# goldenBill/Byzantine_AirComp

Hardware: AMD Instinct MI355X
Metric: GM aggregations/sec at K=1000,d=11M; % HBM roofline; 1/2/4/8 GPUs (higher is better)
Workload: dtype f32; 1 GPU; c3: gm2 K=1000 x d=11000000 fp32, B=200 Byzantine, tol 1e-5, maxiter 1000; K=1000, d=11000000, d_local=11000000, byzantine=200, iters=5, algo=stream, gram_guard=none, layout=panels, parallelism=none, passes_per_aggregation=6, input=row-major fill, packed to panels once (untimed)

## Files before the change

byzantine_aircomp_amd/_lib.py:

```python
from __future__ import annotations

import ctypes as C
import os
import threading

HERE = os.path.dirname(os.path.abspath(__file__))
LIB_PATH = os.environ.get("GMAGG_LIB") or os.path.join(HERE, "libgmagg.so")
ABI_VERSION = 5

GM_MODE_IDEAL, GM_MODE_AIRCOMP = 0, 1
GM_NOISE_PHILOX, GM_NOISE_HOST = 0, 1
GM_ALGO_AUTO, GM_ALGO_STREAM, GM_ALGO_TWOPASS, GM_ALGO_GRAM, GM_ALGO_RESIDENT = 0, 1, 2, 3, 4
GM_ALGO_GRAM_F32 = 5
GM_LAYOUT_ROWS, GM_LAYOUT_PANELS = 0, 1
GM_GUARD_NONE, GM_GUARD_ACCEPTED, GM_GUARD_REJECTED, GM_GUARD_ACCEPTED_FLOOR = 0, 1, 2, 3
GM_EXCHANGE_NONE, GM_EXCHANGE_AGENT, GM_EXCHANGE_XCD_LOCAL, GM_EXCHANGE_XCD_HIER = 0, 1, 2, 3
GM_EXCHANGE_XCD_SPLIT = 4
GM_CLIP_STATIC, GM_CLIP_ARC = 0, 1

NOISE_CB = C.CFUNCTYPE(C.c_int, C.c_void_p, C.c_int64, C.POINTER(C.c_float),
                       C.POINTER(C.c_float), C.POINTER(C.c_float))
ALLREDUCE_CB = C.CFUNCTYPE(C.c_int, C.c_void_p, C.c_void_p, C.c_int64, C.c_void_p)


class GmOpts(C.Structure):
    _fields_ = [
        ("maxiter", C.c_int64),
        ("tol", C.c_double),
        ("eps", C.c_double),
        ("mode", C.c_int32),
        ("has_noise", C.c_int32),
        ("noise_var", C.c_double),
        ("P_max", C.c_double),
        ("seed", C.c_uint64),
        ("noise_source", C.c_int32),
        ("algo", C.c_int32),
        ("noise_cb", NOISE_CB),
        ("noise_user", C.c_void_p),
        ("check_every", C.c_int32),
        ("layout", C.c_int32),
        ("pre_oma", C.c_int32),
        ("pre_oma_var", C.c_double),
        ("pre_oma_seed", C.c_uint64),
    ]


class GmResult(C.Structure):
    _fields_ = [
        ("iters", C.c_int64),
        ("last_movement", C.c_double),
        ("converged", C.c_int32),
        ("algo_used", C.c_int32),
        ("guard", C.c_int32),
        ("gram_kind", C.c_int32),
        ("exchange", C.c_int32),
    ]


class GmCclipOpts(C.Structure):
    _fields_ = [
        ("tau", C.c_double),
        ("maxiter", C.c_int64),
        ("tol", C.c_double),
        ("layout", C.c_int32),
        ("check_every", C.c_int32),
    ]


class GmCclipResult(C.Structure):
    _fields_ = [
        ("iters", C.c_int64),
        ("last_movement", C.c_double),
        ("converged", C.c_int32),
        ("clipped", C.c_int32),
    ]


_P = C.c_void_p
_I64 = C.c_int64
SIGNATURES = [
    ("gm_ctx_create", C.c_int, [C.c_int, C.POINTER(_P)]),
    ("gm_ctx_destroy", C.c_int, [_P]),
    ("gm_ctx_set_shard", C.c_int, [_P, _I64, _I64]),
    ("gm_ctx_set_allreduce", C.c_int, [_P, ALLREDUCE_CB, _P]),
    ("gm_rccl_get_unique_id", C.c_int, [_P]),
    ("gm_ctx_init_rccl", C.c_int, [_P, _P, C.c_int, C.c_int]),
    ("gm_weiszfeld_f32", C.c_int, [_P, _P, _I64, _I64, _I64, _P, _P, C.POINTER(GmOpts),
                                   C.POINTER(GmResult), _P]),
    ("gm_panel_width", _I64, [_I64]),
    ("gm_weiszfeld_bf16", C.c_int, [_P, _P, _I64, _I64, _I64, _P, _P, C.POINTER(GmOpts),
                                    C.POINTER(GmResult), _P]),
    ("gm_panel_width_bf16", _I64, [_I64]),
    ("gm_cclip_f32", C.c_int, [_P, _P, _I64, _I64, _I64, _P, _P, C.POINTER(GmCclipOpts),
                               C.POINTER(GmCclipResult), _P]),
    ("gm_cclip_bf16", C.c_int, [_P, _P, _I64, _I64, _I64, _P, _P, C.POINTER(GmCclipOpts),
                                C.POINTER(GmCclipResult), _P]),
    ("gm_weiszfeld_batched_f32", C.c_int, [_P, _P, _I64, _I64, _I64, _I64, _I64, _P, _I64, _P,
                                           _I64, C.POINTER(GmOpts), C.POINTER(GmResult), _P]),
    ("gm_mean_f32", C.c_int, [_P, _P, _I64, _I64, _I64, _P, _P]),
    ("gm_median_f32", C.c_int, [_P, _P, _I64, _I64, _I64, _P, _P]),
    ("gm_trimmed_mean_f32", C.c_int, [_P, _P, _I64, _I64, _I64, _I64, _P, _P]),
    ("gm_krum_f32", C.c_int, [_P, _P, _I64, _I64, _I64, _I64, _P, C.POINTER(_I64), _P]),
    ("gm_mean_panels_f32", C.c_int, [_P, _P, _I64, _I64, _I64, _P, _P]),
    ("gm_median_panels_f32", C.c_int, [_P, _P, _I64, _I64, _I64, _P, _P]),
    ("gm_trimmed_mean_panels_f32", C.c_int, [_P, _P, _I64, _I64, _I64, _I64, _P, _P]),
    ("gm_krum_panels_f32", C.c_int, [_P, _P, _I64, _I64, _I64, _I64, _P, C.POINTER(_I64), _P]),
    ("gm_krum_last_info", C.c_int, [_P, C.POINTER(_I64)]),
    ("gm_meamed_f32", C.c_int, [_P, _P, _I64, _I64, _I64, C.c_int32, _P, _I64, _I64, _P, _P]),
    ("gm_multi_krum_f32", C.c_int, [_P, _P, _I64, _I64, _I64, C.c_int32, _I64, _I64, _P, _P, _P]),
    ("gm_bulyan_f32", C.c_int, [_P, _P, _I64, _I64, _I64, C.c_int32, _I64, _P, _P, _P]),
    ("gm_nnm_f32", C.c_int, [_P, _P, _I64, _I64, _I64, C.c_int32, _I64, _P, _I64, C.c_int32, _P,
                             _P]),
    ("gm_dnc_f32", C.c_int, [_P, _P, _I64, _I64, _I64, C.c_int32, _P, _I64, _I64, _I64, _I64,
                             C.c_double, _P, _P, C.POINTER(C.c_int32), C.POINTER(_I64),
                             C.POINTER(C.c_int32), C.POINTER(C.c_int32), _P]),
    ("gm_fltrust_f32", C.c_int, [_P, _P, _I64, _I64, _I64, C.c_int32, _P, _I64, _P, _P, _P, _P]),
    ("gm_fltrust_bf16", C.c_int, [_P, _P, _I64, _I64, _I64, C.c_int32, _P, _I64, _P, _P, _P, _P]),
    ("gm_clip_rows_f32", C.c_int, [_P, _P, _I64, _I64, _I64, C.c_int32, _P, C.c_int32, _I64,
                                   C.c_double, _P, _I64, C.c_int32, _P, _P]),
    ("gm_clip_rows_bf16", C.c_int, [_P, _P, _I64, _I64, _I64, C.c_int32, _P, C.c_int32, _I64,
                                    C.c_double, _P, _I64, C.c_int32, _P, _P]),
    ("gm_oma_philox_f32", C.c_int, [_P, _P, _I64, _I64, _I64, C.c_double, C.c_uint64, _P]),
    ("gm_honest_variance_f32", C.c_int, [_P, _P, _I64, _I64, _I64, _P, _P]),
    ("gm_honest_variance_panels_f32", C.c_int, [_P, _P, _I64, _I64, _I64, _I64, _P, _P]),
    ("gm_oma_philox_batched_f32", C.c_int,
     [_P, _P, _I64, _I64, _I64, _I64, _I64, C.c_double, C.c_uint64, _P]),
    ("gm_oma_philox_panels_f32", C.c_int, [_P, _P, _I64, _I64, _I64, C.c_double, C.c_uint64,
                                            _P]),
    ("gm_oma_philox_batched_panels_f32", C.c_int,
     [_P, _P, _I64, _I64, _I64, _I64, _I64, C.c_double, C.c_uint64, _P]),
    ("gm_rows_to_panels_f32", C.c_int, [_P, _P, _I64, _I64, _I64, _P, _I64, _I64, _P]),
    ("gm_rows_to_panels_bf16_from_f32", C.c_int, [_P, _P, _I64, _I64, _I64, _P, _I64, _I64, _P]),
    ("gm_rows_to_panels_bf16", C.c_int, [_P, _P, _I64, _I64, _I64, _P, _I64, _I64, _P]),
    ("gm_bucket_means_f32", C.c_int, [_P, _P, _I64, _I64, _I64, C.c_int32, _P, _I64, _P, _I64,
                                      C.c_int32, _P]),
    ("gm_bucket_means_bf16", C.c_int, [_P, _P, _I64, _I64, _I64, C.c_int32, _P, _I64, _P, _I64,
                                       C.c_int32, _P]),
    ("gm_attack_affine_f32", C.c_int, [_P, _P, _I64, _I64, _I64, C.c_int32, _I64, C.c_double,
                                       C.c_double, _P]),
    ("gm_attack_affine_bf16", C.c_int, [_P, _P, _I64, _I64, _I64, C.c_int32, _I64, C.c_double,
                                        C.c_double, _P]),
    ("gm_attack_minmax_f32", C.c_int, [_P, _P, _I64, _I64, _I64, C.c_int32, _I64, C.c_int32,
                                       C.c_int32, C.POINTER(C.c_double), _P]),
    ("gm_oma_apply_f32", C.c_int, [_P, _P, _I64, _I64, _I64, _P, _P, _P, _P, _P]),
    ("gm_client_chain_f32", C.c_int, [_P, _P, _I64, _P, _I64, _I64, _P, _I64, _I64, _I64,
                                      C.c_int32, C.c_float, C.c_float, _P, _P, _P, _I64,
                                      C.c_int32, _P]),
    ("gm_fill_clients_f32", C.c_int, [_P, _P, _I64, _I64, _I64, _I64, C.c_float, C.c_float,
                                      C.c_float, C.c_float, C.c_uint64, _P]),
    ("gm_fill_normal_f32", C.c_int, [_P, _P, _I64, C.c_float, C.c_float, C.c_uint64, _P]),
    ("gm_ctx_pass_timing", C.c_int, [_P, C.c_int, C.POINTER(C.c_double), C.POINTER(_I64)]),
    ("gm_last_error", C.c_char_p, []),
    ("gm_abi_version", C.c_int, []),
]

_lib = None
_lock = threading.Lock()


class GmError(RuntimeError):
    """A libgmagg call returned a negative status."""


def load():
    global _lib
    with _lock:
        if _lib is not None:
            return _lib
        if not os.path.exists(LIB_PATH):
            raise ImportError(
                f"libgmagg.so not found at {LIB_PATH}: build it with `make` (or "
                "__graft_entry__.build()); there is no non-HIP fallback")
        lib = C.CDLL(LIB_PATH)
        for name, res, args in SIGNATURES:
            fn = getattr(lib, name)
            fn.restype, fn.argtypes = res, args
        if lib.gm_abi_version() != ABI_VERSION:
            raise ImportError(f"libgmagg ABI {lib.gm_abi_version()} != {ABI_VERSION}")
        _lib = lib
        return lib


def check(rc: int, what: str = ""):
    if rc != 0:
        msg = (_lib.gm_last_error() or b"").decode(errors="replace") if _lib else ""
        raise GmError(f"{what} failed ({rc}): {msg}")
    return rc
```

byzantine_aircomp_amd/aggregators.py:

```python
from __future__ import annotations

import atexit
import ctypes as C
import math
import operator
import os
from dataclasses import dataclass

import torch

from . import _lib
from .panels import ClientPanels

__all__ = ["gm2", "gm", "cclip", "OMA", "mean", "median", "trimmed_mean", "Krum", "GMResult",
           "last_result", "Context", "context", "honest_variance", "bucketing", "bucketed",
           "multi_krum", "bulyan", "meamed", "nnm", "mixed", "dnc", "fltrust", "clip", "arc",
           "clipped"]


@dataclass
class GMResult:
    iters: int
    last_movement: float
    converged: bool
    algo: str
    guard: str = "none"
    gram_kind: str = ""
    exchange: str = "none"


last_result: GMResult | None = None
_ALGOS = {"auto": _lib.GM_ALGO_AUTO, "stream": _lib.GM_ALGO_STREAM,
          "twopass": _lib.GM_ALGO_TWOPASS, "gram": _lib.GM_ALGO_GRAM,
          "resident": _lib.GM_ALGO_RESIDENT, "gram_f32": _lib.GM_ALGO_GRAM_F32}
_ALGO_NAMES = {v: k for k, v in _ALGOS.items()}
_GUARD_NAMES = {_lib.GM_GUARD_NONE: "none", _lib.GM_GUARD_ACCEPTED: "accepted",
                _lib.GM_GUARD_REJECTED: "rejected", _lib.GM_GUARD_ACCEPTED_FLOOR: "accepted_floor"}


def _result(res) -> "GMResult":
    return GMResult(res.iters, res.last_movement, bool(res.converged),
                    _ALGO_NAMES.get(res.algo_used, "?"), _GUARD_NAMES.get(res.guard, "?"),
                    {1: "f16_split", 2: "bf16_split", 3: "f32"}.get(res.gram_kind, ""),
                    {1: "agent", 2: "xcd_local", 3: "xcd_hier",
                     4: "xcd_split"}.get(res.exchange, "none"))


class Context:

    def __init__(self, device: int):
        self.lib = _lib.load()
        self.device = device
        h = C.c_void_p()
        _lib.check(self.lib.gm_ctx_create(device, C.byref(h)), "gm_ctx_create")
        self.handle = h
        self._keep = []

    def set_shard(self, d_total: int, d_offset: int):
        _lib.check(self.lib.gm_ctx_set_shard(self.handle, d_total, d_offset), "gm_ctx_set_shard")

    def set_allreduce(self, fn):
        def tramp(user, buf, count, stream):
            try:
                fn(buf, count, stream)
                return 0
            except Exception:
                return 1
        cb = _lib.ALLREDUCE_CB(tramp)
        self._keep.append(cb)
        _lib.check(self.lib.gm_ctx_set_allreduce(self.handle, cb, None), "gm_ctx_set_allreduce")

    def init_rccl(self, unique_id: bytes, nranks: int, rank: int):
        buf = C.create_string_buffer(bytes(unique_id), 128)
        _lib.check(self.lib.gm_ctx_init_rccl(self.handle, buf, nranks, rank), "gm_ctx_init_rccl")

    def pass_timing(self, enable: bool):
        ms, n = C.c_double(), C.c_int64()
        _lib.check(self.lib.gm_ctx_pass_timing(self.handle, int(enable), C.byref(ms),
                                               C.byref(n)), "gm_ctx_pass_timing")
        return ms.value, n.value

    def call(self, fn: str, *args):
        with torch.cuda.device(self.device):
            return _lib.check(getattr(self.lib, fn)(self.handle, *args), fn)

    def close(self):
        h, self.handle = getattr(self, "handle", None), None
        if h:
            self.lib.gm_ctx_destroy(h)
        for k, v in list(_contexts.items()):
            if v is self:
                del _contexts[k]

    def __del__(self):
        try:
            if getattr(self, "handle", None):
                self.lib.gm_ctx_destroy(self.handle)
        except Exception:
            pass


_contexts: dict[int, Context] = {}


def close_all():
    for ctx in list(_contexts.values()):
        ctx.close()


if os.environ.get("GMAGG_ATEXIT_CLOSE", "1") != "0":
    atexit.register(close_all)


def context(device: torch.device | int | None = None) -> Context:
    if not torch.cuda.is_available():
        raise RuntimeError("byzantine_aircomp_amd needs a ROCm GPU (torch.cuda.is_available() "
                           "is False); there is no CPU fallback")
    if device is None:
        idx = torch.cuda.current_device()
    elif isinstance(device, int):
        idx = device
    else:
        idx = device.index if device.index is not None else torch.cuda.current_device()
    ctx = _contexts.get(idx)
    if ctx is None:
        ctx = _contexts[idx] = Context(idx)
    return ctx


def _stream_ptr(dev: torch.device) -> int:
    return torch.cuda.current_stream(dev).cuda_stream


def _stage(t: torch.Tensor, bf16_ok: bool = False) -> torch.Tensor:
    if t.dtype != torch.float32 and not (bf16_ok and t.dtype == torch.bfloat16):
        raise TypeError(f"aggregation kernels are fp32 (got {t.dtype})")
    if t.device.type == "cuda":
        return t
    return t.to(torch.device("cuda", torch.cuda.current_device()))


def _unit_rows(X: torch.Tensor):
    if X.stride(-1) != 1 or X.stride(-2) < X.shape[-1] or X.shape[-2] == 0:
        X = X.contiguous()
    return X, max(X.stride(-2), X.shape[-1])


def _rows(X: torch.Tensor):
    if X.dim() != 2:
        raise ValueError(f"wList must be [K, d] (got {tuple(X.shape)})")
    return _unit_rows(X)


def _fp32_panels(p: ClientPanels, who: str) -> ClientPanels:
    if p.dtype != torch.float32:
        raise TypeError(f"{who} is fp32 only (got {p.dtype} ClientPanels); gm2 / gm read bf16")
    return p


def _bf16_operand(X: torch.Tensor):
    if X.dim() != 2:
        raise ValueError(f"wList must be [K, d] (got {tuple(X.shape)})")
    K, d = X.shape
    if (K > 0 and X.stride(1) == 1 and X.stride(0) >= d and X.stride(0) % 8 == 0 and d % 8 == 0
            and X.data_ptr() % 16 == 0):
        return X, X.stride(0), _lib.GM_LAYOUT_ROWS
    P = ClientPanels.from_rows(X)
    return P.data, P.panel_stride, _lib.GM_LAYOUT_PANELS


def _client_operand(wList):
    if isinstance(wList, ClientPanels):
        K, d = wList.shape
        return wList.data, wList.panel_stride, _lib.GM_LAYOUT_PANELS, K, d
    if wList.dtype == torch.bfloat16:
        K, d = wList.shape
        X, ldx, layout = _bf16_operand(_stage(wList, bf16_ok=True))
        return X, ldx, layout, K, d
    X, ldx = _rows(_stage(wList))
    K, d = X.shape
    return X, ldx, _lib.GM_LAYOUT_ROWS, K, d


def _noise_source(options) -> int:
    src = options.get("noise_source", os.environ.get("BYZ_AIRCOMP_NOISE", "device"))
    if src == "device":
        return _lib.GM_NOISE_PHILOX
    if src == "host":
        return _lib.GM_NOISE_HOST
    raise ValueError(f"noise_source must be 'device' or 'host' (got {src!r})")


def _seed(options) -> int:
    if options.get("seed") is not None:
        return int(options["seed"]) & (2 ** 64 - 1)
    return int(torch.randint(0, 2 ** 62, (1,)).item())


def _host_draws(K: int, d: int, noise_var):
    def cb(user, it, hr, hi, n):
        try:
            a = torch.normal(torch.zeros(K), 1 / math.sqrt(2))
            b = torch.normal(torch.zeros(K), 1 / math.sqrt(2))
            C.memmove(hr, a.data_ptr(), 4 * K)
            C.memmove(hi, b.data_ptr(), 4 * K)
            if noise_var is not None:
                z = torch.normal(torch.zeros(d + 1), math.sqrt(noise_var / 2))
                C.memmove(n, z.data_ptr(), 4 * (d + 1))
            return 0
        except Exception:
            return 1
    return _lib.NOISE_CB(cb)


def _gm_opts(opts: dict, aircomp: bool, layout: int, pre_var=None, pre_seed=None, shape=None):
    o = _lib.GmOpts()
    o.maxiter = int(opts["maxiter"])
    o.tol = float(opts["tol"])
    o.eps = 1e-4
    o.mode = _lib.GM_MODE_AIRCOMP if aircomp else _lib.GM_MODE_IDEAL
    o.algo = _ALGOS[opts.get("algo", "auto")]
    o.check_every = int(opts.get("check_every", 0))
    o.layout = layout
    if pre_var is not None:
        o.pre_oma = 1
        o.pre_oma_var = float(pre_var)
        o.pre_oma_seed = _seed({"seed": pre_seed})
    if aircomp:
        var = opts["noise_var"]
        o.has_noise = int(var is not None)
        o.noise_var = float(var) if var is not None else 0.0
        o.P_max = float(opts["P_max"])
        o.noise_source = _noise_source(opts)
        if o.noise_source == _lib.GM_NOISE_HOST:
            o.noise_cb = o.keep_cb = _host_draws(*shape, var)
        else:
            o.seed = _seed(opts)
    return o


def _weiszfeld(wList: torch.Tensor, options: dict, aircomp: bool):
    global last_result
    opts = {"maxiter": 200, "tol": 1e-5}
    if aircomp:
        opts.update({"noise_var": None, "P_max": 1})
    opts.update(options or {})
    pre_var = None if aircomp else opts.get("pre_oma_var")
    pre_seed = opts.get("pre_oma_seed")
    if pre_var is not None and (opts.get("guess") is None or wList.device.type != "cuda"
                                or _noise_source(opts) == _lib.GM_NOISE_HOST):
        OMA(wList, float(pre_var), noise_source=opts.get("noise_source"), seed=pre_seed)
        pre_var = None
    guess = opts.get("guess")
    bf16 = wList.dtype == torch.bfloat16
    if guess is None:
        guess = wList.mean(dim=0, dtype=torch.float32) if bf16 and not isinstance(
            wList, ClientPanels) else wList.mean(dim=0)
    maxiter = int(opts["maxiter"])
    if maxiter <= 0:
        if pre_var is not None:
            OMA(wList, float(pre_var), seed=pre_seed)
        last_result = GMResult(0, float("nan"), False, "none")
        return guess
    X, ldx, layout, K, d = _client_operand(wList)
    g0 = guess.detach().to(device=X.device, dtype=torch.float32).contiguous()
    if g0.numel() != d:
        raise ValueError(f"guess has {g0.numel()} elements, wList rows have {d}")
    out = torch.empty(d, dtype=torch.float32, device=X.device)
    if d == 0:
        last_result = GMResult(1, 0.0, True, "none")
        return out.to(wList.device)

    o = _gm_opts(opts, aircomp, layout, pre_var, pre_seed, (K, d))
    res = _lib.GmResult()
    context(X.device).call("gm_weiszfeld_bf16" if bf16 else "gm_weiszfeld_f32", X.data_ptr(), K, d,
                           ldx, g0.data_ptr(), out.data_ptr(), C.byref(o), C.byref(res),
                           _stream_ptr(X.device))
    last_result = _result(res)
    if pre_var is not None and not isinstance(wList, ClientPanels) and X is not wList:
        wList.copy_(X)
    return out if wList.device == out.device else out.to(wList.device)


def gm2(wList, options={}):
    return _weiszfeld(wList, options, aircomp=False)


def gm(wList, options={}):
    return _weiszfeld(wList, options, aircomp=True)


_CCLIP_KEYS = ("tau", "clip_iters", "clip_tol")


def _cclip_params(options):
    if options.get("tau") is None:
        raise ValueError("cclip needs options['tau'] (the clipping radius; there is no default)")
    tau = float(options["tau"])
    if not tau > 0:
        raise ValueError(f"cclip: tau must be > 0 (got {options['tau']!r})")
    iters = int(options.get("clip_iters", 1))
    if iters < 0:
        raise ValueError(f"cclip: clip_iters must be >= 0 (got {iters})")
    ctol = options.get("clip_tol")
    if ctol is not None and not float(ctol) >= 0:
        raise ValueError(f"cclip: clip_tol must be None or >= 0 (got {ctol!r})")
    return tau, iters, -1.0 if ctol is None else float(ctol)


def _run_cclip(ctx, ptr: int, bf16: bool, K: int, d: int, ldx: int, layout: int, g0, params,
               check_every: int = 0):
    tau, iters, tol = params
    out = torch.empty(d, dtype=torch.float32, device=g0.device)
    o = _lib.GmCclipOpts()
    o.tau, o.maxiter, o.tol, o.layout, o.check_every = tau, iters, tol, layout, check_every
    res = _lib.GmCclipResult()
    ctx.call("gm_cclip_bf16" if bf16 else "gm_cclip_f32", ptr, K, d, ldx, g0.data_ptr(),
             out.data_ptr(), C.byref(o), C.byref(res), _stream_ptr(g0.device))
    return out, GMResult(res.iters, res.last_movement, bool(res.converged),
                         "stream" if iters else "none"), int(res.clipped)


def cclip(wList, options={}):
    global last_result
    options = options or {}
    params = _cclip_params(options)
    if not isinstance(wList, ClientPanels) and wList.dtype not in (torch.float32, torch.bfloat16):
        raise TypeError(f"cclip reads fp32 or bf16 client updates (got {wList.dtype})")
    guess = options.get("guess")
    if guess is None:
        guess = torch.zeros(wList.shape[1], dtype=torch.float32, device=wList.device)
    if params[1] == 0:
        last_result = GMResult(0, float("nan"), False, "none")
        cclip.last_info = {"clipped": 0}
        return guess
    X, ldx, layout, K, d = _client_operand(wList)
    g0 = guess.detach().to(device=X.device, dtype=torch.float32).contiguous()
    if g0.numel() != d:
        raise ValueError(f"guess has {g0.numel()} elements, wList rows have {d}")
    if d == 0:
        last_result = GMResult(1, 0.0, True, "none")
        cclip.last_info = {"clipped": 0}
        return torch.empty(d, dtype=torch.float32, device=wList.device)
    out, last_result, clipped = _run_cclip(
        context(X.device), X.data_ptr(), X.dtype == torch.bfloat16, K, d, ldx, layout, g0, params,
        int(options.get("check_every", 0)))
    cclip.last_info = {"clipped": clipped}
    return out if wList.device == out.device else out.to(wList.device)


def _cclip_with_options(**fixed):
    unknown = sorted(set(fixed) - set(_CCLIP_KEYS))
    if unknown:
        raise TypeError(f"cclip.with_options takes {', '.join(_CCLIP_KEYS)} (got {unknown})")
    _cclip_params(fixed if "tau" in fixed else dict(fixed, tau=1.0))

    def aggregate(wList, options={}):
        return cclip(wList, {**(options or {}), **fixed})
    aggregate.__name__ = aggregate.__qualname__ = "cclip"
    aggregate.__doc__ = f"cclip with {fixed}"
    return aggregate


cclip.with_options = _cclip_with_options
cclip.last_info = {"clipped": 0}


def _fp32_operand(wList, who: str, fn: str):
    if isinstance(wList, ClientPanels):
        _fp32_panels(wList, who)
        return (wList.data, wList.panel_stride, *wList.shape, fn.replace("_f32", "_panels_f32"))
    X, ldx = _rows(_stage(wList))
    return (X, ldx, *X.shape, fn)


def _coordinate(wList, fn_name, *extra):
    X, ldx, K, d, fn_name = _fp32_operand(wList, fn_name[3:-4], fn_name)
    out = torch.empty(d, dtype=torch.float32, device=X.device)
    context(X.device).call(fn_name, X.data_ptr(), K, d, ldx, *extra, out.data_ptr(),
                           _stream_ptr(X.device))
    return out if wList.device == out.device else out.to(wList.device)


def mean(wList, options={}):
    return _coordinate(wList, "gm_mean_f32")


def median(wList, options={}):
    return _coordinate(wList, "gm_median_f32")


def trimmed_mean(wList, options={}):
    return _coordinate(wList, "gm_trimmed_mean_f32", int(wList.shape[0] * 0.1))


def Krum(wList, options):
    X, ldx, K, d, fn = _fp32_operand(wList, "Krum", "gm_krum_f32")
    out = torch.empty(d, dtype=torch.float32, device=X.device)
    idx = C.c_int64()
    ctx = context(X.device)
    ctx.call(fn, X.data_ptr(), K, d, ldx, int(options["honestSize"]), out.data_ptr(),
             C.byref(idx), _stream_ptr(X.device))
    info = (C.c_int64 * 3)()
    _lib.check(ctx.lib.gm_krum_last_info(ctx.handle, info), "gm_krum_last_info")
    Krum.last_index = idx.value
    Krum.last_info = {"algo": ("exact", "gram")[info[0]], "candidates": info[1],
                      "reason": ("ok", "not_chosen", "not_eligible", "gram_nonfinite",
                                 "candidates")[info[2]]}
    return out if wList.device == out.device else out.to(wList.device)


def _robust_operand(wList, who: str):
    if isinstance(wList, ClientPanels):
        _fp32_panels(wList, who)
        return (wList.data, wList.panel_stride, _lib.GM_LAYOUT_PANELS, *wList.shape)
    X, ldx = _rows(_stage(wList))
    return (X, ldx, _lib.GM_LAYOUT_ROWS, *X.shape)


def _robust_shape(wList, who: str):
    if isinstance(wList, ClientPanels):
        _fp32_panels(wList, who)
    elif not isinstance(wList, torch.Tensor) or wList.dtype != torch.float32:
        raise TypeError(f"{who} is fp32 only (got {getattr(wList, 'dtype', type(wList))})")
    elif wList.dim() != 2:
        raise ValueError(f"wList must be [K, d] (got {tuple(wList.shape)})")
    K, d = (int(n) for n in wList.shape)
    if K < 1:
        raise ValueError(f"{who}: wList has no rows")
    return K, d


def _honest_size(options, who: str) -> int:
    if not options or options.get("honestSize") is None:
        raise ValueError(f"{who} needs options['honestSize']")
    return int(options["honestSize"])


def meamed(wList, options):
    K, d = _robust_shape(wList, "meamed")
    keep = _honest_size(options, "meamed")
    if not 1 <= keep <= K:
        raise ValueError(f"meamed: honestSize {keep} not in [1, {K}]")
    if K > 1024:
        raise ValueError(f"meamed: K <= 1024 (got {K})")
    X, ldx, layout, K, d = _robust_operand(wList, "meamed")
    out = torch.empty(d, dtype=torch.float32, device=X.device)
    context(X.device).call("gm_meamed_f32", X.data_ptr(), K, d, ldx, layout, None, K, keep,
                           out.data_ptr(), _stream_ptr(X.device))
    return out if wList.device == out.device else out.to(wList.device)


def multi_krum(wList, options):
    K, d = _robust_shape(wList, "multi_krum")
    honest = _honest_size(options, "multi_krum")
    if not 2 <= honest <= K + 1:
        raise ValueError(f"multi_krum: honestSize {honest} not in [2, {K + 1}]")
    m = options.get("m")
    m = honest if m is None else int(m)
    if not 1 <= m <= K:
        raise ValueError(f"multi_krum: m = {m} not in [1, {K}]")
    if K > 4096:
        raise ValueError(f"multi_krum: K <= 4096 (got {K})")
    X, ldx, layout, K, d = _robust_operand(wList, "multi_krum")
    out = torch.empty(d, dtype=torch.float32, device=X.device)
    sel = (C.c_int32 * m)()
    if d > 0:
        context(X.device).call("gm_multi_krum_f32", X.data_ptr(), K, d, ldx, layout, honest, m,
                               out.data_ptr(), sel, _stream_ptr(X.device))
    multi_krum.last_selected = list(sel) if d > 0 else []
    return out if wList.device == out.device else out.to(wList.device)


multi_krum.last_selected = None


def bulyan(wList, options):
    K, d = _robust_shape(wList, "bulyan")
    honest = _honest_size(options, "bulyan")
    f = K - honest
    if honest < 1 or f < 0:
        raise ValueError(f"bulyan: honestSize {honest} not in [1, {K}]")
    if K < 4 * f + 3:
        raise ValueError(f"bulyan: K = {K} < 4f + 3 = {4 * f + 3} with f = K - honestSize = {f}")
    if K > 1024:
        raise ValueError(f"bulyan: K <= 1024 (got {K})")
    X, ldx, layout, K, d = _robust_operand(wList, "bulyan")
    out = torch.empty(d, dtype=torch.float32, device=X.device)
    theta = K - 2 * f
    sel = (C.c_int32 * theta)()
    if d > 0:
        context(X.device).call("gm_bulyan_f32", X.data_ptr(), K, d, ldx, layout, honest,
                               out.data_ptr(), sel, _stream_ptr(X.device))
    bulyan.last_selected = list(sel) if d > 0 else []
    return out if wList.device == out.device else out.to(wList.device)


bulyan.last_selected = None


def _bucket_size(s) -> int:
    try:
        if isinstance(s, bool):
            raise TypeError
        n = operator.index(s)
    except TypeError:
        raise ValueError(f"bucketing: s must be an integer >= 1 (got {s!r})") from None
    if n < 1:
        raise ValueError(f"bucketing: s must be >= 1 (got {s!r})")
    return n


def _assignment(K: int, s: int, generator=None) -> torch.Tensor:
    _bucket_size(s)
    return torch.randperm(int(K), generator=generator)


def _bucket_perm(perm, K: int) -> torch.Tensor:
    p = torch.as_tensor(perm).detach().cpu()
    if p.dim() != 1 or p.numel() != K or p.dtype.is_floating_point or p.dtype == torch.bool:
        raise ValueError(f"bucketing: perm must be {K} integers (got {tuple(p.shape)} {p.dtype})")
    p = p.to(torch.int64)
    if not torch.equal(torch.sort(p).values, torch.arange(K)):
        raise ValueError(f"bucketing: perm is not a permutation of 0..{K - 1}")
    return p


def bucketing(wList, s, perm=None, generator=None, layout=None):
    s = _bucket_size(s)
    if layout not in (None, "rows", "panels"):
        raise ValueError(f"bucketing: layout must be None, 'rows' or 'panels' (got {layout!r})")
    panels_in = isinstance(wList, ClientPanels)
    if not panels_in and (not isinstance(wList, torch.Tensor) or wList.dim() != 2):
        raise ValueError("bucketing: wList must be a [K, d] tensor or ClientPanels")
    if wList.dtype not in (torch.float32, torch.bfloat16):
        raise TypeError(f"bucketing reads fp32 or bf16 client updates (got {wList.dtype})")
    if s == 1:
        return wList
    K, d = (int(n) for n in wList.shape)
    if K < 1:
        raise ValueError("bucketing: wList has no rows")
    p = _bucket_perm(perm, K) if perm is not None else _assignment(K, s, generator)
    bucketing.last_perm = p
    if panels_in:
        X, ldx, lin = wList.data, wList.panel_stride, _lib.GM_LAYOUT_PANELS
    else:
        X, ldx = _unit_rows(_stage(wList, bf16_ok=True))
        lin = _lib.GM_LAYOUT_ROWS
    Kb = -(-K // s)
    if layout == "panels" or (layout is None and panels_in):
        out = ClientPanels(Kb, d, device=X.device, zero=False)
        Y, ldy, lout = out.data, out.panel_stride, _lib.GM_LAYOUT_PANELS
    else:
        out = Y = torch.empty(Kb, d, dtype=torch.float32, device=X.device)
        ldy, lout = max(d, 1), _lib.GM_LAYOUT_ROWS
    if d > 0:
        pdev = p.to(device=X.device, dtype=torch.int32)
        context(X.device).call(
            "gm_bucket_means_bf16" if X.dtype == torch.bfloat16 else "gm_bucket_means_f32",
            X.data_ptr(), K, d, ldx, lin, pdev.data_ptr(), s, Y.data_ptr(), ldy, lout,
            _stream_ptr(X.device))
    if out is Y and wList.device != Y.device:
        return Y.to(wList.device)
    return out


bucketing.assignment = _assignment
bucketing.last_perm = None


def bucketed(aggregate, s, generator=None, layout="panels"):
    s = _bucket_size(s)
    if layout not in (None, "rows", "panels"):
        raise ValueError(f"bucketed: layout must be None, 'rows' or 'panels' (got {layout!r})")

    def agg(wList, options={}):
        if s == 1:
            return aggregate(wList, options)
        K = int(wList.shape[0])
        Kb = -(-K // s)
        opts = options
# ... 484 lines not shown
```

byzantine_aircomp_amd/csrc/api.hip:

```cpp
#include <cstring>

#include "host_ctx.h"

using namespace gmh;

extern "C" {

const char* gm_last_error(void) { return g_err.c_str(); }
int gm_abi_version(void) { return GMAGG_ABI_VERSION; }

int64_t gm_panel_width(int64_t K) {
  PassCfg cfg{};
  return K >= 1 && pick_cfg(K, 4, 1, &cfg, true) ? (int64_t)cfg.LPR * cfg.V : 0;
}

int64_t gm_panel_width_bf16(int64_t K) {
  PassCfg cfg{};
  return K >= 1 && pick_cfg(K, 8, 1, &cfg, true, true) ? (int64_t)cfg.LPR * cfg.V : 0;
}

int gm_ctx_create(int device, gm_ctx** out) {
  if (!out) return fail(GM_ERR_INVALID, "gm_ctx_create: out is NULL");
  *out = nullptr;
  int n = 0;
  HIPCHK(hipGetDeviceCount(&n));
  if (device < 0 || device >= n)
    return fail(GM_ERR_INVALID, "gm_ctx_create: device %d of %d", device, n);
  gm_ctx* c = new gm_ctx();
  c->device = device;
  hipDeviceProp_t prop;
  if (hipGetDeviceProperties(&prop, device) == hipSuccess && prop.multiProcessorCount > 0)
    c->num_cu = prop.multiProcessorCount;
  *out = c;
  return GM_OK;
}

int gm_ctx_destroy(gm_ctx* c) {
  if (!c) return GM_OK;
  (void)hipSetDevice(c->device);
  if (c->comm) ncclCommDestroy(c->comm);
  if (c->ws) (void)hipFree(c->ws);
  if (c->stage) (void)hipFree(c->stage);
  if (c->host) (void)hipHostFree(c->host);
  for (auto e : c->poll_ev)
    if (e) (void)hipEventDestroy(e);
  for (auto e : c->ev_free) (void)hipEventDestroy(e);
  for (auto& p : c->ev_used) {
    (void)hipEventDestroy(p.first);
    (void)hipEventDestroy(p.second);
  }
  delete c;
  return GM_OK;
}

int gm_ctx_set_shard(gm_ctx* c, int64_t d_total, int64_t d_offset) {
  if (!c || d_total < -1 || d_offset < 0) return fail(GM_ERR_INVALID, "gm_ctx_set_shard: bad args");
  c->d_total = d_total;
  c->d_offset = d_offset;
  return GM_OK;
}

int gm_ctx_set_allreduce(gm_ctx* c, gm_allreduce_cb fn, void* user) {
  if (!c) return fail(GM_ERR_INVALID, "gm_ctx_set_allreduce: ctx is NULL");
  c->ar_fn = fn;
  c->ar_user = user;
  return GM_OK;
}

int gm_rccl_get_unique_id(void* uid) {
  if (!uid) return fail(GM_ERR_INVALID, "gm_rccl_get_unique_id: NULL");
  static_assert(sizeof(ncclUniqueId) == 128, "ncclUniqueId size");
  ncclUniqueId id;
  ncclResult_t r = ncclGetUniqueId(&id);
  if (r != ncclSuccess) return fail(GM_ERR_COMM, "ncclGetUniqueId: %s", ncclGetErrorString(r));
  memcpy(uid, &id, sizeof id);
  return GM_OK;
}

int gm_ctx_init_rccl(gm_ctx* c, const void* uid, int nranks, int rank) {
  if (!c || !uid || nranks < 1 || rank < 0 || rank >= nranks)
    return fail(GM_ERR_INVALID, "gm_ctx_init_rccl: bad args");
  HIPCHK(hipSetDevice(c->device));
  ncclUniqueId id;
  memcpy(&id, uid, sizeof id);
  ncclResult_t r = ncclCommInitRank(&c->comm, nranks, id, rank);
  if (r != ncclSuccess) {
    c->comm = nullptr;
    return fail(GM_ERR_COMM, "ncclCommInitRank: %s", ncclGetErrorString(r));
  }
  return GM_OK;
}

int gm_ctx_pass_timing(gm_ctx* c, int enable, double* total_ms, int64_t* launches) {
  if (!c) return fail(GM_ERR_INVALID, "gm_ctx_pass_timing: ctx is NULL");
  double tot = 0.0;
  int64_t n = 0;
  for (auto& p : c->ev_used) {
    HIPCHK(hipEventSynchronize(p.second));
    float ms = 0.f;
    HIPCHK(hipEventElapsedTime(&ms, p.first, p.second));
    tot += ms;
    ++n;
    c->ev_free.push_back(p.first);
    c->ev_free.push_back(p.second);
  }
  c->ev_used.clear();
  if (total_ms) *total_ms = tot;
  if (launches) *launches = n;
  c->timing = enable != 0;
  return GM_OK;
}

int gm_mean_f32(gm_ctx* c, const float* X, int64_t K, int64_t d, int64_t ldx, float* out,
                void* stream) {
  if (!c || !X || !out || K < 1 || d < 0 || ldx < d) return fail(GM_ERR_INVALID, "gm_mean_f32: bad args");
  if (d == 0) return GM_OK;
  HIPCHK(hipSetDevice(c->device));
  HIPCHK(launch_col_mean(X, K, d, ldx, out, reinterpret_cast<hipStream_t>(stream)));
  return GM_OK;
}

static int panel_shift(int64_t K, int64_t panel_stride, int* ws) {
  const int64_t W = gm_panel_width(K);
  if (W == 0 || panel_stride < K * W) return GM_ERR_INVALID;
  *ws = wshift_of(W);
  return GM_OK;
}

static int col_select(const char* fn, gm_ctx* c, const float* X, int64_t K, int64_t d, int64_t ldx,
                      int ws, int mode, int64_t trim, float* out, void* stream) {
  if (K > 2048) return fail(GM_ERR_UNSUPPORTED, "%s: K <= 2048", fn);
  if (d == 0) return GM_OK;
  HIPCHK(hipSetDevice(c->device));
  HIPCHK(launch_col_select(X, K, d, ldx, mode, trim, out, reinterpret_cast<hipStream_t>(stream),
                           ws));
  return GM_OK;
}

int gm_mean_panels_f32(gm_ctx* c, const float* X, int64_t K, int64_t d, int64_t panel_stride,
                       float* out, void* stream) {
  int ws = 0;
  if (!c || !X || !out || K < 1 || d < 0 || panel_shift(K, panel_stride, &ws))
    return fail(GM_ERR_INVALID, "gm_mean_panels_f32: bad args");
  if (d == 0) return GM_OK;
  HIPCHK(hipSetDevice(c->device));
  HIPCHK(launch_col_mean(X, K, d, panel_stride, out, reinterpret_cast<hipStream_t>(stream), ws));
  return GM_OK;
}

int gm_median_panels_f32(gm_ctx* c, const float* X, int64_t K, int64_t d, int64_t panel_stride,
                         float* out, void* stream) {
  int ws = 0;
  if (!c || !X || !out || K < 1 || d < 0 || panel_shift(K, panel_stride, &ws))
    return fail(GM_ERR_INVALID, "gm_median_panels_f32: bad args");
  return col_select("gm_median_panels_f32", c, X, K, d, panel_stride, ws, 0, 0, out, stream);
}

int gm_trimmed_mean_panels_f32(gm_ctx* c, const float* X, int64_t K, int64_t d,
                               int64_t panel_stride, int64_t trim, float* out, void* stream) {
  int ws = 0;
  if (!c || !X || !out || K < 1 || d < 0 || trim < 0 || 2 * trim >= K ||
      panel_shift(K, panel_stride, &ws))
    return fail(GM_ERR_INVALID, "gm_trimmed_mean_panels_f32: bad args");
  return col_select("gm_trimmed_mean_panels_f32", c, X, K, d, panel_stride, ws, 1, trim, out,
                    stream);
}

static int honest_variance(gm_ctx* c, const float* X, int64_t honest, int64_t d, int64_t ldx,
                           int wshift, float* out, void* stream) {
  hipStream_t s = reinterpret_cast<hipStream_t>(stream);
  WsOrder order(c, s);
  HIPCHK(order.err);
  const int nb = honest_var_blocks(d, c->num_cu);
  Workspace w;
  const int rc = ensure_ws(c, 1, 1, nb, &w);
  if (rc) return rc;
  HIPCHK(launch_honest_var(X, honest, d, ldx, wshift, nb, w.slab, out, s));
  return GM_OK;
}

int gm_honest_variance_f32(gm_ctx* c, const float* X, int64_t honest, int64_t d, int64_t ldx,
                           float* out, void* stream) {
  if (!c || !X || !out || honest < 1 || d < 1 || ldx < d)
    return fail(GM_ERR_INVALID, "gm_honest_variance_f32: bad args");
  return honest_variance(c, X, honest, d, ldx, 0, out, stream);
}

int gm_honest_variance_panels_f32(gm_ctx* c, const float* X, int64_t K, int64_t honest, int64_t d,
                                  int64_t panel_stride, float* out, void* stream) {
  const int64_t W = gm_panel_width(K);
  if (!c || !X || !out || honest < 1 || honest > K || d < 1 || W == 0 || panel_stride < K * W)
    return fail(GM_ERR_INVALID, "gm_honest_variance_panels_f32: bad args");
  return honest_variance(c, X, honest, d, panel_stride, wshift_of(W), out, stream);
}

int gm_median_f32(gm_ctx* c, const float* X, int64_t K, int64_t d, int64_t ldx, float* out,
                  void* stream) {
  if (!c || !X || !out || K < 1 || d < 0 || ldx < d) return fail(GM_ERR_INVALID, "gm_median_f32: bad args");
  return col_select("gm_median_f32", c, X, K, d, ldx, 0, 0, 0, out, stream);
}

int gm_trimmed_mean_f32(gm_ctx* c, const float* X, int64_t K, int64_t d, int64_t ldx,
                        int64_t trim, float* out, void* stream) {
  if (!c || !X || !out || K < 1 || d < 0 || ldx < d || trim < 0 || 2 * trim >= K)
    return fail(GM_ERR_INVALID, "gm_trimmed_mean_f32: bad args");
  return col_select("gm_trimmed_mean_f32", c, X, K, d, ldx, 0, 1, trim, out, stream);
}

static int krum_impl(gm_ctx* c, const float* X, int64_t K, int64_t d, int64_t ldx, int ws,
                     int64_t honest, float* out, int64_t* index, void* stream);

int gm_krum_f32(gm_ctx* c, const float* X, int64_t K, int64_t d, int64_t ldx, int64_t honest,
                float* out, int64_t* index, void* stream) {
  if (!c || !X || !out || K < 1 || d < 0 || ldx < d || honest < 2 || honest - 1 > K)
    return fail(GM_ERR_INVALID, "gm_krum_f32: bad args (needs 2 <= honestSize <= K+1)");
  if (K > 4096) return fail(GM_ERR_UNSUPPORTED, "gm_krum_f32: K <= 4096");
  return krum_impl(c, X, K, d, ldx, 0, honest, out, index, stream);
}

int gm_krum_panels_f32(gm_ctx* c, const float* X, int64_t K, int64_t d, int64_t panel_stride,
                       int64_t honest, float* out, int64_t* index, void* stream) {
  int ws = 0;
  if (!c || !X || !out || K < 1 || d < 0 || honest < 2 || honest - 1 > K ||
      panel_shift(K, panel_stride, &ws))
    return fail(GM_ERR_INVALID, "gm_krum_panels_f32: bad args (needs 2 <= honestSize <= K+1)");
  if (K > 4096) return fail(GM_ERR_UNSUPPORTED, "gm_krum_panels_f32: K <= 4096");
  return krum_impl(c, X, K, d, panel_stride, ws, honest, out, index, stream);
}

static double krum_gram_eps() { return 6e-5; }

static int krum_mode() {
  const char* e = getenv("GMAGG_KRUM");
  return e ? atoi(e) : 2;
}

static int krum_gram(gm_ctx* c, const float* X, int64_t K, int64_t d, int64_t ldx, int ws,
                     int64_t honest, float* out, int64_t* index, hipStream_t s, bool* done) {
  *done = false;
  const int KT = gram_kt(K), KP = 32 * KT;
  const int64_t kk = honest - 1;
  const GramGrid gg = gram_grid(d, GramKind::H16, c->num_cu);
  const int64_t S = krum_slices(K, d);
  const int64_t RC = krum_refine_max();
  const int64_t maxc = 4 * RC;
  size_t body = std::max(gram_slab_floats(KT, gg), (size_t)2 * (size_t)(S * RC * K + RC * K));
  body = (body + 1) / 2 * 2;
  Workspace w;
  int rc = ensure_ws(c, K, d, 1, &w, body + 2 * (size_t)(maxc + 2), KP);
  if (rc) return rc;
  rc = ensure_host(c, sizeof(KState) + 2 * sizeof(int64_t));
  if (rc) return rc;
  double* part = reinterpret_cast<double*>(w.gslab);
  double* Dc = part + (size_t)S * RC * K;
  int64_t* cand = reinterpret_cast<int64_t*>(w.gslab + body);
  int64_t* didx = reinterpret_cast<int64_t*>(w.r);
  KState* hst = host_state(c);
  int64_t* hcand = host_after_states<int64_t>(c);
  const int64_t W = ws ? (int64_t)1 << ws : 0;
  int64_t n = 0, centre = 0;
  for (int attempt = 0; attempt < 2; ++attempt) {
    float* p = w.g[1];
    HIPCHK(launch_copy_row_k(X, d, ldx, ws, centre, p, s));
    HIPCHK(hipMemsetAsync(w.st, 0, sizeof(KState), s));
    HIPCHK(launch_gram(X, K, d, ws ? W : ldx, p, GramKind::H16, gg, w.gslab, w.G, w.st, s,
                       ws ? ldx : 0, ws));
    HIPCHK(launch_gram_check(w.G, KP, w.st, s));
    HIPCHK(launch_krum_gram_select(w.G, KP, K, kk, krum_gram_eps(),
                                   gram_block_exp(w.gslab, KT, gg), gg.nb, d, w.alpha, w.u, maxc,
                                   cand, s));
    HIPCHK(hipMemcpyAsync(hst, w.st, sizeof(KState), hipMemcpyDeviceToHost, s));
    HIPCHK(hipMemcpyAsync(hcand, cand, sizeof(int64_t), hipMemcpyDeviceToHost, s));
    HIPCHK(hipMemcpyAsync(hcand + 1, cand + maxc + 1, sizeof(int64_t), hipMemcpyDeviceToHost, s));
    HIPCHK(hipStreamSynchronize(s));
    if (hst->gram_bad) {
      c->krum_info[2] = GM_KRUM_REASON_GRAM_NONFINITE;
      return GM_OK;
    }
    n = hcand[0];
    if (n != -2 || hcand[1] == centre) break;
    centre = hcand[1];
  }
  if (n < 1) {
    c->krum_info[2] = GM_KRUM_REASON_CANDIDATES;
    return GM_OK;
  }
  for (int64_t q = 0; q < n; q += RC) {
    const int m = (int)std::min<int64_t>(RC, n - q);
    HIPCHK(launch_krum_refine(X, K, d, ldx, ws, cand + 1 + q, m, kk, part, Dc, w.sums + q, s));
  }
  HIPCHK(launch_krum_pick(w.sums, cand + 1, n, X, d, ldx, ws, didx, out, s));
  if (index) {
    HIPCHK(hipMemcpyAsync(index, didx, sizeof(int64_t), hipMemcpyDeviceToHost, s));
    HIPCHK(hipStreamSynchronize(s));
  }
  c->krum_info[0] = GM_KRUM_GRAM;
  c->krum_info[1] = n;
  c->krum_info[2] = GM_KRUM_REASON_OK;
  *done = true;
  return GM_OK;
}

int gm_krum_last_info(gm_ctx* c, int64_t* info) {
  if (!c || !info) return fail(GM_ERR_INVALID, "gm_krum_last_info: bad args");
  for (int i = 0; i < 3; ++i) info[i] = c->krum_info[i];
  return GM_OK;
}

static int krum_impl(gm_ctx* c, const float* X, int64_t K, int64_t d, int64_t ldx, int ws,
                     int64_t honest, float* out, int64_t* index, void* stream) {
  const hipStream_t s = reinterpret_cast<hipStream_t>(stream);
  WsOrder order(c, s);
  HIPCHK(order.err);
  c->krum_info[0] = GM_KRUM_EXACT;
  c->krum_info[1] = 0;
  c->krum_info[2] = GM_KRUM_REASON_NOT_CHOSEN;
  const bool eligible =
      gram_kt(K) > 0 && d > 0 && honest - 1 <= K &&
      (ws ? (ws >= 6 && ws <= 8 && K * ((int64_t)1 << ws) * 4 <= 0x7fffffff)
          : (d % 4 == 0 && ldx % 4 == 0 && (reinterpret_cast<uintptr_t>(X) & 15) == 0 &&
             ldx < ((int64_t)1 << 26)));
  const int mode = krum_mode();
  const bool want = mode == 1 || (mode == 2 && K >= 64 && (double)K * K * d >= 536870912.0);
  if (want && !eligible) c->krum_info[2] = GM_KRUM_REASON_NOT_ELIGIBLE;
  if (want && eligible) {
    bool done = false;
    const int rc = krum_gram(c, X, K, d, ldx, ws, honest, out, index, s, &done);
    if (rc || done) return rc;
  }
  Workspace w;
  const size_t part_doubles = (size_t)krum_slices(K, d) * (size_t)(K * K);
  int rc = ensure_ws(c, K, 1, 1, &w, 2 * part_doubles, (int)K);
  if (rc) return rc;
  int64_t* didx = reinterpret_cast<int64_t*>(w.u);
  HIPCHK(launch_krum(X, K, d, ldx, honest - 1, w.G, reinterpret_cast<double*>(w.gslab), w.alpha,
                     out, didx, s, ws));
  if (index) {
    HIPCHK(hipMemcpyAsync(index, didx, sizeof(int64_t), hipMemcpyDeviceToHost, s));
    HIPCHK(hipStreamSynchronize(s));
  }
  return GM_OK;
}


static int robust_shift(const char* fn, int64_t K, int64_t d, int64_t ldx, int32_t layout,
                        int* ws) {
  *ws = 0;
  if (layout == GM_LAYOUT_ROWS) {
    if (ldx < d) return fail(GM_ERR_INVALID, "%s: ldx = %lld < d", fn, (long long)ldx);
    return GM_OK;
  }
  const int64_t W = gm_panel_width(K);
  if (W == 0)
    return fail(GM_ERR_UNSUPPORTED, "%s: no panel layout for K = %lld rows (pass them row-major)",
                fn, (long long)K);
  if (ldx < K * W)
    return fail(GM_ERR_INVALID, "%s: panel stride %lld < K * W = %lld", fn, (long long)ldx,
                (long long)(K * W));
  *ws = wshift_of(W);
  return GM_OK;
}

static bool known_layout(int32_t l) { return l == GM_LAYOUT_ROWS || l == GM_LAYOUT_PANELS; }

int gm_meamed_f32(gm_ctx* c, const float* X, int64_t K, int64_t d, int64_t ldx, int32_t layout,
                  const int32_t* rows, int64_t n_rows, int64_t keep, float* out, void* stream) {
  if (!c || !X || !out || K < 1 || d < 0 || !known_layout(layout) || n_rows < 1 || n_rows > K ||
      (!rows && n_rows != K) || keep < 1 || keep > n_rows)
    return fail(GM_ERR_INVALID, "gm_meamed_f32: bad args (a NULL ctx, X or out, K < 1, d < 0, an "
                "unknown layout, n_rows outside [1, K] or != K without rows, keep outside "
                "[1, n_rows])");
  if (K > 1024) return fail(GM_ERR_UNSUPPORTED, "gm_meamed_f32: K <= 1024 (got %lld)", (long long)K);
  int ws = 0;
  const int rc = robust_shift("gm_meamed_f32", K, d, ldx, layout, &ws);
  if (rc) return rc;
  if (d == 0) return GM_OK;
  HIPCHK(hipSetDevice(c->device));
  HIPCHK(launch_meamed(X, d, ldx, ws, rows, n_rows, keep, out,
                       reinterpret_cast<hipStream_t>(stream)));
  return GM_OK;
}

static int krum_distances(gm_ctx* c, const float* X, int64_t K, int64_t d, int64_t ldx, int ws,
                          Workspace* w, hipStream_t s) {
  const size_t part_doubles = (size_t)krum_slices(K, d) * (size_t)(K * K);
  const int rc = ensure_ws(c, K, 1, 1, w, 2 * part_doubles, (int)K);
  if (rc) return rc;
  HIPCHK(launch_krum_dist(X, K, d, ldx, ws, w->G, reinterpret_cast<double*>(w->gslab), s));
  return GM_OK;
}

static int copy_selected(int32_t* selected, const int32_t* dev, int64_t n, hipStream_t s) {
  if (!selected) return GM_OK;
  HIPCHK(hipMemcpyAsync(selected, dev, sizeof(int32_t) * (size_t)n, hipMemcpyDeviceToHost, s));
  HIPCHK(hipStreamSynchronize(s));
  return GM_OK;
}

int gm_multi_krum_f32(gm_ctx* c, const float* X, int64_t K, int64_t d, int64_t ldx, int32_t layout,
                      int64_t honest, int64_t m, float* out, int32_t* selected, void* stream) {
  if (!c || !X || !out || K < 1 || d < 0 || !known_layout(layout) || honest < 2 ||
      honest - 1 > K || m < 1 || m > K)
    return fail(GM_ERR_INVALID, "gm_multi_krum_f32: bad args (a NULL ctx, X or out, K < 1, d < 0, "
                "an unknown layout; needs 2 <= honestSize <= K+1 and 1 <= m <= K)");
  if (K > 4096)
    return fail(GM_ERR_UNSUPPORTED, "gm_multi_krum_f32: K <= 4096 (got %lld)", (long long)K);
  int ws = 0;
  int rc = robust_shift("gm_multi_krum_f32", K, d, ldx, layout, &ws);
  if (rc) return rc;
  if (d == 0) return GM_OK;
  const hipStream_t s = reinterpret_cast<hipStream_t>(stream);
  WsOrder order(c, s);
  HIPCHK(order.err);
  Workspace w;
  rc = krum_distances(c, X, K, d, ldx, ws, &w, s);
  if (rc) return rc;
  HIPCHK(launch_krum_scores(w.G, K, honest - 1, w.alpha, s));
  int32_t* flag = reinterpret_cast<int32_t*>(w.u);
  int32_t* list = flag + K;
  HIPCHK(launch_multi_krum_pick(w.alpha, K, m, X, d, ldx, ws, flag, list, out, s));
  return copy_selected(selected, list, m, s);
}

int gm_bulyan_f32(gm_ctx* c, const float* X, int64_t K, int64_t d, int64_t ldx, int32_t layout,
                  int64_t honest, float* out, int32_t* selected, void* stream) {
  const int64_t f = K - honest;
  if (!c || !X || !out || K < 1 || d < 0 || !known_layout(layout) || honest < 1 || f < 0 ||
      K < 4 * f + 3)
    return fail(GM_ERR_INVALID, "gm_bulyan_f32: bad args (a NULL ctx, X or out, K < 1, d < 0, an "
                "unknown layout; needs f = K - honestSize >= 0 and K >= 4f + 3)");
  if (K > 1024) return fail(GM_ERR_UNSUPPORTED, "gm_bulyan_f32: K <= 1024 (got %lld)", (long long)K);
  int ws = 0;
  int rc = robust_shift("gm_bulyan_f32", K, d, ldx, layout, &ws);
  if (rc) return rc;
  if (d == 0) return GM_OK;
  const int64_t theta = K - 2 * f, beta = theta - 2 * f;
  const hipStream_t s = reinterpret_cast<hipStream_t>(stream);
  WsOrder order(c, s);
  HIPCHK(order.err);
  Workspace w;
  rc = krum_distances(c, X, K, d, ldx, ws, &w, s);
  if (rc) return rc;
  int32_t* alive = reinterpret_cast<int32_t*>(w.u);
  int32_t* list = alive + K;
  int32_t* picked = reinterpret_cast<int32_t*>(w.r);
  int32_t* ord = reinterpret_cast<int32_t*>(w.gslab);
  HIPCHK(launch_bulyan_select(w.G, K, f, theta, w.alpha, ord, alive, picked, list, s));
  HIPCHK(launch_meamed(X, d, ldx, ws, list, theta, beta, out, s));
  return copy_selected(selected, picked, theta, s);
}

static int nnm_stop() { return env_int("GMAGG_NNM_STOP", 0); }

int gm_nnm_f32(gm_ctx* c, const float* X, int64_t K, int64_t d, int64_t ldx, int32_t layout_in,
               int64_t f, float* Y, int64_t ldy, int32_t layout_out, int32_t* neighbors,
               void* stream) {
  if (!c || !X || !Y || K < 1 || d < 0 || f < 0 || f > K - 1 || !known_layout(layout_in) ||
      !known_layout(layout_out))
    return fail(GM_ERR_INVALID, "gm_nnm_f32: bad args (a NULL ctx, X or Y, K < 1, d < 0, f outside "
                "[0, K - 1] or an unknown layout)");
  if (K > 4096) return fail(GM_ERR_UNSUPPORTED, "gm_nnm_f32: K <= 4096 (got %lld)", (long long)K);
  int ws = 0, wsy = 0;
  int rc = robust_shift("gm_nnm_f32", K, d, ldx, layout_in, &ws);
  if (rc) return rc;
  rc = robust_shift("gm_nnm_f32", K, d, ldy, layout_out, &wsy);
  if (rc) return rc;
  if (d == 0) return GM_OK;
  if (c->d_total > 0 || c->comm || c->ar_fn)
    return fail(GM_ERR_UNSUPPORTED, "gm_nnm_f32: a d-sharded or collective context (the distances would need a "
                "K x K all-reduce)");
  const int64_t m = K - f;
  const hipStream_t s = reinterpret_cast<hipStream_t>(stream);
  WsOrder order(c, s);
  HIPCHK(order.err);
  const size_t part_doubles = (size_t)krum_slices(K, d) * (size_t)(K * K);
  Workspace w;
  rc = ensure_ws(c, K, 1, 1, &w, std::max(2 * part_doubles, (size_t)nnm_mask_words(K)), (int)K);
  if (rc) return rc;
  HIPCHK(launch_krum_dist(X, K, d, ldx, ws, w.G, reinterpret_cast<double*>(w.gslab), s));
  const int stop = nnm_stop();
  if (stop == 1) return GM_OK;
  uint32_t* mask = reinterpret_cast<uint32_t*>(w.gslab);
  HIPCHK(launch_nnm_neighbors(w.G, K, m, mask, neighbors, s));
  if (stop == 2) return GM_OK;
  HIPCHK(launch_nnm_mix(X, K, d, ldx, ws, mask, m, Y, ldy, wsy, s));
  return GM_OK;
}

static int dnc_stop() { return env_int("GMAGG_DNC_STOP", 0); }

constexpr int64_t kDncMaxElems = (int64_t)1 << 27;

int gm_dnc_f32(gm_ctx* c, const float* X, int64_t K, int64_t d, int64_t ldx, int32_t layout,
               const int64_t* columns, int64_t n, int64_t iters, int64_t remove,
               int64_t power_iters, double power_tol, float* out, double* scores, int32_t* good,
               int64_t* n_good, int32_t* niter, int32_t* converged, void* stream) {
  if (!c || !X || !out || !scores || !good || !n_good || !niter || !converged ||
      (remove > 0 && !columns))
    return fail(GM_ERR_INVALID, "gm_dnc_f32: a NULL ctx, X, out, scores, good, n_good, niter or "
                "converged, or NULL columns with remove > 0");
  if (K < 2 || d < 0 || !known_layout(layout) || iters < 1 || remove < 0 || remove >= K ||
      (remove > 0 && iters > (K - 1) / remove) || power_iters < 1 || !(power_tol >= 0) ||
      (remove > 0 && (n < 1 || n > d)))
    return fail(GM_ERR_INVALID, "gm_dnc_f32: bad args (K < 2, d < 0, an unknown layout, iters < 1, "
                "remove < 0, remove * iters >= K, power_iters < 1, power_tol not >= 0, n outside "
                "[1, d])");
  if (K > 4096) return fail(GM_ERR_UNSUPPORTED, "gm_dnc_f32: K <= 4096 (got %lld)", (long long)K);
  if (remove > 0 && n > kDncMaxElems / K)
    return fail(GM_ERR_UNSUPPORTED, "gm_dnc_f32: K * n = %lld x %lld sampled elements exceed %lld",
                (long long)K, (long long)n, (long long)kDncMaxElems);
  int ws = 0;
  int rc = robust_shift("gm_dnc_f32", K, d, ldx, layout, &ws);
  if (rc) return rc;
  if (c->d_total > 0 || c->comm || c->ar_fn)
    return fail(GM_ERR_UNSUPPORTED, "gm_dnc_f32: a d-sharded or collective context (the sampled "
                "columns and the final mean would span the shards)");
  const hipStream_t s = reinterpret_cast<hipStream_t>(stream);
  if (remove == 0) {
    HIPCHK(hipSetDevice(c->device));
    if (d > 0) HIPCHK(launch_col_mean(X, K, d, ldx, out, s, ws));
    HIPCHK(hipMemsetAsync(scores, 0, sizeof(double) * (size_t)(iters * K), s));
    for (int64_t t = 0; t < iters; ++t) { niter[t] = 0; converged[t] = 1; }
    for (int64_t k = 0; k < K; ++k) good[k] = (int32_t)k;
    *n_good = K;
    return GM_OK;
  }
  WsOrder order(c, s);
  HIPCHK(order.err);
  DncWork w{};
  dnc_slices(K, n, &w.slices, &w.slice_rows);
  int32_t *flag = nullptr, *goodf = nullptr, *list = nullptr;
  auto lay = [&](char* base) {
    Carve cv{base};
    w.st = cv.take<DncState>(1);
    w.G = cv.take<float>((size_t)(K * n));
    w.mu = cv.take<double>(n);
    w.v = cv.take<double>(n);
    w.w = cv.take<double>(n);
    w.part = cv.take<double>((size_t)(w.slices * n));
    w.p = cv.take<double>(K);
    w.bn = cv.take<double>(kDncBlocks);
    w.bm = cv.take<double>(kDncBlocks);
    flag = cv.take<int32_t>(K);
    goodf = cv.take<int32_t>(K);
    list = cv.take<int32_t>(K);
    return cv.off;
  };
  rc = grow_ws(c, lay(nullptr));
  if (rc) return rc;
  lay(c->ws);
  rc = ensure_host(c, 256 + sizeof(int32_t) * (size_t)K);
  if (rc) return rc;
  DncState* hst = reinterpret_cast<DncState*>(c->host);
  int32_t* hflag = reinterpret_cast<int32_t*>(c->host + 256);
  const int stop = dnc_stop();
  for (int64_t t = 0; t < iters; ++t) {
    HIPCHK(launch_dnc_gather(X, K, ldx, ws, columns + t * n, n, w.G, s));
    if (stop == 1) return GM_OK;
    HIPCHK(launch_dnc_center(w, K, n, s));
    HIPCHK(launch_dnc_start(w, K, n, s));
    for (int64_t it = 0; it < power_iters;) {
      const int64_t chunk = std::min<int64_t>(it == 0 ? 8 : 16, power_iters - it);
      HIPCHK(launch_dnc_iterate(w, K, n, power_tol, chunk, s));
      it += chunk;
      HIPCHK(hipMemcpyAsync(hst, w.st, sizeof(DncState), hipMemcpyDeviceToHost, s));
      HIPCHK(hipStreamSynchronize(s));
      if (hst->done) break;
    }
    niter[t] = hst->iters;
    converged[t] = hst->converged;
    double* sc = scores + t * K;
    HIPCHK(launch_dnc_scores(w, K, n, sc, s));
    HIPCHK(launch_score_top_m(sc, K, K - remove, flag, s));
    HIPCHK(launch_dnc_and_flags(goodf, flag, K, t == 0, s));
  }
  HIPCHK(launch_flags_to_list(goodf, K, 1, list, s));
  HIPCHK(hipMemcpyAsync(hflag, goodf, sizeof(int32_t) * (size_t)K, hipMemcpyDeviceToHost, s));
  HIPCHK(hipStreamSynchronize(s));
  int64_t m = 0;
  for (int64_t k = 0; k < K; ++k)
    if (hflag[k]) good[m++] = (int32_t)k;
  *n_good = m;
  if (stop == 2) return GM_OK;
  HIPCHK(launch_gather_mean(X, d, ldx, ws, list, m, out, s));
  return GM_OK;
}

int gm_oma_philox_f32(gm_ctx* c, float* X, int64_t K, int64_t d, int64_t ldx, double noise_var,
                      uint64_t seed, void* stream) {
  if (!c || !X || K < 0 || d < 0 || ldx < d || noise_var < 0)
    return fail(GM_ERR_INVALID, "gm_oma_philox_f32: bad args");
  if (K == 0 || d == 0) return GM_OK;
  HIPCHK(hipSetDevice(c->device));
  const int64_t d_total = c->d_total > 0 ? c->d_total : d;
  const int64_t col_off = c->d_total > 0 ? c->d_offset : 0;
  HIPCHK(launch_oma_philox(X, K, d, ldx, d_total, col_off, (float)std::sqrt(noise_var), seed,
                           reinterpret_cast<hipStream_t>(stream)));
  return GM_OK;
}

int gm_oma_philox_batched_f32(gm_ctx* c, float* X, int64_t P, int64_t K, int64_t d, int64_t ldx,
                              int64_t pstride, double noise_var, uint64_t seed, void* stream) {
  if (!c || !X || P < 0 || K < 0 || d < 0 || ldx < d || noise_var < 0 ||
      (P > 1 && pstride < K * ldx))
    return fail(GM_ERR_INVALID, "gm_oma_philox_batched_f32: bad args");
// ... 262 lines not shown
```

byzantine_aircomp_amd/csrc/gmagg_internal.h:

```cpp
#pragma once
#include <hip/hip_runtime.h>
#include <stdint.h>

namespace gmk {

constexpr int kTPB = 1024;
constexpr int kWaves = kTPB / 64;

struct alignas(64) KState {
  int32_t done;
  int32_t converged;
  int64_t iters;
  double last_movement;
  float a_noise;
  float s;
  double guard_q;
  double guard_r;
  int32_t gram_bad;
  int32_t clipped;
  double pad1;
};

struct PassCfg {
  int V, NW, LPR, R;
  int OCC = 1;
  bool B16 = false;
};

struct PassArgs {
  const float* X;
  int64_t K, d, ldx;
  const float* g_old;
  float* g_new;
  const float* coef;
  const KState* st;
  double* slab;
  int64_t slab_stride;
  int noise;
  const float* hnoise;
  uint64_t seed;
  int64_t iter;
  int64_t col_off;
  int64_t x_ps, gold_ps, gnew_ps;
  int64_t panel_stride;
  float oma_sd;
  uint64_t oma_seed;
  int chunk_pair;
};

__host__ __device__ inline int64_t first_chunk(int P, int64_t b, int64_t grid) {
  if (P <= 0 || grid % (2 * P) != 0) return b;
  return 2 * ((b / (2 * P)) * P + b % P) + (b / P) % 2;
}

constexpr uint64_t kSeedStride = 0x9E3779B97F4A7C15ull;
constexpr double kFloorUlps = 2.0;

constexpr int kModeCclip = 2;

struct KspaceArgs {
  int64_t K, d_total, t;
  int mode;
  int has_noise, noise_src;
  float tol, eps;
  double P_max, noise_sd;
  uint64_t seed;
  int do_check, do_coef;
  const double* sums;
  double* r;
  const float* h_re;
  const float* h_im;
  const float* n_last;
  float* coef;
  KState* st;
  int64_t sums_ps;
  int* n_done;
  KState* mirror;
  double tau;
};

constexpr int kPassStepSelf = 5;
hipError_t launch_pass(const PassCfg& cfg, int mode, int grid, const PassArgs& a, hipStream_t s,
                       int problems = 1);
int pass_blocks_per_cu(const PassCfg& cfg, int mode);
bool rows_pass_eligible(const PassArgs& a, int mode);
hipError_t launch_rows_pass(int mode, int grid, const PassArgs& a, hipStream_t s);
bool pass_cfg_supported(const PassCfg& cfg);
int pass_variant();
const void* pass_kernel_bf16(const PassCfg& cfg, int mode, bool panel);
const void* pass_kernel_self(const PassCfg& cfg, bool panel);

hipError_t launch_slab_reduce(const double* slab, int nb, int64_t S, double* sums,
                              const KState* st, hipStream_t s, int problems = 1,
                              int64_t sums_ps = 0);
hipError_t launch_kspace(const KspaceArgs& a, hipStream_t s, int problems = 1);
hipError_t launch_twopass(bool init, const float* X, int64_t K, int64_t d, int64_t ldx,
                          const float* g_old, float* g_new, const float* coef, const KState* st,
                          int noise, const float* hnoise, uint64_t seed, int64_t iter,
                          int64_t col_off, double* slab, int nb, double* sums, hipStream_t s);
int twopass_blocks(int64_t K, int64_t d, int num_cu);
hipError_t launch_batched_finalize(const float* g0, const float* g1, int64_t d, int problems,
                                   const KState* st, float* out, int64_t ldo, hipStream_t s);

struct ResArgs {
  const float* X;
  int64_t K, d, ldx;
  int64_t pstride;
  int wshift;
  const float* guess0;
  float* out;
  int64_t maxiter;
  float tol, eps;
  int mode, has_noise;
  double P_max, noise_sd;
  uint64_t seed;
  unsigned long long* gran;
  unsigned* bar;
  unsigned long long* checkin;
  unsigned need;
  unsigned stride;
  int local;
  int hier;
  unsigned long long* lvl2;
  int split;
  unsigned long long* granL;
  KState* st;
};
bool resident_plan(const PassCfg& cfg, int64_t nch, int num_cu, int* cpb, int* nb);
size_t resident_gran_words(int64_t K, const PassCfg& cfg, int nb);
bool resident_has_exchange(const PassCfg& cfg, int cpb, int xg);
hipError_t launch_resident(const PassCfg& cfg, int cpb, int grid, const ResArgs& a, hipStream_t s);
bool res_coop_launch();

struct ResBArgs {
  const float* X;
  int64_t P, K, d, ldx, x_ps, pstride;
  int wshift;
  int prob_bytes;
  int nb;
  const float* guess0;
  int64_t ldg;
  float* out;
  int64_t ldo;
  int64_t maxiter;
  float tol, eps;
  int mode, has_noise;
  double P_max, noise_sd;
  uint64_t seed;
  int pre_oma;
  float oma_sd;
  uint64_t oma_seed;
  unsigned long long* gran;
  unsigned* flag;
  unsigned long long* checkin;
  unsigned need;
  int xcd_major;
  int local;
  int hier;
  unsigned long long* lvl2;
  KState* st;
};
struct RbPlan {
  int kr;
  int nb;
  int ng;
  int mode;
};
bool rb_plan(int64_t K, int64_t d, int64_t P, int mode, int num_cu, RbPlan* plan,
             bool xcd_whole = false);
size_t rb_gran_words(int64_t K, const RbPlan& plan);
hipError_t launch_resident_batched(const RbPlan& plan, const ResBArgs& a, bool coop, hipStream_t s);

enum class GramKind { F32, BF16, H16 };
struct GramGrid {
  int nb;
  int64_t cpb;
  int nseg;
};
int gram_kt(int64_t K);
GramGrid gram_grid(int64_t d, GramKind kind, int num_cu);
size_t gram_slab_floats(int KT, const GramGrid& g);
int* gram_block_exp(float* slab, int KT, const GramGrid& g);
hipError_t launch_gram(const float* X, int64_t K, int64_t d, int64_t ldx, const float* p,
                       GramKind kind, const GramGrid& g, float* slab, double* G, KState* st,
                       hipStream_t s, int64_t pstride = 0, int wshift = 0);
hipError_t launch_gram_check(const double* G, int KP, KState* st, hipStream_t s);
hipError_t launch_gram_verify(const double* G, int KP, int64_t K, float eps, const double* u,
                              const double* alpha, const double* Dx, double* bvec, KState* st,
                              hipStream_t s);
hipError_t launch_gram_solve(const double* G, int KP, int64_t K, int64_t maxiter, float tol,
                             float eps, double* alpha, double* u, float* coef, KState* st,
                             hipStream_t s);

hipError_t launch_col_mean(const float* X, int64_t K, int64_t d, int64_t ldx, float* out,
                           hipStream_t s, int ws = 0);
hipError_t launch_col_select(const float* X, int64_t K, int64_t d, int64_t ldx, int mode,
                             int64_t b, float* out, hipStream_t s, int ws = 0);
int honest_var_blocks(int64_t d, int num_cu);
hipError_t launch_honest_var(const float* X, int64_t H, int64_t d, int64_t ldx, int wshift,
                             int nb, double* part, float* out, hipStream_t s);
int64_t krum_slices(int64_t K, int64_t d);
hipError_t launch_krum(const float* X, int64_t K, int64_t d, int64_t ldx, int64_t kk, double* D,
                       double* part, double* score, float* out, int64_t* index, hipStream_t s,
                       int ws = 0);
hipError_t launch_krum_dist(const float* X, int64_t K, int64_t d, int64_t ldx, int ws, double* D,
                            double* part, hipStream_t s);
hipError_t launch_krum_scores(const double* D, int64_t K, int64_t kk, double* score,
                              hipStream_t s);
hipError_t launch_meamed(const float* X, int64_t d, int64_t ldx, int ws, const int32_t* rows,
                         int64_t n, int64_t keep, float* out, hipStream_t s);
hipError_t launch_multi_krum_pick(const double* score, int64_t K, int64_t m, const float* X,
                                  int64_t d, int64_t ldx, int ws, int32_t* flag, int32_t* list,
                                  float* out, hipStream_t s);
hipError_t launch_score_top_m(const double* score, int64_t K, int64_t m, int32_t* flag,
                              hipStream_t s);
hipError_t launch_flags_to_list(const int32_t* flag, int64_t K, int32_t want, int32_t* list,
                                hipStream_t s);
hipError_t launch_gather_mean(const float* X, int64_t d, int64_t ldx, int ws, const int32_t* list,
                              int64_t m, float* out, hipStream_t s);
hipError_t launch_bulyan_select(const double* D, int64_t K, int64_t f, int64_t theta,
                                double* score, int32_t* ord, int32_t* alive, int32_t* order,
                                int32_t* list, hipStream_t s);
hipError_t launch_copy_row_k(const float* X, int64_t d, int64_t ldx, int ws, int64_t k, float* out,
                             hipStream_t s);
hipError_t launch_krum_gram_select(const double* G, int KP, int64_t K, int64_t kk, double epsg,
                                   const int* bexp, int nb, int64_t d, double* lb, double* ub,
                                   int64_t maxc, int64_t* cand, hipStream_t s);
int krum_refine_max();
hipError_t launch_krum_refine(const float* X, int64_t K, int64_t d, int64_t ldx, int ws,
                              const int64_t* cidx, int m, int64_t kk, double* part, double* Dc,
                              double* score, hipStream_t s);
hipError_t launch_krum_pick(const double* score, const int64_t* cidx, int64_t m, const float* X,
                            int64_t d, int64_t ldx, int ws, int64_t* index, float* out,
                            hipStream_t s);

struct ClientChainArgs {
  const float* data;
  int64_t ldd;
  const int64_t* labels;
  int64_t F, C;
  const int* idx;
  int64_t K, B, honest;
  int attack;
  float gamma, wd;
  float* W;
  float* b;
  float* X;
  int64_t ldx;
  int64_t pstride;
  int wshift;
  int stage;
};
bool client_chain_supported(int64_t F, int64_t C, int64_t B);
hipError_t launch_client_chain(const ClientChainArgs& a, hipStream_t s);

hipError_t launch_oma_apply(float* X, int64_t K, int64_t d, int64_t ldx, const float* hr,
                            const float* hi, const float* nr, const float* ni, hipStream_t s);
hipError_t launch_rows_to_panels(const float* X, int64_t K, int64_t d, int64_t ldx, float* P,
                                 int64_t W, int64_t pstride, hipStream_t s);
hipError_t launch_rows_to_panels_bf16(const void* X, bool src_f32, int64_t K, int64_t d,
                                      int64_t ldx, uint16_t* P, int64_t W, int64_t pstride,
                                      hipStream_t s);
hipError_t launch_bucket_means(const void* X, bool bf16, int64_t K, int64_t d, int64_t ldx,
                               int64_t Wi, const int32_t* perm, int64_t s, float* Y, int64_t ldy,
                               int64_t Wo, hipStream_t stream);
int64_t nnm_mask_words(int64_t K);
hipError_t launch_nnm_neighbors(const double* D, int64_t K, int64_t m, uint32_t* mask,
                                int32_t* list, hipStream_t s);
hipError_t launch_nnm_mix(const float* X, int64_t K, int64_t d, int64_t ldx, int ws,
                          const uint32_t* mask, int64_t m, float* Y, int64_t ldy, int wsy,
                          hipStream_t s);
struct DncState {
  int32_t done;
  int32_t converged;
  int32_t iters;
  int32_t degenerate;
  int64_t kstar;
  double val;
  double movement;
};
constexpr int kDncBlocks = 1024;
struct DncWork {
  float* G;
  double* mu;
  double* v;
  double* w;
  double* part;
  double* p;
  double* bn;
  double* bm;
  DncState* st;
  int64_t slices, slice_rows;
};
void dnc_slices(int64_t K, int64_t n, int64_t* slices, int64_t* slice_rows);
hipError_t launch_dnc_gather(const float* X, int64_t K, int64_t ldx, int ws, const int64_t* cols,
                             int64_t n, float* G, hipStream_t s);
hipError_t launch_dnc_center(const DncWork& w, int64_t K, int64_t n, hipStream_t s);
hipError_t launch_dnc_start(const DncWork& w, int64_t K, int64_t n, hipStream_t s);
hipError_t launch_dnc_iterate(const DncWork& w, int64_t K, int64_t n, double tol, int64_t count,
                              hipStream_t s);
hipError_t launch_dnc_scores(const DncWork& w, int64_t K, int64_t n, double* score, hipStream_t s);
hipError_t launch_dnc_and_flags(int32_t* good, const int32_t* flag, int64_t K, bool first,
                                hipStream_t s);
hipError_t launch_attack_affine(void* X, bool bf16, int64_t K, int64_t H, int64_t d, int64_t ldx,
                                int ws, double a, double b, hipStream_t stream);
int attack_term_blocks(int64_t d);
hipError_t launch_attack_minmax(float* X, int64_t K, int64_t H, int64_t d, int64_t ldx, int ws,
                                int rule, int dev, const double* D, double* mu, double* p,
                                double* slab, int nb, double* sums, double* rb, double* gam,
                                hipStream_t stream);
hipError_t launch_oma_philox(float* X, int64_t K, int64_t d, int64_t ldx, int64_t d_total,
                             int64_t col_off, float sd, uint64_t seed, hipStream_t s,
                             int wshift = 0, int64_t problems = 1, int64_t pstride = 0);
hipError_t launch_fill_clients(float* X, int64_t K, int64_t d, int64_t ldx, int64_t B,
                               float mu_h, float sd_h, float mu_b, float sd_b, int64_t d_total,
                               int64_t col_off, uint64_t seed, hipStream_t s);
hipError_t launch_fill_normal(float* v, int64_t n, float mu, float sd, int64_t off,
                              uint64_t seed, hipStream_t s);

}
```

byzantine_aircomp_amd/csrc/host_ctx.h:

```cpp
#pragma once
#include <rccl/rccl.h>

#include <algorithm>
#include <cmath>
#include <cstdarg>
#include <cstdio>
#include <cstdlib>
#include <string>
#include <utility>
#include <vector>

#include "../../include/gmagg.h"
#include "gmagg_internal.h"

struct gm_ctx {
  int device = 0;
  int num_cu = 256;
  int64_t d_total = -1;
  int64_t d_offset = 0;
  gm_allreduce_cb ar_fn = nullptr;
  void* ar_user = nullptr;
  ncclComm_t comm = nullptr;
  char* ws = nullptr;
  size_t ws_bytes = 0;
  char* host = nullptr;
  size_t host_bytes = 0;
  bool timing = false;
  hipEvent_t poll_ev[2] = {nullptr, nullptr};
  std::vector<hipEvent_t> ev_free;
  std::vector<std::pair<hipEvent_t, hipEvent_t>> ev_used;
  hipEvent_t ws_ev = nullptr;
  hipStream_t ws_stream = nullptr;
  bool ws_pending = false;
  float* stage = nullptr;
  size_t stage_bytes = 0;
  int res_skip = 0;
  int64_t krum_info[3] = {GM_KRUM_EXACT, 0, GM_KRUM_REASON_NOT_CHOSEN};
};

namespace gmh {

using namespace gmk;

inline thread_local std::string g_err;

inline int fail(int code, const char* fmt, ...) __attribute__((format(printf, 2, 3)));
inline int fail(int code, const char* fmt, ...) {
  char buf[512];
  va_list ap;
  va_start(ap, fmt);
  vsnprintf(buf, sizeof buf, fmt, ap);
  va_end(ap);
  g_err = buf;
  return code;
}

#define HIPCHK(expr)                                                                    \
  do {                                                                                  \
    hipError_t e_ = (expr);                                                             \
    if (e_ != hipSuccess)                                                               \
      return fail(GM_ERR_HIP, "%s failed: %s (%s:%d)", #expr, hipGetErrorString(e_),    \
                  __FILE__, __LINE__);                                                  \
  } while (0)

constexpr size_t align_up(size_t v, size_t a) { return (v + a - 1) / a * a; }

inline int wshift_of(int64_t W) {
  int ws = 0;
  while (((int64_t)1 << ws) < W) ++ws;
  return ws;
}

constexpr int kDeclined = 1;

inline int env_int(const char* name, int dflt) {
  const char* e = getenv(name);
  return e ? atoi(e) : dflt;
}
inline int env_pos(const char* name, int dflt) {
  const int v = env_int(name, 0);
  return v > 0 ? v : dflt;
}


constexpr int kResSkipAfterCheckinFail = 64;

inline bool resident_allowed(gm_ctx* c) {
  if (c->res_skip <= 0) return true;
  --c->res_skip;
  return false;
}

inline unsigned checkin_need(unsigned blocks) {
  return blocks + (env_int("GMAGG_RES_CHECKIN_FAIL", 0) != 0 ? 1u : 0u);
}

inline int res_xcd_mode() { return env_int("GMAGG_RES_XCD", 2); }
inline int rb_hier_mode() { return env_int("GMAGG_RB_HIER", 0); }
inline int res_split_mode() { return env_int("GMAGG_RES_SPLIT", 1); }
inline int res_hier_mode() { return env_int("GMAGG_RES_HIER", 1); }
inline unsigned res_xcd_stride(int nb, int num_cu) {
  static const int bpc = std::max(1, env_int("GMAGG_RES_XCD_BPC", 1));
  return (res_xcd_mode() != 0 && nb <= num_cu / 8 * bpc) ? 8u : 1u;
}
inline void resident_tile(PassCfg* cfg, int64_t K) {
  if (cfg->LPR != 64) return;
  int nw = 0, r = 0;
  if (const char* e = getenv("GMAGG_RES_CFG")) {
    if (sscanf(e, "%d,%d", &nw, &r) != 2 || (int64_t)nw * r < K) nw = 0;
  } else if (K > 32 && K <= 64 && cfg->NW == 16 && cfg->R == 4) {
    nw = 8;
    r = 8;
  }
  if (nw > 0) {
    cfg->NW = nw;
    cfg->R = r;
  }
}
inline int rb_xcd_major() {
  return env_int("GMAGG_RB_XCD", 1);
}


inline double noise_sd(const gm_opts* o) { return std::sqrt(std::max(0.0, o->noise_var) / 2.0); }
inline int aircomp_noise(const gm_opts* o) { return o->mode == GM_MODE_AIRCOMP && o->has_noise; }
inline float pre_oma_sd(const gm_opts* o) {
  return (float)std::sqrt(std::max(0.0, o->pre_oma_var));
}
struct AirNoise {
  int has_noise;
  double noise_sd, P_max;
  uint64_t seed;
};
inline AirNoise air_noise(const gm_opts* o) {
  return {aircomp_noise(o), noise_sd(o), o->P_max, o->seed};
}
inline KspaceArgs kspace_args(int64_t K, int64_t d_total, int mode, double tol, double eps,
                              const AirNoise& n) {
  KspaceArgs ka{};
  ka.K = K;
  ka.d_total = d_total;
  ka.mode = mode;
  ka.has_noise = n.has_noise;
  ka.tol = (float)tol;
  ka.eps = (float)eps;
  ka.P_max = n.P_max;
  ka.noise_sd = n.noise_sd;
  ka.seed = n.seed;
  return ka;
}

inline gm_result result_from(const KState& st, int algo) {
  gm_result r{};
  r.iters = st.iters;
  r.last_movement = st.last_movement;
  r.converged = st.converged;
  r.algo_used = algo;
  return r;
}


struct WsOrder {
  gm_ctx* c;
  hipStream_t s;
  hipError_t err;
  WsOrder(gm_ctx* c_, hipStream_t s_) : c(c_), s(s_), err(hipSetDevice(c_->device)) {
    if (err == hipSuccess && !c->ws_ev) err = hipEventCreateWithFlags(&c->ws_ev, hipEventDisableTiming);
    if (err == hipSuccess && c->ws_pending && c->ws_stream != s)
      err = hipStreamWaitEvent(s, c->ws_ev, 0);
  }
  ~WsOrder() {
    if (c->ws_ev && hipEventRecord(c->ws_ev, s) == hipSuccess) {
      c->ws_stream = s;
      c->ws_pending = true;
    }
  }
};

inline int grow_ws(gm_ctx* c, size_t bytes) {
  if (bytes <= c->ws_bytes) return GM_OK;
  if (c->ws) HIPCHK(hipFree(c->ws));
  c->ws = nullptr;
  c->ws_bytes = 0;
  HIPCHK(hipMalloc(&c->ws, bytes));
  c->ws_bytes = bytes;
  return GM_OK;
}

struct Carve {
  char* base;
  size_t off = 0;
  template <class T>
  T* take(size_t count) {
    const size_t o = off;
    off = align_up(off + sizeof(T) * count, 256);
    return base ? reinterpret_cast<T*>(base + o) : nullptr;
  }
};

struct Workspace {
  KState* st;
  double* sums;
  double* r;
  float* coef;
  double* slab;
  float* g[2];
  float* h_re;
  float* h_im;
  float* hnoise;
  float* gslab;
  double* G;
  double* alpha;
  double* u;
};

inline int ensure_ws(gm_ctx* c, int64_t K, int64_t d, int nb, Workspace* w,
                     size_t gram_slab_n = 0, int KP = 0) {
  const size_t S = 2 * K + 2;
  auto lay = [&](char* base) {
    Carve cv{base};
    w->st = cv.take<KState>(1);
    w->sums = cv.take<double>(S);
    w->r = cv.take<double>(K);
    w->coef = cv.take<float>(K);
    w->slab = cv.take<double>(S * (size_t)nb);
    w->g[0] = cv.take<float>(d);
    w->g[1] = cv.take<float>(d);
    w->h_re = cv.take<float>(K);
    w->h_im = cv.take<float>(K);
    w->hnoise = cv.take<float>(d + 1);
    w->gslab = cv.take<float>(gram_slab_n);
    w->G = cv.take<double>((size_t)KP * KP);
    w->alpha = cv.take<double>(K);
    w->u = cv.take<double>(K);
    return cv.off;
  };
  const int rc = grow_ws(c, lay(nullptr));
  if (rc) return rc;
  lay(c->ws);
  return GM_OK;
}

inline KState* host_state(gm_ctx* c) { return reinterpret_cast<KState*>(c->host); }
inline KState* host_lagged(gm_ctx* c) { return host_state(c) + 1; }
constexpr size_t kHostNoiseOff = align_up(3 * sizeof(KState), 256);
inline float* host_noise_stage(gm_ctx* c) { return reinterpret_cast<float*>(c->host + kHostNoiseOff); }
template <class T>
inline T* host_after_states(gm_ctx* c, int64_t P = 1) {
  return reinterpret_cast<T*>(c->host + sizeof(KState) * P);
}

inline int ensure_host(gm_ctx* c, size_t bytes) {
  if (bytes <= c->host_bytes) return GM_OK;
  if (c->host) HIPCHK(hipHostFree(c->host));
  c->host = nullptr;
  c->host_bytes = 0;
  HIPCHK(hipHostMalloc(&c->host, bytes, hipHostMallocDefault));
  c->host_bytes = bytes;
  return GM_OK;
}


inline int allreduce(gm_ctx* c, double* buf, int64_t n, hipStream_t s) {
  if (c->comm) {
    ncclResult_t r = ncclAllReduce(buf, buf, (size_t)n, ncclDouble, ncclSum, c->comm, s);
    if (r != ncclSuccess) return fail(GM_ERR_COMM, "ncclAllReduce: %s", ncclGetErrorString(r));
    return GM_OK;
  }
  if (c->ar_fn) {
    if (c->ar_fn(c->ar_user, buf, n, (void*)s) != 0)
      return fail(GM_ERR_CALLBACK, "all-reduce callback failed");
  }
  return GM_OK;
}

inline int record_pass_begin(gm_ctx* c, hipStream_t s, hipEvent_t* e0, hipEvent_t* e1) {
  *e0 = *e1 = nullptr;
  if (!c->timing) return GM_OK;
  for (int i = 0; i < 2; ++i) {
    hipEvent_t e;
    if (!c->ev_free.empty()) {
      e = c->ev_free.back();
      c->ev_free.pop_back();
    } else {
      HIPCHK(hipEventCreate(&e));
    }
    (i == 0 ? *e0 : *e1) = e;
  }
  HIPCHK(hipEventRecord(*e0, s));
  return GM_OK;
}

inline int record_pass_end(gm_ctx* c, hipStream_t s, hipEvent_t e0, hipEvent_t e1) {
  if (!c->timing) return GM_OK;
  HIPCHK(hipEventRecord(e1, s));
  c->ev_used.emplace_back(e0, e1);
  return GM_OK;
}

inline void drop_last_timing(gm_ctx* c) {
  if (!c->timing || c->ev_used.empty()) return;
  c->ev_free.push_back(c->ev_used.back().first);
  c->ev_free.push_back(c->ev_used.back().second);
  c->ev_used.pop_back();
}


inline bool pick_cfg(int64_t K, int V, int64_t ldx, PassCfg* cfg, bool panel = false,
                     bool b16 = false) {
  int nw = 16, lpr, r, occ = 1;
  if (K <= 16) { lpr = 64; r = 1; }
  else if (K <= 32) { lpr = 64; r = 2; }
  else if (K <= 64) { if (panel) { nw = 8; lpr = 32; r = 4; } else { lpr = 64; r = 4; } }
  else if (K <= 128) { lpr = 64; r = 8; }
  else if (K <= 256) { if (panel) { lpr = 16; r = 4; } else { lpr = 32; r = 8; } }
  else if (K <= 512) { lpr = 16; r = 8; }
  else if (K <= 1024) { nw = 8; lpr = 8; r = 16; occ = 2; }
  else if (K <= 2048) { lpr = 4; r = 8; }
  else return false;
  if (const char* e = getenv("GMAGG_PASS_CFG")) {
    int a = 0, b = 0, c2 = 0, o = 1;
    const int n = sscanf(e, "%d,%d,%d,%d", &a, &b, &c2, &o);
    if (n >= 3 && b > 0 && (int64_t)a * (64 / b) * c2 >= K) {
      nw = a; lpr = b; r = c2; occ = n == 4 ? o : 1;
    }
  }
  if ((uint64_t)(64 / lpr) * (uint64_t)ldx * 4u >= (1ull << 31)) return false;
  *cfg = PassCfg{V, nw, lpr, r, occ, b16};
  return pass_cfg_supported(*cfg);
}

inline PassCfg light_cfg(int64_t K, const PassCfg& step) {
  if (getenv("GMAGG_PASS_CFG") || step.V != 4 || K <= 128 || K > 256) return step;
  const PassCfg c{4, 16, 64, 16, 1};
  return pass_cfg_supported(c) ? c : step;
}

inline int pick_vec(const float* X, int64_t d, int64_t ldx) {
  const uintptr_t p = reinterpret_cast<uintptr_t>(X);
  if (d % 4 == 0 && ldx % 4 == 0 && p % 16 == 0) return 4;
  if (d % 2 == 0 && ldx % 2 == 0 && p % 8 == 0) return 2;
  return 1;
}

inline int chunk_pair(const gm_ctx* c, const PassCfg& cfg, int64_t grid) {
  static const bool off = env_int("GMAGG_CHUNK_PAIR", 1) == 0;
  return !off && cfg.OCC == 2 && grid == 2 * (int64_t)c->num_cu ? c->num_cu : 0;
}


inline bool stage_enabled() {
  static const bool on = env_int("GMAGG_STAGE_PANELS", 1) != 0;
  return on;
}

inline bool ensure_stage(gm_ctx* c, size_t bytes) {
  if (bytes <= c->stage_bytes) return true;
  if (c->stage) (void)hipFree(c->stage);
  c->stage = nullptr;
  c->stage_bytes = 0;
  if (hipMalloc(&c->stage, bytes) != hipSuccess) {
    (void)hipGetLastError();
    c->stage = nullptr;
    return false;
  }
  c->stage_bytes = bytes;
  return true;
}


struct PreOma {
  bool pending;
  float* X;
  int64_t K, d, ldx, d_total, col_off;
  bool panels;
  float sd;
  uint64_t seed;
  hipStream_t s;
  int64_t P = 1, ldp = 0;
  int apply() {
    if (!pending) return GM_OK;
    pending = false;
    const int wshift = panels ? wshift_of(gm_panel_width(K)) : 0;
    HIPCHK(launch_oma_philox(X, K, d, ldx, d_total, col_off, sd, seed, s, wshift, P,
                             P > 1 ? ldp : 0));
    return GM_OK;
  }
};

struct StreamPasses {
  gm_ctx* c;
  hipStream_t s;
  PassArgs a;
  bool twopass;
  PassCfg cfg[2];
  int mode[2], nb[2];
  int problems;
  double* sums;
  int64_t sums_ps;
  bool pair;
  PreOma* oma;
};

inline int stream_pass(const StreamPasses& p, int64_t t, const float* g_old, int64_t gold_ps,
                       float* g_new) {
  const bool init = t < 0;
  const PassCfg& cfg = p.cfg[init];
  const int nb = p.nb[init];
  int mode = p.mode[init];
  PassArgs a = p.a;
  a.g_old = g_old; a.gold_ps = gold_ps; a.g_new = g_new;
  a.slab_stride = init ? 2 * a.K + 2 : a.K + 2;
  a.iter = t;
  a.chunk_pair = p.pair ? chunk_pair(p.c, cfg, nb) : 0;
  if (init && p.oma->pending) {
    if (!p.twopass && cfg.V == 4 && mode == 1 && a.col_off % 4 == 0) {
      mode = 4;
      a.oma_sd = p.oma->sd;
      a.oma_seed = p.oma->seed;
      p.oma->pending = false;
    } else {
      const int rco = p.oma->apply();
      if (rco) return rco;
    }
  }
  hipEvent_t e0, e1;
  int rc = init ? GM_OK : record_pass_begin(p.c, p.s, &e0, &e1);
  if (rc) return rc;
  if (p.twopass)
    HIPCHK(launch_twopass(init, a.X, a.K, a.d, a.ldx, g_old, g_new, a.coef, a.st, a.noise,
                          a.hnoise, a.seed, t, a.col_off, a.slab, nb, p.sums, p.s));
  else
    HIPCHK(launch_pass(cfg, mode, nb, a, p.s, p.problems));
  if (!init) { rc = record_pass_end(p.c, p.s, e0, e1); if (rc) return rc; }
  if (!p.twopass)
    HIPCHK(launch_slab_reduce(a.slab, nb, a.slab_stride, p.sums, a.st, p.s, p.problems,
                              p.sums_ps));
  return GM_OK;
}

int run_resident_batched(gm_ctx* c, const float* X, int64_t P, int64_t K, int64_t d,
                         int64_t ldx, int64_t ldp, bool panels, int64_t Wp, const float* guess0,
                         int64_t ldg, float* out, int64_t ldo, const gm_opts* o,
                         gm_result* results, hipStream_t s, bool res_ok);

}
```

byzantine_aircomp_amd/csrc/host_weiszfeld.hip:

```cpp
#include <cstring>

#include "host_ctx.h"

using namespace gmh;

namespace {

struct CallTraits {
  bool sharded;
  int64_t d_total, col_off;
  bool host_noise;
  bool collective;
};

CallTraits traits_of(const gm_ctx* c, int64_t d) {
  CallTraits tr{};
  tr.sharded = c->d_total > 0;
  tr.d_total = tr.sharded ? c->d_total : d;
  tr.col_off = tr.sharded ? c->d_offset : 0;
  tr.collective = tr.sharded || c->comm || c->ar_fn;
  return tr;
}

enum class Rule { Gm2, Gm, Cclip };

struct StreamJob {
  const void* X;
  int64_t K, d, ldx;
  bool panels;
  PassCfg cfg;
  int algo;
  const float* guess0;
  float* out;
  Rule rule;
  double tau;
  int64_t maxiter;
  double tol, eps;
  int check_every;
  AirNoise air;
  gm_noise_cb noise_cb;
  void* noise_user;
  CallTraits tr;
  PreOma oma;
  hipStream_t s;
  bool guard_rejected;
};

int upload_draws(gm_ctx* c, const StreamJob& j, const Workspace& w, int64_t it) {
  const int64_t K = j.K, d = j.d;
  hipStream_t s = j.s;
  float* h_hr = host_noise_stage(c);
  float* h_hi = h_hr + K;
  float* h_n = h_hi + K;
  if (j.noise_cb(j.noise_user, it, h_hr, h_hi, j.air.has_noise ? h_n : nullptr) != 0)
    return fail(GM_ERR_CALLBACK, "noise callback failed at iteration %lld", (long long)it);
  HIPCHK(hipMemcpyAsync(w.h_re, h_hr, sizeof(float) * K, hipMemcpyHostToDevice, s));
  HIPCHK(hipMemcpyAsync(w.h_im, h_hi, sizeof(float) * K, hipMemcpyHostToDevice, s));
  if (j.air.has_noise) {
    const float* n_cols = h_n + j.tr.col_off;
    HIPCHK(hipMemcpyAsync(w.hnoise, n_cols, sizeof(float) * d, hipMemcpyHostToDevice, s));
    HIPCHK(hipMemcpyAsync(w.hnoise + d, h_n + j.tr.d_total, sizeof(float), hipMemcpyHostToDevice,
                          s));
  }
  return GM_OK;
}

int run_resident(gm_ctx* c, const float* X, int64_t K, int64_t d, int64_t ldx,
                 const float* guess0, float* out, const gm_opts* o, gm_result* res,
                 const PassCfg& cfg, int cpb, int nb, hipStream_t s, bool* timed_out,
                 int64_t pstride = 0, int wshift = 0) {
  *timed_out = false;
  const size_t words = resident_gran_words(K, cfg, nb);
  const int64_t S = 2 * K + 2;
  Workspace w;
  int rc = ensure_ws(c, K, d, (int)((words + S - 1) / S), &w);
  if (rc) return rc;
  rc = ensure_host(c, sizeof(KState));
  if (rc) return rc;
  unsigned* bar = reinterpret_cast<unsigned*>(w.sums);
  HIPCHK(hipMemsetAsync(w.st, 0, sizeof(KState), s));
  HIPCHK(hipMemsetAsync(bar, 0, 16, s));
  HIPCHK(hipMemsetAsync(w.slab, 0, align_up(words * 8, 16), s));
  ResArgs a{};
  a.X = X; a.K = K; a.d = d; a.ldx = ldx; a.guess0 = guess0; a.out = out;
  a.pstride = pstride; a.wshift = wshift;
  a.maxiter = o->maxiter; a.tol = (float)o->tol; a.eps = (float)o->eps;
  a.mode = o->mode; a.has_noise = aircomp_noise(o);
  a.P_max = o->P_max; a.noise_sd = noise_sd(o);
  a.seed = o->seed;
  a.gran = reinterpret_cast<unsigned long long*>(w.slab);
  a.checkin = a.gran + (size_t)2 * nb * S;
  a.need = checkin_need((unsigned)nb);
  a.stride = res_xcd_stride(nb, c->num_cu);
  const int hm = res_hier_mode();
  a.hier = a.stride == 1 && nb > 8 && 2 * K + 2 <= cfg.NW * 64 &&
           (hm == 2 || (hm == 1 && nb >= 90 && K > 32)) && resident_has_exchange(cfg, cpb, 1);
  a.local = (a.stride == 8 || a.hier) && res_xcd_mode() == 2;
  a.lvl2 = a.checkin + nb + 1;
  a.split = a.stride == 1 && !a.hier && nb > 8 && res_xcd_mode() == 2 && res_split_mode() != 0 &&
            resident_has_exchange(cfg, cpb, 2);
  a.granL = a.lvl2 + (size_t)32 * (2 * K + 2);
  a.bar = bar; a.st = w.st;
  hipEvent_t e0, e1;
  rc = record_pass_begin(c, s, &e0, &e1);
  if (rc) return rc;
  HIPCHK(launch_resident(cfg, cpb, nb * (int)a.stride, a, s));
  rc = record_pass_end(c, s, e0, e1);
  if (rc) return rc;
  KState* hst = host_state(c);
  HIPCHK(hipMemcpyAsync(hst, w.st, sizeof(KState), hipMemcpyDeviceToHost, s));
  unsigned hbar[4] = {0, 0, 0, 0};
  HIPCHK(hipMemcpyAsync(hbar, bar, 16, hipMemcpyDeviceToHost, s));
  HIPCHK(hipStreamSynchronize(s));
  static const bool verbose = getenv("GMAGG_RES_VERBOSE") != nullptr;
  if (verbose)
    fprintf(stderr, "gmagg resident: nb=%d stride=%u local=%d (requested %d) timed_out=%u\n", nb,
            a.stride, hbar[0] ? (int)hbar[0] - 1 : -1, a.local, hbar[2]);
  if (hbar[2]) {
    *timed_out = true;
    if (!hbar[3]) c->res_skip = kResSkipAfterCheckinFail;
    drop_last_timing(c);
    return GM_OK;
  }
  gm_result r = result_from(*hst, GM_ALGO_RESIDENT);
  r.exchange = a.hier ? GM_EXCHANGE_XCD_HIER
               : hbar[0] != 2 ? GM_EXCHANGE_AGENT
               : a.split ? GM_EXCHANGE_XCD_SPLIT : GM_EXCHANGE_XCD_LOCAL;
  if (res) *res = r;
  return GM_OK;
}

int run_gram(gm_ctx* c, const float* X, int64_t K, int64_t d, int64_t ldx, const float* guess0,
             float* out, const gm_opts* o, gm_result* res, const PassCfg& cfg, hipStream_t s,
             bool split, bool guarded, bool* rejected, int64_t pstride = 0) {
  *rejected = false;
  int wshift = 0;
  if (pstride) {
    const int W = cfg.LPR * cfg.V;
    wshift = wshift_of(W);
    if ((1 << wshift) != W || W % 64 || !split) return fail(GM_ERR_UNSUPPORTED, "Gram on panels: W=%d", W);
  }
  const int KT = gram_kt(K), KP = 32 * KT;
  const char* kind_env = getenv("GMAGG_GRAM_KIND");
  const bool force_bf16 = kind_env && strcmp(kind_env, "bf16") == 0;
  GramKind kind = !split ? GramKind::F32 : (force_bf16 && !pstride) ? GramKind::BF16 : GramKind::H16;
  GramGrid gg = gram_grid(d, kind, c->num_cu);
  const GramGrid gb = gram_grid(d, GramKind::BF16, c->num_cu);
  const size_t slab_n = std::max(gram_slab_floats(KT, gg),
                                 kind == GramKind::H16 ? gram_slab_floats(KT, gb) : 0);
  const PassCfg ccfg = (guarded || pstride) ? cfg : light_cfg(K, cfg);
  const int J = ccfg.LPR * ccfg.V;
  const int nb_p = (int)std::max<int64_t>(
      1, std::min<int64_t>((d + J - 1) / J,
                           (int64_t)c->num_cu * pass_blocks_per_cu(ccfg, guarded ? 0 : 3)));
  Workspace w;
  int rc = ensure_ws(c, K, d, nb_p, &w, slab_n, KP);
  if (rc) return rc;
  rc = ensure_host(c, sizeof(KState) + 4 * sizeof(double));
  if (rc) return rc;
  KState* hst = host_state(c);
  double* hsums = host_after_states<double>(c);
  float* p = w.g[1];
  HIPCHK(hipMemcpyAsync(p, guess0, sizeof(float) * d, hipMemcpyDeviceToDevice, s));
again:
  HIPCHK(hipMemsetAsync(w.st, 0, sizeof(KState), s));
  hipEvent_t e0, e1;
  rc = record_pass_begin(c, s, &e0, &e1);
  if (rc) return rc;
  HIPCHK(launch_gram(X, K, d, ldx, p, kind, gg, w.gslab, w.G, w.st, s, pstride, wshift));
  rc = record_pass_end(c, s, e0, e1);
  if (rc) return rc;
  rc = allreduce(c, w.G, (int64_t)KP * KP, s);
  if (rc) return rc;
  HIPCHK(launch_gram_check(w.G, KP, w.st, s));
  HIPCHK(launch_gram_solve(w.G, KP, K, o->maxiter, (float)o->tol, (float)o->eps, w.alpha, w.u,
                           w.coef, w.st, s));
  const int64_t S = guarded ? K + 2 : 2;
  PassArgs a{};
  a.X = X; a.K = K; a.d = d; a.ldx = pstride ? pstride : ldx;
  a.g_old = p; a.g_new = out; a.coef = w.coef; a.st = w.st;
  a.slab = w.slab; a.slab_stride = S;
  a.panel_stride = pstride;
  HIPCHK(launch_pass(ccfg, guarded ? 0 : 3, nb_p, a, s));
  HIPCHK(launch_slab_reduce(w.slab, nb_p, S, w.sums, w.st, s));
  rc = allreduce(c, w.sums, S, s);
  if (rc) return rc;
  if (guarded)
    HIPCHK(launch_gram_verify(w.G, KP, K, (float)o->eps, w.u, w.alpha, w.sums, w.r, w.st, s));
  HIPCHK(hipMemcpyAsync(hst, w.st, sizeof(KState), hipMemcpyDeviceToHost, s));
  HIPCHK(hipMemcpyAsync(hsums, w.sums + (S - 2), 2 * sizeof(double), hipMemcpyDeviceToHost, s));
  HIPCHK(hipStreamSynchronize(s));
  if (hst->gram_bad && kind == GramKind::H16) {
    if (pstride) {
      *rejected = true;
      return GM_OK;
    }
    kind = GramKind::BF16;
    gg = gb;
    goto again;
  }
  bool floor_band = false;
  if (guarded) {
    const double u = std::ldexp(1.0, -24);
    const double gn = std::sqrt(std::max(0.0, hsums[1]));
    double rho = hst->guard_r;
    rho = rho != rho ? 0.5 : std::min(0.95, std::max(0.5, rho));
    const double pred = hst->guard_q / (1.0 - rho) / gn;
    const bool accurate = pred <= 1e-6;
    const double floor = kFloorUlps * u * gn;
    const bool floor_ok = !hst->converged || floor <= o->tol;
    floor_band = hst->converged && floor > o->tol / 3.0;
    static const bool dbg = getenv("GMAGG_GUARD_DEBUG") != nullptr;
    if (dbg)
      fprintf(stderr, "[gram guard] K=%lld d=%lld q=%.3e rho=%.3f |g|=%.4e pred=%.3e converged=%d "
              "iters=%d floor_ok=%d band=%d accurate=%d\n", (long long)K, (long long)d, hst->guard_q,
              rho, gn, pred, (int)hst->converged, (int)hst->iters, (int)floor_ok, (int)floor_band,
              (int)accurate);
    if (!accurate || !floor_ok) {
      *rejected = true;
      return GM_OK;
    }
  }
  gm_result r = result_from(*hst, split ? GM_ALGO_GRAM : GM_ALGO_GRAM_F32);
  r.gram_kind = kind == GramKind::H16 ? 1 : kind == GramKind::BF16 ? 2 : 3;
  r.guard = !guarded ? GM_GUARD_NONE : floor_band ? GM_GUARD_ACCEPTED_FLOOR : GM_GUARD_ACCEPTED;
  if (res) *res = r;
  return GM_OK;
}

void stream_grids(const gm_ctx* c, int64_t K, int64_t d, int algo, const PassCfg& cfg,
                  const PassCfg& cfg_i, int init_mode, int step_mode, int* nb_step, int* nb_init) {
  if (algo != GM_ALGO_STREAM) {
    *nb_step = *nb_init = twopass_blocks(K, d, c->num_cu);
    return;
  }
  const int J = cfg.LPR * cfg.V, Ji = cfg_i.LPR * cfg_i.V;
  const int64_t nch = (d + J - 1) / J, nchi = (d + Ji - 1) / Ji;
  const int64_t cap_s = (int64_t)c->num_cu * pass_blocks_per_cu(cfg, step_mode);
  const int64_t cap_i = (int64_t)c->num_cu * pass_blocks_per_cu(cfg_i, init_mode);
  *nb_step = (int)std::max<int64_t>(1, std::min(nch, cap_s));
  *nb_init = (int)std::max<int64_t>(1, std::min(nchi, cap_i));
}

int run_stream(gm_ctx* c, StreamJob& j, gm_result* res, KState* final_state = nullptr) {
  const int64_t K = j.K, d = j.d;
  hipStream_t s = j.s;
  const bool host_noise = j.tr.host_noise;
  const int64_t d_total = j.tr.d_total;
  const bool cclip = j.rule == Rule::Cclip, air = j.rule == Rule::Gm;
  const int init_mode = air ? 2 : 1;
  const int step_mode = cclip ? kPassStepSelf : 0;
  const int noise_kind = cclip ? 3 : !j.air.has_noise ? 0 : (host_noise ? 2 : 1);
  const int kmode = cclip ? kModeCclip : air ? GM_MODE_AIRCOMP : GM_MODE_IDEAL;

  StreamPasses sp{c, s};
  sp.twopass = j.algo != GM_ALGO_STREAM;
  sp.cfg[0] = j.cfg;
  sp.cfg[1] = j.panels ? j.cfg : light_cfg(K, j.cfg);
  sp.mode[0] = step_mode;
  sp.mode[1] = init_mode;
  stream_grids(c, K, d, j.algo, sp.cfg[0], sp.cfg[1], init_mode, step_mode, &sp.nb[0], &sp.nb[1]);
  const int nb = std::max(sp.nb[0], sp.nb[1]);
  Workspace w;
  int rc = ensure_ws(c, K, d, nb, &w);
  if (rc) return rc;
  rc = ensure_host(c, kHostNoiseOff + sizeof(float) * (2 * K + d_total + 1) + 256);
  if (rc) return rc;
  KState* hst = host_state(c);
  KState* hslot = host_lagged(c);
  HIPCHK(hipMemsetAsync(w.st, 0, sizeof(KState), s));

  sp.a.X = static_cast<const float*>(j.X);
  sp.a.K = K; sp.a.d = d; sp.a.ldx = j.ldx;
  sp.a.coef = w.coef; sp.a.st = w.st; sp.a.slab = w.slab;
  sp.a.noise = noise_kind; sp.a.hnoise = w.hnoise; sp.a.seed = j.air.seed;
  sp.a.col_off = j.tr.col_off;
  sp.a.panel_stride = j.panels ? j.ldx : 0;
  sp.problems = 1;
  sp.sums = w.sums;
  sp.pair = !j.panels;
  sp.oma = &j.oma;

  KspaceArgs ka = kspace_args(K, d_total, kmode, j.tol, j.eps, j.air);
  ka.tau = j.tau;
  ka.noise_src = host_noise ? 1 : 0;
  ka.sums = w.sums;
  ka.r = w.r;
  ka.h_re = w.h_re;
  ka.h_im = w.h_im;
  ka.n_last = w.hnoise + d;
  ka.coef = w.coef;
  ka.st = w.st;

  auto poll = [&](KState* dst) -> int {
    HIPCHK(hipMemcpyAsync(dst, w.st, sizeof(KState), hipMemcpyDeviceToHost, s));
    HIPCHK(hipStreamSynchronize(s));
    return GM_OK;
  };

  auto do_pass = [&](int64_t t) -> int {
    const int rc2 = t <= 0 ? stream_pass(sp, t, j.guess0, 0, t < 0 ? nullptr : w.g[0])
                           : stream_pass(sp, t, w.g[(t - 1) & 1], 0, w.g[t & 1]);
    return rc2 ? rc2 : allreduce(c, w.sums, t < 0 ? 2 * K + 2 : K + 2, s);
  };

  rc = do_pass(-1);
  if (rc) return rc;
  ka.t = -1;
  ka.do_check = 0;
  if (host_noise) { rc = upload_draws(c, j, w, 0); if (rc) return rc; }
  ka.do_coef = 1;
  HIPCHK(launch_kspace(ka, s));

  int check_every = j.check_every;
  if (check_every <= 0) check_every = (K * d_total >= (int64_t)1 << 24) ? 1 : 16;
  if (host_noise) check_every = 1;
  static const bool no_lag = getenv("GMAGG_NO_LAG") != nullptr;
  const bool lagged = check_every == 1 && !host_noise && !no_lag;
  if (lagged)
    for (auto& e : c->poll_ev)
      if (!e) HIPCHK(hipEventCreateWithFlags(&e, hipEventDisableTiming));
  int64_t pending = -1;

  int64_t t = 0, enqueued = 0;
  const KState* final_st = nullptr;
  for (; t < j.maxiter; ++t) {
    rc = do_pass(t);
    if (rc) return rc;
    enqueued = t + 1;
    const bool last = t + 1 == j.maxiter;
    ka.t = t;
    if (host_noise) {
      ka.do_check = 1;
      ka.do_coef = 0;
      HIPCHK(launch_kspace(ka, s));
      rc = poll(hst);
      if (rc) return rc;
      if (hst->done || last) break;
      rc = upload_draws(c, j, w, t + 1);
      if (rc) return rc;
      ka.do_check = 0;
      ka.do_coef = 1;
      HIPCHK(launch_kspace(ka, s));
      continue;
    }
    ka.do_check = 1;
    ka.do_coef = last ? 0 : 1;
    ka.mirror = lagged && !last ? &hslot[t & 1] : nullptr;
    HIPCHK(launch_kspace(ka, s));
    ka.mirror = nullptr;
    if (lagged && !last) {
      HIPCHK(hipEventRecord(c->poll_ev[t & 1], s));
      if (pending >= 0) {
        HIPCHK(hipEventSynchronize(c->poll_ev[pending & 1]));
        if (hslot[pending & 1].done) {
          final_st = &hslot[pending & 1];
          break;
        }
      }
      pending = t;
      continue;
    }
    if (last || (t + 1) % check_every == 0) {
      rc = poll(hst);
      if (rc) return rc;
      if (hst->done) break;
    }
  }
  if (!final_st) {
    rc = poll(hst);
    if (rc) return rc;
    final_st = hst;
  }
  gm_result r = result_from(*final_st, j.algo);
  r.guard = j.guard_rejected ? GM_GUARD_REJECTED : GM_GUARD_NONE;
  if (r.iters < 1) return fail(GM_ERR_HIP, "Weiszfeld loop recorded no iteration");
  for (int64_t k = r.iters; k < enqueued; ++k) drop_last_timing(c);
  HIPCHK(hipMemcpyAsync(j.out, w.g[(r.iters - 1) & 1], sizeof(float) * d, hipMemcpyDeviceToDevice,
                        s));
  if (res) *res = r;
  if (final_state) *final_state = *final_st;
  return GM_OK;
}

struct Call {
  gm_ctx* c;
  const float* X;
  StreamJob j;
  const gm_opts* o;
  gm_result* res;
  bool res_ok;
};

int try_gram(Call& q, int64_t ldx, const PassCfg& cfg, bool split, bool guarded,
             int64_t pstride = 0) {
  bool rejected = false;
  int rc = q.j.oma.apply();
  if (rc) return rc;
  rc = run_gram(q.c, q.X, q.j.K, q.j.d, ldx, q.j.guess0, q.j.out, q.o, q.res, cfg, q.j.s, split,
                guarded, &rejected, pstride);
  if (rc || !rejected) return rc;
  q.j.guard_rejected = true;
  return kDeclined;
}

bool panel_cfg(int64_t K, int64_t W, PassCfg* cfg) {
  return W != 0 && pick_cfg(K, 4, W, cfg, true) && cfg->LPR * cfg->V == W;
}

int check_panels(const char* who, const void* X, int64_t K, int64_t W, int64_t ldx, int elem) {
  if (ldx < K * W || (reinterpret_cast<uintptr_t>(X) & 15) || (elem == 2 && ldx % 8) ||
      K * W * elem > 0x7fffffff)
    return fail(GM_ERR_INVALID, "%s: panel layout: need panel stride >= K*W (%lld)%s, 16-byte "
                "aligned X, K*W*%d < 2^31 (ldx=%lld)", who, (long long)(K * W),
                elem == 2 ? " and a multiple of 8" : "", elem, (long long)ldx);
  return GM_OK;
}

int f32_panel_tile(const char* who, const float* X, int64_t K, int64_t ldx, PassCfg* cfg) {
  const int64_t W = gm_panel_width(K);
  if (!panel_cfg(K, W, cfg))
    return fail(GM_ERR_UNSUPPORTED, "%s: panel layout: no streaming tile of width %lld for "
                "K=%lld", who, (long long)W, (long long)K);
  return check_panels(who, X, K, W, ldx, 4);
}

int select_panels(Call& q, PassCfg* cfg) {
  gm_ctx* c = q.c;
  const gm_opts* o = q.o;
  const int64_t K = q.j.K, d = q.j.d, ldx = q.j.ldx;
  const int64_t W = gm_panel_width(K);
  const int rcp = f32_panel_tile("gm_weiszfeld_f32", q.X, K, ldx, cfg);
  if (rcp) return rcp;
  const bool gram_ok = o->mode == GM_MODE_IDEAL && gram_kt(K) > 0 && W % 64 == 0 &&
                       (W & (W - 1)) == 0;
  if ((q.j.algo == GM_ALGO_AUTO && gram_ok && q.j.tr.d_total >= (int64_t)1 << 18) ||
      (q.j.algo == GM_ALGO_GRAM && gram_ok)) {
    static const bool unguarded = getenv("GMAGG_GRAM_UNGUARDED") != nullptr;
    const int rc0 = try_gram(q, W, *cfg, true, q.j.algo == GM_ALGO_AUTO || !unguarded, ldx);
    if (rc0 != kDeclined) return rc0;
    q.j.algo = GM_ALGO_STREAM;
  }
  auto wants_resident = [&] {
    return (q.j.algo == GM_ALGO_AUTO || q.j.algo == GM_ALGO_RESIDENT) && !q.j.tr.collective;
  };
  if (wants_resident() && !q.j.tr.host_noise && K <= 64 && q.res_ok) {
    PassCfg rcfg{};
    int cpb = 0, nbr = 0;
    if (pick_cfg(K, 2, W, &rcfg) && W % rcfg.V == 0 && (resident_tile(&rcfg, K), true) &&
        resident_plan(rcfg, (d + rcfg.LPR * rcfg.V - 1) / (rcfg.LPR * rcfg.V), c->num_cu, &cpb,
                      &nbr) &&
        res_xcd_stride(nbr, c->num_cu) == 8) {
      bool timed_out = false;
      int rco = q.j.oma.apply();
      if (rco) return rco;
      const int rc0 = run_resident(c, q.X, K, d, K * W, q.j.guess0, q.j.out, o, q.res, rcfg, cpb,
                                   nbr, q.j.s, &timed_out, ldx, wshift_of(W));
      if (rc0 || !timed_out) return rc0;
      q.j.algo = GM_ALGO_STREAM;
    }
  }
  if (wants_resident()) {
    const int rc0 = run_resident_batched(c, q.X, 1, K, d, ldx, (d + W - 1) / W * ldx, true, W,
                                         q.j.guess0, d, q.j.out, d, o, q.res, q.j.s, q.res_ok);
    if (rc0 != kDeclined) return rc0;
  }
  if (q.j.algo == GM_ALGO_AUTO) q.j.algo = GM_ALGO_STREAM;
  if (q.j.algo != GM_ALGO_STREAM)
    return fail(GM_ERR_UNSUPPORTED, "panel layout: streaming, (gm2, K <= 256) Gram or (K <= 52 "
                "gm2 / K <= 50 gm, unsharded) resident only (algo %d)", q.j.algo);
  return kDeclined;
}

int rows_gram_auto(Call& q, int V) {
  const int64_t K = q.j.K, ldx = q.j.ldx, d_total = q.j.tr.d_total;
  PassCfg cfg{};
  const bool local_ok = gram_kt(K) > 0 && V == 4 && ldx < ((int64_t)1 << 26) &&
                        pick_cfg(K, V, ldx, &cfg);
  const bool take = q.j.algo == GM_ALGO_AUTO && q.o->mode == GM_MODE_IDEAL && gram_kt(K) > 0 &&
                    d_total >= (int64_t)1 << 18 && (q.j.tr.sharded ? d_total % 4 == 0 : local_ok);
  if (!take) return kDeclined;
  if (!local_ok)
    return fail(GM_ERR_INVALID, "sharded gm2 (AUTO -> Gram, d_total=%lld): this rank's shard "
                "must be 16-byte aligned with d_local %% 4 == 0 and ldx %% 4 == 0 like every "
                "other rank's (use sharded.shard_range + contiguous shards)",
                (long long)d_total);
  return try_gram(q, ldx, cfg, true, true);
}

int rows_resident(Call& q, int V) {
  gm_ctx* c = q.c;
  PassCfg cfg{};
  if (!((q.j.algo == GM_ALGO_AUTO || q.j.algo == GM_ALGO_RESIDENT) && !q.j.tr.host_noise &&
        !q.j.tr.collective && pick_cfg(q.j.K, V, q.j.ldx, &cfg)))
    return kDeclined;
  resident_tile(&cfg, q.j.K);
  const int J = cfg.LPR * cfg.V;
  const int64_t nch = (q.j.d + J - 1) / J;
  int cpb = 0, nbr = 0;
  if (!(q.res_ok && resident_plan(cfg, nch, c->num_cu, &cpb, &nbr))) return kDeclined;
  bool timed_out = false;
  int rco = q.j.oma.apply();
  if (rco) return rco;
  const int rc0 = run_resident(c, q.X, q.j.K, q.j.d, q.j.ldx, q.j.guess0, q.j.out, q.o, q.res, cfg,
                               cpb, nbr, q.j.s, &timed_out);
  if (rc0 || !timed_out) return rc0;
  if (q.j.algo == GM_ALGO_RESIDENT) q.j.algo = GM_ALGO_AUTO;
  return kDeclined;
}

int rows_staged(Call& q) {
  gm_ctx* c = q.c;
  const gm_opts* o = q.o;
  const int64_t K = q.j.K, d = q.j.d;
  if (!(q.j.algo == GM_ALGO_AUTO && aircomp_noise(o) && !q.j.tr.host_noise &&
        o->maxiter >= 64 && K * d >= ((int64_t)1 << 24)))
    return kDeclined;
  const int64_t W = gm_panel_width(K);
  PassCfg pcfg{};
  if (!stage_enabled() || W <= 0 || K * W * 4 > 0x7fffffff || !panel_cfg(K, W, &pcfg) ||
      !ensure_stage(c, sizeof(float) * (size_t)((d + W - 1) / W) * (size_t)(K * W)))
    return kDeclined;
  HIPCHK(launch_rows_to_panels(q.X, K, d, q.j.ldx, c->stage, W, K * W, q.j.s));
  StreamJob staged = q.j;
  staged.X = c->stage;
  staged.ldx = K * W;
  staged.panels = true;
  staged.cfg = pcfg;
  staged.algo = GM_ALGO_STREAM;
  return run_stream(c, staged, q.res);
}

int rows_gram_explicit(Call& q, int V, PassCfg* cfg) {
  const gm_opts* o = q.o;
  const int64_t K = q.j.K, d = q.j.d, ldx = q.j.ldx;
  if (o->mode != GM_MODE_IDEAL)
    return fail(GM_ERR_UNSUPPORTED, "Gram variant is gm2 only (AirComp noise leaves span(X))");
  if (gram_kt(K) == 0 || V != 4 || !pick_cfg(K, V, ldx, cfg))
    return fail(GM_ERR_UNSUPPORTED, "Gram variant needs K <= 256, d and ldx multiples of 4, "
                "16-byte aligned X (K=%lld d=%lld ldx=%lld)", (long long)K, (long long)d,
                (long long)ldx);
  const bool split = q.j.algo == GM_ALGO_GRAM && ldx < ((int64_t)1 << 26);
  static const bool unguarded = getenv("GMAGG_GRAM_UNGUARDED") != nullptr;
  const int rc0 = try_gram(q, ldx, *cfg, split, !unguarded);
  if (rc0 == kDeclined) q.j.algo = GM_ALGO_STREAM;
  return rc0;
}

int select_rows(Call& q, PassCfg* cfg) {
  const int V = pick_vec(q.X, q.j.d, q.j.ldx);
  int rc = rows_gram_auto(q, V);
  if (rc != kDeclined) return rc;
  rc = rows_resident(q, V);
  if (rc != kDeclined) return rc;
  if (q.j.algo == GM_ALGO_RESIDENT)
    return fail(GM_ERR_UNSUPPORTED, "resident kernel: problem too large, sharded or host noise");
  rc = rows_staged(q);
  if (rc != kDeclined) return rc;
  if (q.j.algo == GM_ALGO_AUTO || q.j.algo == GM_ALGO_STREAM) {
    if (pick_cfg(q.j.K, V, q.j.ldx, cfg)) q.j.algo = GM_ALGO_STREAM;
    else if (q.j.algo == GM_ALGO_STREAM)
      return fail(GM_ERR_UNSUPPORTED, "streaming pass supports K <= 2048 (K=%lld)",
                  (long long)q.j.K);
    else q.j.algo = GM_ALGO_TWOPASS;
  }
  if (q.j.algo == GM_ALGO_GRAM || q.j.algo == GM_ALGO_GRAM_F32) {
    rc = rows_gram_explicit(q, V, cfg);
    if (rc != kDeclined) return rc;
  }
  if (q.j.algo != GM_ALGO_STREAM && q.j.algo != GM_ALGO_TWOPASS)
    return fail(GM_ERR_INVALID, "unknown algo %d", q.o->algo);
  return kDeclined;
}


template <class Opts>
int begin_call(const char* who, gm_ctx* c, const void* X, int64_t K, int64_t d, int64_t ldx,
               const float* guess0, float* out, const Opts* o, void* stream, StreamJob* j) {
  if (!c || !o || !out || !guess0 || !X) return fail(GM_ERR_INVALID, "%s: NULL argument", who);
  if (o->layout != GM_LAYOUT_ROWS && o->layout != GM_LAYOUT_PANELS)
    return fail(GM_ERR_INVALID, "%s: unknown layout %d", who, o->layout);
  if (K < 1 || d < 1 || (ldx < d && o->layout == GM_LAYOUT_ROWS))
    return fail(GM_ERR_INVALID, "%s: bad shape K=%lld d=%lld ldx=%lld", who, (long long)K,
                (long long)d, (long long)ldx);
  if (o->maxiter < 0) return fail(GM_ERR_INVALID, "%s: maxiter < 0", who);
  *j = StreamJob{};
  j->X = X; j->K = K; j->d = d; j->ldx = ldx;
  j->panels = o->layout == GM_LAYOUT_PANELS;
  j->algo = GM_ALGO_STREAM;
  j->guess0 = guess0;
  j->out = out;
  j->maxiter = o->maxiter;
  j->tol = o->tol;
  j->check_every = o->check_every;
  j->tr = traits_of(c, d);
  j->s = reinterpret_cast<hipStream_t>(stream);
  return GM_OK;
}

int gm_rule(const char* who, const gm_opts* o, StreamJob* j) {
  if (o->mode != GM_MODE_IDEAL && o->mode != GM_MODE_AIRCOMP)
    return fail(GM_ERR_INVALID, "%s: unknown mode %d", who, o->mode);
  if (o->mode == GM_MODE_AIRCOMP && o->noise_source == GM_NOISE_HOST && !o->noise_cb)
    return fail(GM_ERR_INVALID, "%s: GM_NOISE_HOST needs noise_cb", who);
  j->rule = o->mode == GM_MODE_AIRCOMP ? Rule::Gm : Rule::Gm2;
  j->eps = o->eps;
  j->air = air_noise(o);
  j->noise_cb = o->noise_cb;
  j->noise_user = o->noise_user;
  j->tr.host_noise = o->mode == GM_MODE_AIRCOMP && o->noise_source == GM_NOISE_HOST;
  return GM_OK;
}

int cclip_rule(const char* who, const gm_cclip_opts* o, StreamJob* j) {
  if (!(o->tau > 0.0))
    return fail(GM_ERR_INVALID, "%s: tau must be > 0 (+inf allowed; got %g)", who, o->tau);
  j->rule = Rule::Cclip;
  j->tau = o->tau;
  return GM_OK;
}

int bf16_refuse_collective(const gm_ctx* c, const char* who) {
  if (c->d_total > 0 || c->comm || c->ar_fn)
    return fail(GM_ERR_UNSUPPORTED, "%s: sharded / collective contexts are not supported", who);
  return GM_OK;
}

int bf16_tile(const char* who, StreamJob* j) {
  const int64_t K = j->K, d = j->d, ldx = j->ldx;
  if (!pick_cfg(K, 8, ldx, &j->cfg, j->panels, true))
    return fail(GM_ERR_UNSUPPORTED, "%s: no streaming tile for K=%lld (K <= 2048) at ldx=%lld",
                who, (long long)K, (long long)ldx);
  if (j->panels) return check_panels(who, j->X, K, (int64_t)j->cfg.LPR * j->cfg.V, ldx, 2);
  if ((reinterpret_cast<uintptr_t>(j->X) & 15) || ldx % 8 || d % 8)
    return fail(GM_ERR_UNSUPPORTED, "%s: row-major bf16 needs 16-byte aligned X with d and ldx "
                "multiples of 8 (d=%lld ldx=%lld); pack panels (gm_rows_to_panels_bf16)", who,
                (long long)d, (long long)ldx);
  return GM_OK;
}

template <class Res>
int no_iteration(StreamJob& j, Res* res) {
  const int rc = j.oma.apply();
  if (rc) return rc;
  HIPCHK(hipMemcpyAsync(j.out, j.guess0, sizeof(float) * j.d, hipMemcpyDeviceToDevice, j.s));
  if (res) {
    *res = Res{};
    res->last_movement = NAN;
  }
  return GM_OK;
}

int run_cclip(gm_ctx* c, StreamJob& j, gm_cclip_result* res) {
  gm_result r{};
  KState fin{};
  const int rc = run_stream(c, j, &r, &fin);
  if (rc || !res) return rc;
  res->iters = r.iters;
  res->last_movement = r.last_movement;
  res->converged = r.converged;
  res->clipped = fin.clipped;
  return GM_OK;
}

}

extern "C" int gm_cclip_f32(gm_ctx* c, const float* X, int64_t K, int64_t d, int64_t ldx,
                            const float* guess0, float* out, const gm_cclip_opts* o,
                            gm_cclip_result* res, void* stream) {
  static const char* const who = "gm_cclip_f32";
  StreamJob j;
  int rc = begin_call(who, c, X, K, d, ldx, guess0, out, o, stream, &j);
  if (!rc) rc = cclip_rule(who, o, &j);
  if (rc) return rc;
  WsOrder order(c, j.s);
  HIPCHK(order.err);
  if (j.maxiter == 0) return no_iteration(j, res);
  if (j.panels) {
    rc = f32_panel_tile(who, X, K, ldx, &j.cfg);
    if (rc) return rc;
// ... 74 lines not shown
```

byzantine_aircomp_amd/csrc/stream_pass.hip:

```cpp
#include "stream_pass_kernel.h"

namespace gmk {


int pass_variant() {
  static const int v = [] {
    const char* e = getenv("GMAGG_PASS_VARIANT");
    return e ? atoi(e) : -1;
  }();
  return v;
}

template <int V, int NW, int LPR, int R, int MODE, int OCC>
static const void* pass_fn(bool panel) {
  constexpr bool kRollDefault = MODE == 0;
  constexpr bool kRollPanel = kRollDefault || MODE == 1 || MODE == 2;
  if constexpr (V == 4) {
    if (panel) {
      const int pv = pass_variant();
      if (pv == 3)
        return reinterpret_cast<const void*>(&weiszfeld_pass<V, NW, LPR, R, MODE, 3, OCC, true>);
      if (pv == 2 || (pv < 0 && kRollPanel))
        return reinterpret_cast<const void*>(&weiszfeld_pass<V, NW, LPR, R, MODE, 2, OCC, true>);
      return reinterpret_cast<const void*>(&weiszfeld_pass<V, NW, LPR, R, MODE, 0, OCC, true>);
    }
  } else if (panel) {
    return nullptr;
  }
#ifdef GMK_PIPE_VARIANT
  if (pass_variant() == 1)
    return reinterpret_cast<const void*>(&weiszfeld_pass<V, NW, LPR, R, MODE, 1, OCC>);
#endif
  if (pass_variant() == 2 || (pass_variant() < 0 && kRollDefault && V == 4))
    return reinterpret_cast<const void*>(&weiszfeld_pass<V, NW, LPR, R, MODE, 2, OCC>);
  return reinterpret_cast<const void*>(&weiszfeld_pass<V, NW, LPR, R, MODE, 0, OCC>);
}

template <int V, int NW, int LPR, int R, int OCC>
static const void* pass_fn_mode(int mode, bool panel) {
  switch (mode) {
    case 0: return pass_fn<V, NW, LPR, R, 0, OCC>(panel);
    case 1: return pass_fn<V, NW, LPR, R, 1, OCC>(panel);
    case 2: return pass_fn<V, NW, LPR, R, 2, OCC>(panel);
    case 4:
      if constexpr (V == 4) return pass_fn<V, NW, LPR, R, 4, OCC>(panel);
      else return nullptr;
    default: return pass_fn<V, NW, LPR, R, 3, OCC>(panel);
  }
}

static const void* pass_kernel(const PassCfg& cfg, int mode, bool panel = false) {
  if (cfg.B16) return pass_kernel_bf16(cfg, mode, panel);
  if (mode == kPassStepSelf) return pass_kernel_self(cfg, panel);
#define GMK_CASE(V_, W_, L_, R_, O_)                                                 \
  if (cfg.V == V_ && cfg.NW == W_ && cfg.LPR == L_ && cfg.R == R_ && cfg.OCC == O_) \
    return pass_fn_mode<V_, W_, L_, R_, O_>(mode, panel);
  GMK_FOR_EACH_CFG(GMK_CASE, 4)
  GMK_FOR_EACH_CFG(GMK_CASE, 2)
  GMK_FOR_EACH_CFG(GMK_CASE, 1)
#undef GMK_CASE
  return nullptr;
}

bool pass_cfg_supported(const PassCfg& cfg) { return pass_kernel(cfg, 0) != nullptr; }

hipError_t launch_pass(const PassCfg& cfg, int mode, int grid, const PassArgs& a, hipStream_t s,
                       int problems) {
  if (problems == 1 && cfg.V == 4 && cfg.NW == 8 && cfg.LPR == 8 && cfg.R == 16 && cfg.OCC == 2 &&
      rows_pass_eligible(a, mode))
    return launch_rows_pass(mode, grid, a, s);
  const void* fn = pass_kernel(cfg, mode, a.panel_stride > 0);
  if (!fn) return hipErrorInvalidValue;
  void* args[] = {const_cast<PassArgs*>(&a)};
  return hipLaunchKernel(fn, dim3(grid, problems), dim3(cfg.NW * 64), args, 0, s);
}

int pass_blocks_per_cu(const PassCfg& cfg, int mode) {
  const void* fn = pass_kernel(cfg, mode);
  int n = 0;
  if (!fn || hipOccupancyMaxActiveBlocksPerMultiprocessor(&n, fn, cfg.NW * 64, 0) != hipSuccess ||
      n < 1)
    return 1;
  return n;
}

}
```

byzantine_aircomp_amd/csrc/stream_pass_bf16.hip:

```cpp
#include "stream_pass_kernel.h"

namespace gmk {

template <int NW, int LPR, int R, int OCC, int MODE, bool SELF = false>
static const void* pass_fn_bf16(bool panel) {
  const int pv = pass_variant();
  constexpr bool kRollSpills = OCC > 1 || (MODE == 2 && R >= 8) ||
                               (MODE == 0 && LPR == 16 && R == 8);
  const bool roll = pv == 2 || (pv != 0 && (panel || MODE == 0) && !kRollSpills);
  if (panel)
    return roll ? reinterpret_cast<const void*>(&weiszfeld_pass<8, NW, LPR, R, MODE, 2, OCC, true, true, SELF>)
                : reinterpret_cast<const void*>(&weiszfeld_pass<8, NW, LPR, R, MODE, 0, OCC, true, true, SELF>);
  return roll ? reinterpret_cast<const void*>(&weiszfeld_pass<8, NW, LPR, R, MODE, 2, OCC, false, true, SELF>)
              : reinterpret_cast<const void*>(&weiszfeld_pass<8, NW, LPR, R, MODE, 0, OCC, false, true, SELF>);
}

#define GMK_FOR_EACH_BF16_CFG(X_)                                                         \
  X_(16, 64, 1, 1) X_(16, 64, 2, 1) X_(16, 64, 4, 1) X_(8, 32, 4, 1) X_(16, 64, 8, 1)     \
  X_(16, 32, 8, 1) X_(16, 16, 4, 1) X_(16, 16, 8, 1) X_(8, 8, 16, 2) X_(16, 4, 8, 1)

const void* pass_kernel_bf16(const PassCfg& cfg, int mode, bool panel) {
  if (!cfg.B16 || cfg.V != 8) return nullptr;
#define GMK_CASE(W_, L_, R_, O_)                                                     \
  if (cfg.NW == W_ && cfg.LPR == L_ && cfg.R == R_ && cfg.OCC == O_) {               \
    switch (mode) {                                                                  \
      case 0: return pass_fn_bf16<W_, L_, R_, O_, 0>(panel);                         \
      case 1: return pass_fn_bf16<W_, L_, R_, O_, 1>(panel);                         \
      case 2: return pass_fn_bf16<W_, L_, R_, O_, 2>(panel);                         \
      case kPassStepSelf: return pass_fn_bf16<W_, L_, R_, O_, 0, true>(panel);       \
      default: return nullptr;                                                       \
    }                                                                                \
  }
  GMK_FOR_EACH_BF16_CFG(GMK_CASE)
#undef GMK_CASE
  return nullptr;
}

}
```

byzantine_aircomp_amd/csrc/stream_pass_kernel.h:

```cpp
#pragma once
#include "device_util.h"
#include "gmagg_internal.h"
#include "philox.h"

#define GMK_FOR_EACH_CFG(X_, V_)                                                             \
  X_(V_, 16, 64, 1, 1) X_(V_, 16, 64, 2, 1) X_(V_, 16, 64, 4, 1) X_(V_, 16, 64, 8, 1)        \
  X_(V_, 16, 32, 8, 1) X_(V_, 16, 16, 8, 1) X_(V_, 16, 8, 8, 1) X_(V_, 16, 4, 8, 1)          \
  X_(V_, 16, 4, 4, 1) X_(V_, 16, 16, 4, 1) X_(V_, 8, 8, 16, 1) X_(V_, 8, 4, 8, 1)            \
  X_(V_, 8, 16, 8, 1) X_(V_, 8, 8, 8, 1) X_(V_, 4, 8, 8, 1) X_(V_, 4, 16, 4, 1)              \
  X_(V_, 8, 32, 4, 1) X_(V_, 16, 8, 8, 2) X_(V_, 16, 16, 16, 1) X_(V_, 8, 8, 16, 2)          \
  X_(V_, 8, 32, 4, 4)                                                                        \
  X_(V_, 16, 32, 8, 2) X_(V_, 16, 64, 4, 2) X_(V_, 16, 64, 16, 1) X_(V_, 8, 16, 8, 2)

namespace gmk {

template <int V, int R, bool B16 = false>
struct Tile {
  static_assert(!B16 || V == 8, "bf16 tiles: 8 columns = one 16-byte load per lane");
  typedef typename std::conditional<B16, uint32_t, float>::type word;
  word x[R][B16 ? V / 2 : V];
  float gold;
  float hn;
};

template <int V, int NW, int LPR, int R, int MODE, int SCHED, int OCC = 1, bool PANEL = false,
          bool B16 = false, bool SELF = false>
__global__ void __launch_bounds__(NW * 64, OCC * NW / 4) weiszfeld_pass(PassArgs a) {
  static_assert(!SELF || MODE == 0, "the old iterate as column term: STEP passes only");
  constexpr bool PIPE = SCHED == 1, ROLL = SCHED == 2 || SCHED == 3, ROLL2 = SCHED == 3;
  constexpr bool SUM_ONLY = MODE == 3;
  constexpr bool OMA_INIT = MODE == 4;
  constexpr bool INIT = MODE == 1 || MODE == 2 || OMA_INIT;
  constexpr bool WANT_R = MODE == 2;
  static_assert(!OMA_INIT || V == 4, "fused OMA: one Philox block per float4 group");
  static_assert(!B16 || (!SUM_ONLY && !OMA_INIT && !PIPE && !ROLL2), "bf16: modes 0-2, SCHED 0 / 2");
  constexpr int ES = B16 ? 2 : 4;
  constexpr int QW = 64 / LPR;
  constexpr int NRG = NW * QW;
  constexpr int J = LPR * V;
  constexpr int RPL = R > LPR ? R / LPR : 1;
  static_assert(J <= NW * 64, "one finisher thread per column");
  using T = Tile<V, R, B16>;

  typedef typename std::conditional<SELF, double, float>::type red_t;
  __shared__ red_t s_red[NW][J];
  __shared__ float s_g[INIT ? 2 : 1][J];
  __shared__ double s_fin[2][NW];
  __shared__ float s_w[OCC > 1 ? NW * QW * R : 1];

  if (gridDim.y > 1) {
    const int64_t pb = blockIdx.y;
    a.X += pb * a.x_ps;
    a.g_old += pb * a.gold_ps;
    if (a.g_new) a.g_new += pb * a.gnew_ps;
    a.coef += pb * a.K;
    a.st += pb;
    a.slab += pb * (int64_t)gridDim.x * a.slab_stride;
    a.seed += (uint64_t)pb * kSeedStride;
    a.oma_seed += (uint64_t)pb * kSeedStride;
  }
  if (!SUM_ONLY && a.st->done) return;

  const int tid = threadIdx.x, lane = tid & 63;
  const int w = __builtin_amdgcn_readfirstlane(tid >> 6);
  const int c = lane % LPR, q = lane / LPR;
  const int rg = w * QW + q;
  const int64_t K = a.K, d = a.d;
  const int64_t nch = (d + J - 1) / J;
  const int64_t grid = gridDim.x;

  bool rval[R];
#pragma unroll
  for (int i = 0; i < R; ++i) rval[i] = rg + (int64_t)NRG * i < K;
  typedef typename std::conditional<B16, uint16_t, float>::type elem;
  const elem* const Xe = reinterpret_cast<const elem*>(a.X);
  const elem* base[R];
#pragma unroll
  for (int i = 0; i < R; ++i) base[i] = Xe + (int64_t)(w * QW + NRG * i) * a.ldx;
  const uint32_t goff = (uint32_t)q * (uint32_t)a.ldx;
  const uint32_t poff = ((uint32_t)q * J + (uint32_t)(c * V)) * ES;

  float osc[OMA_INIT ? R : 1];
  if constexpr (OMA_INIT) {
#pragma unroll
    for (int i = 0; i < R; ++i)
      osc[i] = rval[i] ? oma_row_scale(a.oma_seed, (uint64_t)(rg + NRG * i), a.oma_sd) : 0.f;
  }
  float wt[OCC > 1 ? 1 : R];
  float a_noise = 0.f;
  if constexpr (!INIT) {
    if constexpr (OCC > 1) {
      for (int k = tid; k < NRG * R; k += NW * 64) s_w[k] = k < K ? a.coef[k] : 0.f;
      __syncthreads();
    } else {
#pragma unroll
      for (int i = 0; i < R; ++i) wt[i] = rval[i] ? a.coef[rg + NRG * i] : 0.f;
    }
    a_noise = a.st->a_noise;
  }

  typedef float f2 __attribute__((ext_vector_type(2)));
  auto xpair = [](const T& t, int i, int j) -> f2 {
    const uint32_t p = (uint32_t)t.x[i][j];
    return f2{__uint_as_float(p << 16), __uint_as_float(p & 0xffff0000u)};
  };
  auto zero_col = [](T& t, int i, int v) {
    if constexpr (B16) t.x[i][v >> 1] &= (v & 1) ? 0x0000ffffu : 0xffff0000u;
    else t.x[i][v] = 0.f;
  };
  auto fetch_row = [&](int64_t ch, T& t, int i) {
    if constexpr (PANEL) {
      constexpr int64_t GB = (int64_t)NRG * J * ES;
      const int64_t wb = (int64_t)(w * QW) * J * ES + i * GB;
      const int64_t nrec = (int64_t)K * J * ES - wb;
      const uint32_t vo = (ch < nch && ch * J + c * V < d) ? poff : 0x80000000u;
      load_rows<B16 ? 4 : V>(reinterpret_cast<const typename T::word*>(
                                 reinterpret_cast<const char*>(Xe + ch * a.panel_stride) + wb),
                             vo, t.x[i], nrec <= 0 ? 0 : nrec > 0x7fffffff ? 0x7fffffff : (int)nrec);
      if (!B16 && (ch + 1) * J > d) {
#pragma unroll
        for (int v = 0; v < V; ++v)
          if (ch * J + c * V + v >= d) zero_col(t, i, v);
      }
      return;
    }
    const int64_t col = ch * J + (int64_t)c * V;
    const bool cval = ch < nch && col < d;
    if (cval && rval[i]) {
      load_cols<B16 ? 4 : V>(reinterpret_cast<const typename T::word*>(
                                 base[i] + (goff + (uint32_t)col)), t.x[i]);
    } else {
#pragma unroll
      for (int v = 0; v < (B16 ? V / 2 : V); ++v) t.x[i][v] = 0;
    }
  };
  auto zero_padding = [&](int64_t ch, T& t) {
    if constexpr (B16 && PANEL) {
      if ((ch + 1) * J > d) {
#pragma unroll
        for (int i = 0; i < R; ++i)
#pragma unroll
          for (int v = 0; v < V; ++v)
            if (ch * J + c * V + v >= d) zero_col(t, i, v);
      }
    }
  };
  auto fetch_aux = [&](int64_t ch, T& t) {
    const int64_t gj = ch * J + tid;
    const bool fin = tid < J && ch < nch && gj < d;
    t.gold = fin ? a.g_old[gj] : 0.f;
    if constexpr (!INIT) t.hn = (fin && a.noise == 2) ? a.hnoise[gj] : 0.f;
  };
  auto fetch = [&](int64_t ch, T& t) {
#pragma unroll
    for (int i = 0; i < R; ++i) fetch_row(ch, t, i);
    fetch_aux(ch, t);
  };

  double row_acc[RPL], row_acc2[RPL];
#pragma unroll
  for (int m = 0; m < RPL; ++m) row_acc[m] = row_acc2[m] = 0.0;
  double mv_acc = 0.0, gn_acc = 0.0;

  int par = 0;
  auto oma_tile = [&](int64_t ch, auto& t) {
    const int64_t col = ch * J + (int64_t)c * V;
    if (ch >= nch || col >= d) return;
#pragma unroll
    for (int i = 0; i < R; ++i) {
      if (!rval[i]) continue;
      const int64_t k = rg + (int64_t)NRG * i;
      float z[4];
      normal4_hw(a.oma_seed, kStreamOmaNoise, (uint64_t)k, (uint64_t)(a.col_off + col) >> 2, z);
#pragma unroll
      for (int v = 0; v < V; ++v)
        if (col + v < d) t.x[i][v] = oma_noisy(t.x[i][v], osc[i], z[v]);
      float* dst;
      if constexpr (PANEL)
        dst = const_cast<float*>(a.X) + ch * a.panel_stride + k * J + c * V;
      else
        dst = reinterpret_cast<float*>(const_cast<elem*>(base[i])) + goff + col;
      if (col + V <= d) {
        typedef float f4 __attribute__((ext_vector_type(4)));
        *reinterpret_cast<f4*>(dst) = f4{t.x[i][0], t.x[i][1], t.x[i][2], t.x[i][3]};
      } else {
#pragma unroll
        for (int v = 0; v < V; ++v)
          if (col + v < d) dst[v] = t.x[i][v];
      }
    }
  };
  auto process = [&](int64_t ch, T& t, int64_t nxt) {
    float gv[V];
    zero_padding(ch, t);
    if constexpr (OMA_INIT) oma_tile(ch, t);
    if constexpr (INIT) {
      if (tid < J) {
        s_g[par][tid] = t.gold;
        gn_acc += (double)(t.gold * t.gold);
      }
      __syncthreads();
#pragma unroll
      for (int v = 0; v < V; ++v) gv[v] = s_g[par][c * V + v];
      par ^= 1;
    } else {
      float acc[V];
      f2 accp[B16 ? V / 2 : 1];
      red_t accd[SELF ? V : 1];
      if constexpr (SELF) {
#pragma unroll
        for (int v = 0; v < V; ++v) accd[v] = 0;
      }
#pragma unroll
      for (int v = 0; v < V; ++v) acc[v] = 0.f;
#pragma unroll
      for (int j = 0; j < (B16 ? V / 2 : 1); ++j) accp[j] = f2{0.f, 0.f};
#pragma unroll
      for (int i = 0; i < R; ++i) {
        float wi;
        if constexpr (OCC > 1) wi = s_w[rg + NRG * i];
        else wi = wt[i];
        if constexpr (B16) {
#pragma unroll
          for (int j = 0; j < V / 2; ++j) {
            const f2 xv = xpair(t, i, j);
            if constexpr (SELF) {
              accd[2 * j] = fma((double)wi, (double)xv[0], accd[2 * j]);
              accd[2 * j + 1] = fma((double)wi, (double)xv[1], accd[2 * j + 1]);
            } else {
              accp[j] = __builtin_elementwise_fma(f2{wi, wi}, xv, accp[j]);
            }
          }
        } else {
#pragma unroll
          for (int v = 0; v < V; ++v) {
            if constexpr (SELF) accd[v] = fma((double)wi, (double)t.x[i][v], accd[v]);
            else acc[v] = fmaf(wi, t.x[i][v], acc[v]);
          }
        }
      }
      if constexpr (B16) {
#pragma unroll
        for (int v = 0; v < V; ++v) acc[v] = accp[v >> 1][v & 1];
      }
#pragma unroll
      for (int o = LPR; o < 64; o <<= 1)
#pragma unroll
        for (int v = 0; v < V; ++v) {
          if constexpr (SELF) accd[v] += __shfl_xor(accd[v], o, 64);
          else acc[v] += __shfl_xor(acc[v], o, 64);
        }
      if (q == 0) {
#pragma unroll
        for (int v = 0; v < V; ++v) {
          if constexpr (SELF) s_red[w][c * V + v] = accd[v];
          else s_red[w][c * V + v] = acc[v];
        }
      }
      __syncthreads();
      if (tid < J) {
        red_t sum = 0;
#pragma unroll
        for (int ww = 0; ww < NW; ++ww) sum += s_red[ww][tid];
        const int64_t gj = ch * J + tid;
        float gnew = 0.f;
        if (gj < d) {
          if constexpr (!SELF) gnew = sum;
          if (a.noise == 1) {
            gnew = fmaf(a_noise, normal1(a.seed, kStreamNoise, a.iter, a.col_off + gj), gnew);
          } else if (a.noise == 2) {
            gnew = fmaf(a_noise, t.hn, gnew);
          }
          if constexpr (SELF) gnew = (float)fma((double)a_noise, (double)t.gold, (double)sum);
          a.g_new[gj] = gnew;
          const float diff = t.gold - gnew;
          mv_acc += (double)(diff * diff);
          gn_acc += (double)(gnew * gnew);
        }
        s_g[0][tid] = gnew;
      }
      __syncthreads();
#pragma unroll
      for (int v = 0; v < V; ++v) gv[v] = s_g[0][c * V + v];
    }
    if constexpr (SUM_ONLY) {
      if constexpr (ROLL) fetch(nxt, t);
      return;
    }
    if constexpr (B16 && !INIT) {
#pragma unroll
      for (int i = 0; i < R; ++i)
#pragma unroll
        for (int v = 0; v < V / 2; ++v) asm volatile("" : "+v"(t.x[i][v]));
    }
    float e[R], e2[WANT_R ? R : 1];
#pragma unroll
    for (int i = 0; i < R; ++i) {
      float s = 0.f, s2 = 0.f;
      if constexpr (B16) {
        f2 sp = f2{0.f, 0.f}, sp2 = f2{0.f, 0.f};
#pragma unroll
        for (int j = 0; j < V / 2; ++j) {
          const f2 xv = xpair(t, i, j);
          const f2 tt = xv - f2{gv[2 * j], gv[2 * j + 1]};
          sp = __builtin_elementwise_fma(tt, tt, sp);
          if constexpr (WANT_R) sp2 = __builtin_elementwise_fma(xv, xv, sp2);
        }
        s = sp[0] + sp[1];
        s2 = sp2[0] + sp2[1];
      } else {
#pragma unroll
        for (int v = 0; v < V; ++v) {
          const float tt = t.x[i][v] - gv[v];
          s = fmaf(tt, tt, s);
          if constexpr (WANT_R) s2 = fmaf(t.x[i][v], t.x[i][v], s2);
        }
      }
      e[i] = s;
      if constexpr (WANT_R) e2[i] = s2;
      if constexpr (ROLL) {
        __builtin_amdgcn_sched_barrier(0);
        asm volatile("" ::: "memory");
        fetch_row(nxt, t, i);
      }
    }
    if constexpr (ROLL) fetch_aux(nxt, t);
    transpose_reduce<LPR, R>(e, c);
#pragma unroll
    for (int m = 0; m < RPL; ++m) row_acc[m] += (double)e[m];
    if constexpr (WANT_R) {
      transpose_reduce<LPR, R>(e2, c);
#pragma unroll
      for (int m = 0; m < RPL; ++m) row_acc2[m] += (double)e2[m];
    }
  };

  if constexpr (PIPE) {
    T ta, tb;
    int64_t ch = blockIdx.x;
    fetch(ch, ta);
    for (; ch < nch; ch += 2 * grid) {
      fetch(ch + grid, tb);
      process(ch, ta, -1);
      if (ch + grid >= nch) break;
      fetch(ch + 2 * grid, ta);
      process(ch + grid, tb, -1);
    }
  } else if constexpr (ROLL2) {
    T ta, tb;
    int64_t ch = blockIdx.x;
    fetch(ch, ta);
    fetch(ch + grid, tb);
    for (; ch < nch; ch += 2 * grid) {
      process(ch, ta, ch + 2 * grid);
      if (ch + grid >= nch) break;
      process(ch + grid, tb, ch + 3 * grid);
    }
  } else if constexpr (ROLL) {
    T t;
    fetch(blockIdx.x, t);
    for (int64_t ch = blockIdx.x; ch < nch; ch += grid) process(ch, t, ch + grid);
  } else {
    for (int64_t ch = blockIdx.x; ch < nch; ch += grid) {
      T t;
      fetch(ch, t);
      process(ch, t, -1);
    }
  }

  double* out = a.slab + (int64_t)blockIdx.x * a.slab_stride;
  const int i_c = row_of_lane<LPR, R>(c);
  constexpr int SPAN = R < LPR ? LPR / R : 1;
  if (!SUM_ONLY && (c % SPAN) == 0) {
#pragma unroll
    for (int m = 0; m < RPL; ++m) {
      const int64_t k = rg + (int64_t)NRG * (i_c + m);
      if (k < K) {
        out[k] = row_acc[m];
        if constexpr (INIT) out[K + k] = row_acc2[m];
      }
    }
  }
  const double mv = wave_sum(mv_acc), gn = wave_sum(gn_acc);
  if (lane == 0) {
    s_fin[0][w] = mv;
    s_fin[1][w] = gn;
  }
  __syncthreads();
  if (tid == 0) {
    double m = 0.0, g = 0.0;
#pragma unroll
    for (int ww = 0; ww < NW; ++ww) {
      m += s_fin[0][ww];
      g += s_fin[1][ww];
    }
    const int64_t b = SUM_ONLY ? 0 : INIT ? 2 * K : K;
    out[b] = m;
    out[b + 1] = g;
  }
}

}
```

byzantine_aircomp_amd/csrc/weiszfeld.hip:

```cpp
#include "device_util.h"
#include "gmagg_internal.h"
#include "philox.h"

namespace gmk {

__global__ void __launch_bounds__(1024) slab_reduce(const double* __restrict__ slab, int nb,
                                                    int64_t S, double* __restrict__ sums,
                                                    const KState* st, int64_t sums_ps) {
  const int64_t pb = blockIdx.y;
  st += pb;
  slab += pb * nb * S;
  sums += pb * sums_ps;
  if (st->done) return;
  __shared__ double red[32][33];
  const int cx = threadIdx.x & 31, by = threadIdx.x >> 5;
  const int64_t j = (int64_t)blockIdx.x * 32 + cx;
  double acc = 0.0;
  if (j < S) {
    constexpr int U = 16;
    for (int b0 = by; b0 < nb; b0 += 32 * U) {
      double v[U];
#pragma unroll
      for (int u = 0; u < U; ++u) {
        const int b = b0 + 32 * u;
        v[u] = b < nb ? slab[(int64_t)b * S + j] : 0.0;
      }
#pragma unroll
      for (int u = 0; u < U; ++u)
        if (b0 + 32 * u < nb) acc += v[u];
    }
  }
  red[by][cx] = acc;
  __syncthreads();
  if (by == 0 && j < S) {
    double s = 0.0;
#pragma unroll
    for (int y = 0; y < 32; ++y) s += red[y][cx];
    sums[j] = s;
  }
}

__device__ void kspace_body(KspaceArgs& a);

__global__ void __launch_bounds__(1024) kspace_step(KspaceArgs a) {
  kspace_body(a);
  if (a.mirror && threadIdx.x == 0 && gridDim.x == 1) *a.mirror = *a.st;
}

__device__ void kspace_body(KspaceArgs& a) {
  if (gridDim.x > 1) {
    const int64_t pb = blockIdx.x;
    a.sums += pb * a.sums_ps;
    a.r += pb * a.K;
    a.coef += pb * a.K;
    a.st += pb;
    a.seed += (uint64_t)pb * kSeedStride;
  }
  KState* st = a.st;
  if (st->done) return;
  __shared__ double scratch[16];
  __shared__ int s_stop;
  const int tid = threadIdx.x;
  const int64_t K = a.K;
  const bool init = a.t < 0;
  const double* D2 = a.sums;
  const double gn2 = init ? a.sums[2 * K + 1] : a.sums[K + 1];

  if (tid == 0) {
    s_stop = 0;
    if (a.do_check && !init) {
      const float mv = (float)sqrt(a.sums[K]);
      st->last_movement = (double)mv;
      st->iters = a.t + 1;
      if (mv <= a.tol) {
        st->done = 1;
        st->converged = 1;
        s_stop = 1;
        if (a.n_done) atomicAdd(a.n_done, 1);
      }
    }
  }
  if (init && a.mode == 1)
    for (int64_t k = tid; k < K; k += blockDim.x) a.r[k] = a.sums[K + k];
  __syncthreads();
  if (s_stop || !a.do_coef) return;

  if (a.mode == 0) {
    double wsum = 0.0;
    for (int64_t k = tid; k < K; k += blockDim.x) wsum += 1.0 / (double)clamp_dist(D2[k], a.eps);
    const double W = block_sum(wsum, scratch);
    for (int64_t k = tid; k < K; k += blockDim.x)
      a.coef[k] = (float)((1.0 / (double)clamp_dist(D2[k], a.eps)) / W);
    return;
  }

  if (a.mode == kModeCclip) {
    double csum = 0.0, nclip = 0.0;
    for (int64_t k = tid; k < K; k += blockDim.x) {
      const double dist = sqrt(D2[k]);
      const double lam = dist <= a.tau ? 1.0 : a.tau / dist;
      const float ck = (float)(lam / (double)K);
      a.coef[k] = ck;
      csum += (double)ck;
      nclip += dist > a.tau ? 1.0 : 0.0;
    }
    const double C = block_sum(csum, scratch);
    const double N = block_sum(nclip, scratch);
    if (tid == 0) {
      st->a_noise = (float)(1.0 - C);
      st->clipped = (int32_t)N;
    }
    return;
  }

  const int64_t it = a.t + 1;
  const float s = sqrtf((float)(gn2 / (double)a.d_total));
  const float thr = (s * s) * 500.0f;
  const double s2 = (double)s * (double)s;
  double csum = 0.0;
  for (int64_t k = tid; k < K; k += blockDim.x) {
    float hr, hi;
    if (a.noise_src == 0) {
      float n[4];
      normal4(a.seed, kStreamChannel, (uint64_t)it, (uint64_t)k, n);
      hr = n[0] * 0.70710678118654752f;
      hi = n[1] * 0.70710678118654752f;
    } else {
      hr = a.h_re[k];
      hi = a.h_im[k];
    }
    const float h2 = hr * hr + hi * hi;
    const float dist = clamp_dist(D2[k], a.eps);
    const double dd = (double)dist;
    const double p = (a.r[k] + s2) / (dd * dd * (double)(a.d_total + 1)) / (double)h2;
    const double pup = p != p ? p : fmax(p, (double)thr);
    const double gain = sqrt(a.P_max / pup);
    const double ck = gain / dd;
    a.coef[k] = (float)ck;
    csum += ck;
  }
  const double Sc = block_sum(csum, scratch);
  double nd = 0.0;
  if (a.has_noise)
    nd = a.noise_src == 0
             ? a.noise_sd * (double)normal1(a.seed, kStreamNoise, (uint64_t)it, (uint64_t)a.d_total)
             : (double)a.n_last[0];
  const double yd = (double)s * Sc + nd;
  const double scale = (double)s / yd;
  __syncthreads();
  for (int64_t k = tid; k < K; k += blockDim.x) a.coef[k] = (float)((double)a.coef[k] * scale);
  if (tid == 0) {
    st->s = s;
    st->a_noise = a.has_noise ? (float)(scale * (a.noise_src == 0 ? a.noise_sd : 1.0)) : 0.f;
  }
}


__global__ void __launch_bounds__(256) twopass_sum(const float* __restrict__ X, int64_t K,
                                                   int64_t d, int64_t ldx,
                                                   const float* __restrict__ g_old,
                                                   float* __restrict__ g_new,
                                                   const float* __restrict__ coef,
                                                   const KState* st, int noise,
                                                   const float* __restrict__ hnoise,
                                                   uint64_t seed, int64_t iter, int64_t col_off,
                                                   double* slab) {
  if (st->done) return;
  __shared__ double scratch[16];
  double mv = 0.0, gn = 0.0;
  for (int64_t j = (int64_t)blockIdx.x * blockDim.x + threadIdx.x; j < d;
       j += (int64_t)gridDim.x * blockDim.x) {
    if (g_new == nullptr) {
      const float g = g_old[j];
      gn += (double)(g * g);
      continue;
    }
    float acc = 0.f;
    int64_t k = 0;
    for (; k + 8 <= K; k += 8) {
      float x[8];
#pragma unroll
      for (int u = 0; u < 8; ++u) x[u] = __builtin_nontemporal_load(X + (k + u) * ldx + j);
#pragma unroll
      for (int u = 0; u < 8; ++u) acc = fmaf(coef[k + u], x[u], acc);
    }
    for (; k < K; ++k) acc = fmaf(coef[k], X[k * ldx + j], acc);
    if (noise == 1) acc = fmaf(st->a_noise, normal1(seed, kStreamNoise, iter, col_off + j), acc);
    else if (noise == 2) acc = fmaf(st->a_noise, hnoise[j], acc);
    else if (noise == 3) acc = fmaf(st->a_noise, g_old[j], acc);
    g_new[j] = acc;
    const float diff = g_old[j] - acc;
    mv += (double)(diff * diff);
    gn += (double)(acc * acc);
  }
  const double m = block_sum(mv, scratch);
  const double g = block_sum(gn, scratch);
  if (threadIdx.x == 0) {
    slab[(int64_t)blockIdx.x * 2] = m;
    slab[(int64_t)blockIdx.x * 2 + 1] = g;
  }
}

__global__ void __launch_bounds__(256) twopass_dist(const float* __restrict__ X, int64_t K,
                                                    int64_t d, int64_t ldx,
                                                    const float* __restrict__ g, bool init,
                                                    const KState* st, double* sums) {
  if (st->done) return;
  __shared__ double scratch[16];
  const int64_t k = blockIdx.x;
  const float* row = X + k * ldx;
  double acc = 0.0, acc2 = 0.0;
  for (int64_t j = threadIdx.x; j < d; j += blockDim.x) {
    const float x = __builtin_nontemporal_load(row + j);
    const float t = x - g[j];
    acc += (double)(t * t);
    acc2 += (double)(x * x);
  }
  const double s1 = block_sum(acc, scratch);
  const double s2 = init ? block_sum(acc2, scratch) : 0.0;
  if (threadIdx.x == 0) {
    sums[k] = s1;
    if (init) sums[K + k] = s2;
  }
}

__global__ void __launch_bounds__(256) batched_finalize(const float* __restrict__ g0,
                                                        const float* __restrict__ g1, int64_t d,
                                                        const KState* st, float* out,
                                                        int64_t ldo) {
  const int64_t pb = blockIdx.y;
  const int64_t it = st[pb].iters;
  const float* src = ((it - 1) & 1) ? g1 : g0;
  for (int64_t j = (int64_t)blockIdx.x * blockDim.x + threadIdx.x; j < d;
       j += (int64_t)gridDim.x * blockDim.x)
    out[pb * ldo + j] = src[pb * d + j];
}

hipError_t launch_batched_finalize(const float* g0, const float* g1, int64_t d, int problems,
                                   const KState* st, float* out, int64_t ldo, hipStream_t s) {
  const int64_t bx = (d + 255) / 256;
  hipLaunchKernelGGL(batched_finalize, dim3((unsigned)(bx < 64 ? bx : 64), problems), dim3(256), 0,
                     s, g0, g1, d, st, out, ldo);
  return hipGetLastError();
}


hipError_t launch_slab_reduce(const double* slab, int nb, int64_t S, double* sums,
                              const KState* st, hipStream_t s, int problems, int64_t sums_ps) {
  const int grid = (int)((S + 31) / 32);
  hipLaunchKernelGGL(slab_reduce, dim3(grid, problems), dim3(1024), 0, s, slab, nb, S, sums, st,
                     sums_ps);
  return hipGetLastError();
}

hipError_t launch_kspace(const KspaceArgs& a, hipStream_t s, int problems) {
  const int threads = a.K >= 1024 ? 1024 : (int)((a.K + 63) / 64 * 64);
  hipLaunchKernelGGL(kspace_step, dim3(problems), dim3(threads), 0, s, a);
  return hipGetLastError();
}

int twopass_blocks(int64_t K, int64_t d, int num_cu) {
  (void)K;
  const int64_t want = (d + 255) / 256;
  const int64_t cap = (int64_t)num_cu * 8;
  return (int)(want < cap ? (want > 0 ? want : 1) : cap);
}

hipError_t launch_twopass(bool init, const float* X, int64_t K, int64_t d, int64_t ldx,
                          const float* g_old, float* g_new, const float* coef, const KState* st,
                          int noise, const float* hnoise, uint64_t seed, int64_t iter,
                          int64_t col_off, double* slab, int nb, double* sums, hipStream_t s) {
  const int64_t base = init ? 2 * K : K;
  hipLaunchKernelGGL(twopass_sum, dim3(nb), dim3(256), 0, s, X, K, d, ldx, g_old,
                     init ? nullptr : g_new, coef, st, noise, hnoise, seed, iter, col_off, slab);
  hipError_t e = hipGetLastError();
  if (e != hipSuccess) return e;
  hipLaunchKernelGGL(twopass_dist, dim3((unsigned)K), dim3(256), 0, s, X, K, d, ldx,
                     init ? g_old : g_new, init, st, sums);
  e = hipGetLastError();
  if (e != hipSuccess) return e;
  return launch_slab_reduce(slab, nb, 2, sums + base, st, s);
}

}
```

byzantine_aircomp_amd/sharded.py:

```python
from __future__ import annotations

import ctypes as C

import torch

from . import _lib
from .aggregators import (GMResult, Context, _cclip_params, _clip_centre, _clip_info, _clip_shape,
                          _clip_tau, _fltrust_info, _fltrust_server, _fltrust_shape, _fltrust_vec,
                          _gm_opts, _nnm_f, _noise_source, _result, _run_cclip, _run_clip,
                          _run_fltrust, _stream_ptr)
from .panels import ClientPanels

__all__ = ["shard_range", "ShardedGM", "torch_allreduce_adapter"]

ALIGN = 256


def shard_range(d: int, world: int, rank: int, align: int = ALIGN):
    if world < 1 or not 0 <= rank < world:
        raise ValueError(f"rank {rank} of {world}")
    per = -(-d // world)
    per = -(-per // align) * align
    lo = min(d, rank * per)
    return lo, min(d, lo + per)


def _wrap(ptr: int, count: int, device: torch.device) -> torch.Tensor:
    if device.type == "cpu":
        buf = (C.c_double * count).from_address(ptr)
        return torch.frombuffer(buf, dtype=torch.float64, count=count)

    class _Iface:
        __cuda_array_interface__ = {"shape": (count,), "typestr": "<f8", "data": (ptr, False),
                                    "version": 2, "strides": None}
    return torch.as_tensor(_Iface(), device=device)


def torch_allreduce_adapter(group=None, device: torch.device | None = None):
    import torch.distributed as dist

    def fn(ptr, count, stream):
        dev = device or torch.device("cpu")
        t = _wrap(ptr, count, dev)
        if dev.type == "cuda":
            s = torch.cuda.ExternalStream(stream, device=dev) if stream else torch.cuda.current_stream(dev)
            with torch.cuda.stream(s):
                dist.all_reduce(t, group=group)
        else:
            dist.all_reduce(t, group=group)
    return fn


def _aligned(shards, d_total: int) -> bool:
    if not all(0 <= lo <= hi <= d_total and lo % ALIGN == 0 and (hi % 4 == 0 or hi == d_total)
               for lo, hi in shards):
        return False
    if len(shards) == 1:
        return True
    end = 0
    for lo, hi in sorted(shards):
        if lo != end:
            return False
        end = hi
    return end == d_total


class ShardedGM:

    def __init__(self, d_total: int, group=None, device: torch.device | None = None,
                 transport: str = "rccl", shard: tuple[int, int] | None = None):
        import torch.distributed as dist
        self.group = group
        self.world = dist.get_world_size(group)
        self.rank = dist.get_rank(group)
        self.device = device or torch.device("cuda", torch.cuda.current_device())
        self.d_total = d_total
        if shard is None:
            self.lo, self.hi = shard_range(d_total, self.world, self.rank)
        else:
            self.lo, self.hi = int(shard[0]), int(shard[1])
            shards = [None] * self.world
            dist.all_gather_object(shards, (self.lo, self.hi), group=group)
            if not _aligned(shards, d_total):
                raise ValueError(f"shards {shards} of d_total={d_total}: each must be [lo, hi) "
                                 f"within [0, d_total) with lo % {ALIGN} == 0 and hi % 4 == 0 "
                                 "(or hi == d_total), tiling [0, d_total) at world size > 1")
        self.ctx = Context(self.device.index)
        self.ctx.set_shard(d_total, self.lo)
        if transport == "rccl":
            uid = [None]
            if self.rank == 0:
                buf = C.create_string_buffer(128)
                _lib.check(self.ctx.lib.gm_rccl_get_unique_id(buf), "gm_rccl_get_unique_id")
                uid[0] = buf.raw
            dist.broadcast_object_list(uid, src=dist.get_global_rank(group, 0) if group else 0,
                                       group=group)
            self.ctx.init_rccl(uid[0], self.world, self.rank)
        elif transport == "torch":
            self.ctx.set_allreduce(torch_allreduce_adapter(group, self.device))
        else:
            raise ValueError(f"transport must be 'rccl' or 'torch' (got {transport!r})")
        self.last_result: GMResult | None = None
        self.last_info: dict | None = None

    @property
    def d_local(self) -> int:
        return self.hi - self.lo

    def _run(self, X: torch.Tensor, options: dict, aircomp: bool) -> torch.Tensor:
        opts = {"maxiter": 200, "tol": 1e-5, "noise_var": None, "P_max": 1}
        opts.update(options or {})
        opts["check_every"] = 0
        X_in = X
        X, ptr, ldx, layout = self._operand(X)
        guess = opts.get("guess")
        if guess is None:
            raise ValueError("sharded aggregation needs options['guess'] (this rank's shard)")
        g0 = guess.to(device=self.device, dtype=torch.float32).contiguous()
        out = torch.empty(self.d_local, dtype=torch.float32, device=self.device)
        pre_var = None if aircomp else opts.get("pre_oma_var")
        if pre_var is not None and opts.get("pre_oma_seed") is None:
            raise ValueError("sharded pre-noise needs options['pre_oma_seed'] identical on "
                             "every rank")
        if aircomp:
            if _noise_source(opts) != _lib.GM_NOISE_PHILOX:
                raise ValueError("sharded AirComp uses on-device Philox noise")
            if opts.get("seed") is None:
                raise ValueError("sharded AirComp needs options['seed'] identical on every rank")
        o = _gm_opts(opts, aircomp, layout, pre_var, opts.get("pre_oma_seed"))
        res = _lib.GmResult()
        self.ctx.call("gm_weiszfeld_f32", ptr, X.shape[0], self.d_local, ldx, g0.data_ptr(),
                      out.data_ptr(), C.byref(o), C.byref(res), _stream_ptr(self.device))
        self.last_result = _result(res)
        if o.pre_oma and X is not X_in:
            X_in.copy_(X)
        return out

    def _operand(self, X):
        if X.shape[1] != self.d_local or X.device != self.device or X.dtype != torch.float32:
            raise ValueError(f"X must be fp32 [K, {self.d_local}] on {self.device}")
        if isinstance(X, ClientPanels):
            return X, X.data.data_ptr(), X.panel_stride, _lib.GM_LAYOUT_PANELS
        if X.stride(1) != 1 or X.data_ptr() % 16 or (X.stride(0) % 4 and X.shape[0] > 1):
            X = X.clone(memory_format=torch.contiguous_format)
        return X, X.data_ptr(), max(X.stride(0), self.d_local), _lib.GM_LAYOUT_ROWS

    def cclip(self, X, options):
        options = options or {}
        params = _cclip_params(options)
        guess = options.get("guess")
        if guess is None:
            raise ValueError("sharded aggregation needs options['guess'] (this rank's shard)")
        X, ptr, ldx, layout = self._operand(X)
        g0 = guess.to(device=self.device, dtype=torch.float32).contiguous()
        if g0.numel() != self.d_local:
            raise ValueError(f"guess has {g0.numel()} elements, this shard has {self.d_local}")
        out, self.last_result, self.last_clipped = _run_cclip(
            self.ctx, ptr, False, X.shape[0], self.d_local, ldx, layout, g0, params)
        return out

    def fltrust(self, X, options):
        options = options or {}
        K, _ = _fltrust_shape(X, "ShardedGM.fltrust")
        if X.dtype != torch.float32:
            raise TypeError(f"ShardedGM.fltrust reads fp32 shards (got {X.dtype})")
        su, row = _fltrust_server(options, K, self.d_local)
        guess = options.get("guess")
        if guess is not None and guess.numel() != self.d_local:
            raise ValueError(f"guess has {guess.numel()} elements, this shard has {self.d_local}")
        X, ptr, ldx, layout = self._operand(X)
        data = X.data if isinstance(X, ClientPanels) else X
        server = _fltrust_vec(su, self.d_local, self.device, "server_update")
        centre = _fltrust_vec(guess, self.d_local, self.device, "guess")
        out, stats = _run_fltrust(self.ctx, data, K, self.d_local, ldx, layout, server, row,
                                  centre)
        self.last_info = _fltrust_info(stats, K)
        return out

    def _clip(self, who, X, rule, f, tau, centre):
        K, _ = _clip_shape(X, who)
        if X.dtype != torch.float32:
            raise TypeError(f"{who} reads fp32 shards (got {X.dtype})")
        if rule == _lib.GM_CLIP_ARC:
            f, tau = _nnm_f(f, K, who), 0.0
        else:
            f, tau = 0, _clip_tau(tau, who)
        centre = _clip_centre(centre, self.d_local, who)
        X, ptr, ldx, layout = self._operand(X)
        panels = isinstance(X, ClientPanels)
        out, stats = _run_clip(self.ctx, X.data if panels else X, K, self.d_local, ldx, layout,
                               _fltrust_vec(centre, self.d_local, self.device, "centre"), rule, f,
                               tau, panels)
        self.last_info = _clip_info(stats, K)
        return out

    def arc(self, X, f, centre=None):
        return self._clip("ShardedGM.arc", X, _lib.GM_CLIP_ARC, f, None, centre)

    def clip(self, X, tau, centre=None):
        return self._clip("ShardedGM.clip", X, _lib.GM_CLIP_STATIC, None, tau, centre)

    def gm2(self, X, options=None):
        return self._run(X, options or {}, aircomp=False)

    def gm(self, X, options=None):
        return self._run(X, options or {}, aircomp=True)

    def close(self):
        self.ctx.close()
```

include/gmagg.h:

```cpp
#ifndef GMAGG_H
#define GMAGG_H

#include <stdint.h>

#ifdef __cplusplus
extern "C" {
#endif

#define GMAGG_ABI_VERSION 5

enum gm_status {
    GM_OK = 0,
    GM_ERR_INVALID = -1,
    GM_ERR_HIP = -2,
    GM_ERR_UNSUPPORTED = -3,
    GM_ERR_CALLBACK = -4,
    GM_ERR_COMM = -5
};

enum gm_mode {
    GM_MODE_IDEAL = 0,
    GM_MODE_AIRCOMP = 1
};

enum gm_noise_source {
    GM_NOISE_PHILOX = 0,
    GM_NOISE_HOST = 1
};

enum gm_layout {
    GM_LAYOUT_ROWS = 0,
    GM_LAYOUT_PANELS = 1
};

enum gm_algo {
    GM_ALGO_AUTO = 0,
    GM_ALGO_STREAM = 1,
    GM_ALGO_TWOPASS = 2,
    GM_ALGO_GRAM = 3,
    GM_ALGO_RESIDENT = 4,
    GM_ALGO_GRAM_F32 = 5
};

typedef int (*gm_noise_cb)(void* user, int64_t iter, float* h_re, float* h_im, float* noise);

typedef int (*gm_allreduce_cb)(void* user, double* dev_buf, int64_t count, void* stream);

typedef struct gm_opts {
    int64_t maxiter;
    double tol;
    double eps;
    int32_t mode;
    int32_t has_noise;
    double noise_var;
    double P_max;
    uint64_t seed;
    int32_t noise_source;
    int32_t algo;
    gm_noise_cb noise_cb;
    void* noise_user;
    int32_t check_every;
    int32_t layout;
    int32_t pre_oma;
    double pre_oma_var;
    uint64_t pre_oma_seed;
} gm_opts;

enum gm_guard {
    GM_GUARD_NONE = 0,
    GM_GUARD_ACCEPTED = 1,
    GM_GUARD_REJECTED = 2,
    GM_GUARD_ACCEPTED_FLOOR = 3
};

enum gm_exchange {
    GM_EXCHANGE_NONE = 0,
    GM_EXCHANGE_AGENT = 1,
    GM_EXCHANGE_XCD_LOCAL = 2,
    GM_EXCHANGE_XCD_HIER = 3,
    GM_EXCHANGE_XCD_SPLIT = 4
};

typedef struct gm_result {
    int64_t iters;
    double last_movement;
    int32_t converged;
    int32_t algo_used;
    int32_t guard;
    int32_t gram_kind;
    int32_t exchange;
} gm_result;

typedef struct gm_ctx gm_ctx;

int gm_ctx_create(int device, gm_ctx** out);
int gm_ctx_destroy(gm_ctx* ctx);

int gm_ctx_set_shard(gm_ctx* ctx, int64_t d_total, int64_t d_offset);
int gm_ctx_set_allreduce(gm_ctx* ctx, gm_allreduce_cb fn, void* user);
int gm_rccl_get_unique_id(void* unique_id_128);
int gm_ctx_init_rccl(gm_ctx* ctx, const void* unique_id_128, int nranks, int rank);

int gm_weiszfeld_f32(gm_ctx* ctx, const float* X, int64_t K, int64_t d, int64_t ldx,
                     const float* guess0, float* out, const gm_opts* opts,
                     gm_result* result, void* stream);

int64_t gm_panel_width(int64_t K);

int gm_weiszfeld_bf16(gm_ctx* ctx, const uint16_t* X, int64_t K, int64_t d, int64_t ldx,
                      const float* guess0, float* out, const gm_opts* opts,
                      gm_result* result, void* stream);

int64_t gm_panel_width_bf16(int64_t K);

typedef struct gm_cclip_opts {
    double tau;
    int64_t maxiter;
    double tol;
    int32_t layout;
    int32_t check_every;
} gm_cclip_opts;

typedef struct gm_cclip_result {
    int64_t iters;
    double last_movement;
    int32_t converged;
    int32_t clipped;
} gm_cclip_result;

int gm_cclip_f32(gm_ctx* ctx, const float* X, int64_t K, int64_t d, int64_t ldx,
                 const float* guess0, float* out, const gm_cclip_opts* opts,
                 gm_cclip_result* result, void* stream);
int gm_cclip_bf16(gm_ctx* ctx, const uint16_t* X, int64_t K, int64_t d, int64_t ldx,
                  const float* guess0, float* out, const gm_cclip_opts* opts,
                  gm_cclip_result* result, void* stream);

int gm_weiszfeld_batched_f32(gm_ctx* ctx, const float* X, int64_t P, int64_t K, int64_t d,
                             int64_t ldx, int64_t ldp, const float* guess0, int64_t ldg,
                             float* out, int64_t ldo, const gm_opts* opts, gm_result* results,
                             void* stream);

int gm_mean_f32(gm_ctx* ctx, const float* X, int64_t K, int64_t d, int64_t ldx, float* out,
                void* stream);
int gm_median_f32(gm_ctx* ctx, const float* X, int64_t K, int64_t d, int64_t ldx, float* out,
                  void* stream);
int gm_trimmed_mean_f32(gm_ctx* ctx, const float* X, int64_t K, int64_t d, int64_t ldx,
                        int64_t trim, float* out, void* stream);
int gm_krum_f32(gm_ctx* ctx, const float* X, int64_t K, int64_t d, int64_t ldx,
                int64_t honest_size, float* out, int64_t* index, void* stream);
int gm_mean_panels_f32(gm_ctx* ctx, const float* X, int64_t K, int64_t d, int64_t panel_stride,
                       float* out, void* stream);
int gm_median_panels_f32(gm_ctx* ctx, const float* X, int64_t K, int64_t d, int64_t panel_stride,
                         float* out, void* stream);
int gm_trimmed_mean_panels_f32(gm_ctx* ctx, const float* X, int64_t K, int64_t d,
                               int64_t panel_stride, int64_t trim, float* out, void* stream);
int gm_krum_panels_f32(gm_ctx* ctx, const float* X, int64_t K, int64_t d, int64_t panel_stride,
                       int64_t honest_size, float* out, int64_t* index, void* stream);

enum gm_krum_algo { GM_KRUM_EXACT = 0, GM_KRUM_GRAM = 1 };
enum gm_krum_reason {
  GM_KRUM_REASON_OK = 0,
  GM_KRUM_REASON_NOT_CHOSEN = 1,
  GM_KRUM_REASON_NOT_ELIGIBLE = 2,
  GM_KRUM_REASON_GRAM_NONFINITE = 3,
  GM_KRUM_REASON_CANDIDATES = 4
};
int gm_krum_last_info(gm_ctx* ctx, int64_t* info);

int gm_meamed_f32(gm_ctx* ctx, const float* X, int64_t K, int64_t d, int64_t ldx, int32_t layout,
                  const int32_t* rows, int64_t n_rows, int64_t keep, float* out, void* stream);
int gm_multi_krum_f32(gm_ctx* ctx, const float* X, int64_t K, int64_t d, int64_t ldx,
                      int32_t layout, int64_t honest, int64_t m, float* out, int32_t* selected,
                      void* stream);
int gm_bulyan_f32(gm_ctx* ctx, const float* X, int64_t K, int64_t d, int64_t ldx, int32_t layout,
                  int64_t honest, float* out, int32_t* selected, void* stream);

int gm_honest_variance_f32(gm_ctx* ctx, const float* X, int64_t honest, int64_t d, int64_t ldx,
                           float* out, void* stream);
int gm_honest_variance_panels_f32(gm_ctx* ctx, const float* X, int64_t K, int64_t honest,
                                  int64_t d, int64_t panel_stride, float* out, void* stream);

int gm_oma_philox_f32(gm_ctx* ctx, float* X, int64_t K, int64_t d, int64_t ldx,
                      double noise_var, uint64_t seed, void* stream);

int gm_oma_philox_batched_f32(gm_ctx* ctx, float* X, int64_t P, int64_t K, int64_t d, int64_t ldx,
                              int64_t pstride, double noise_var, uint64_t seed, void* stream);

int gm_oma_philox_batched_panels_f32(gm_ctx* ctx, float* X, int64_t P, int64_t K, int64_t d,
                                     int64_t panel_stride, int64_t pstride, double noise_var,
                                     uint64_t seed, void* stream);

int gm_oma_philox_panels_f32(gm_ctx* ctx, float* X, int64_t K, int64_t d, int64_t panel_stride,
                             double noise_var, uint64_t seed, void* stream);

int gm_rows_to_panels_f32(gm_ctx* ctx, const float* X, int64_t K, int64_t d, int64_t ldx,
                          float* P, int64_t W, int64_t panel_stride, void* stream);

int gm_rows_to_panels_bf16_from_f32(gm_ctx* ctx, const float* X, int64_t K, int64_t d,
                                    int64_t ldx, uint16_t* P, int64_t W, int64_t panel_stride,
                                    void* stream);
int gm_rows_to_panels_bf16(gm_ctx* ctx, const uint16_t* X, int64_t K, int64_t d, int64_t ldx,
                           uint16_t* P, int64_t W, int64_t panel_stride, void* stream);

int gm_bucket_means_f32 (gm_ctx* ctx, const float*    X, int64_t K, int64_t d, int64_t ldx,
                         int32_t layout_in, const int32_t* perm, int64_t s, float* Y, int64_t ldy,
                         int32_t layout_out, void* stream);
int gm_bucket_means_bf16(gm_ctx* ctx, const uint16_t* X, int64_t K, int64_t d, int64_t ldx,
                         int32_t layout_in, const int32_t* perm, int64_t s, float* Y, int64_t ldy,
                         int32_t layout_out, void* stream);

int gm_nnm_f32(gm_ctx* ctx, const float* X, int64_t K, int64_t d, int64_t ldx, int32_t layout_in,
               int64_t f, float* Y, int64_t ldy, int32_t layout_out, int32_t* neighbors,
               void* stream);

int gm_dnc_f32(gm_ctx* ctx, const float* X, int64_t K, int64_t d, int64_t ldx, int32_t layout,
               const int64_t* columns, int64_t n, int64_t iters, int64_t remove,
               int64_t power_iters, double power_tol, float* out, double* scores, int32_t* good,
               int64_t* n_good, int32_t* niter, int32_t* converged, void* stream);

int gm_fltrust_f32 (gm_ctx* ctx, const float*    X, int64_t K, int64_t d, int64_t ldx,
                    int32_t layout, const float* server, int64_t server_row, const float* centre,
                    float* out, double* stats, void* stream);
int gm_fltrust_bf16(gm_ctx* ctx, const uint16_t* X, int64_t K, int64_t d, int64_t ldx,
                    int32_t layout, const float* server, int64_t server_row, const float* centre,
                    float* out, double* stats, void* stream);

typedef enum gm_clip_rule {
    GM_CLIP_STATIC = 0,
    GM_CLIP_ARC = 1
} gm_clip_rule;
int gm_clip_rows_f32 (gm_ctx* ctx, const float*    X, int64_t K, int64_t d, int64_t ldx,
                      int32_t layout_in, const float* centre, int32_t rule, int64_t f, double tau,
                      float* Y, int64_t ldy, int32_t layout_out, double* stats, void* stream);
int gm_clip_rows_bf16(gm_ctx* ctx, const uint16_t* X, int64_t K, int64_t d, int64_t ldx,
                      int32_t layout_in, const float* centre, int32_t rule, int64_t f, double tau,
                      float* Y, int64_t ldy, int32_t layout_out, double* stats, void* stream);

int gm_attack_affine_f32 (gm_ctx* ctx, float*    X, int64_t K, int64_t d, int64_t ldx,
                          int32_t layout, int64_t byz, double a, double b, void* stream);
int gm_attack_affine_bf16(gm_ctx* ctx, uint16_t* X, int64_t K, int64_t d, int64_t ldx,
                          int32_t layout, int64_t byz, double a, double b, void* stream);
int gm_attack_minmax_f32 (gm_ctx* ctx, float* X, int64_t K, int64_t d, int64_t ldx, int32_t layout,
                          int64_t byz, int32_t rule, int32_t dev, double* gamma, void* stream);

int gm_client_chain_f32(gm_ctx* ctx, const float* data, int64_t ldd, const int64_t* labels,
                        int64_t F, int64_t C, const int32_t* idx, int64_t K, int64_t B,
                        int64_t honest, int32_t attack, float gamma, float weight_decay,
                        float* W, float* b, float* X, int64_t ldx, int32_t layout, void* stream);

int gm_oma_apply_f32(gm_ctx* ctx, float* X, int64_t K, int64_t d, int64_t ldx,
                     const float* h_re, const float* h_im, const float* n_re,
                     const float* n_im, void* stream);

int gm_fill_clients_f32(gm_ctx* ctx, float* X, int64_t K, int64_t d, int64_t ldx, int64_t B,
                        float mu_h, float sd_h, float mu_b, float sd_b, uint64_t seed,
                        void* stream);
int gm_fill_normal_f32(gm_ctx* ctx, float* v, int64_t n, float mu, float sd, uint64_t seed,
                       void* stream);

int gm_ctx_pass_timing(gm_ctx* ctx, int enable, double* total_ms, int64_t* launches);

const char* gm_last_error(void);
int gm_abi_version(void);

#ifdef __cplusplus
}
#endif

#endif
```

Baseline: 26.12 aggregations/s.

## Add delta Weiszfeld passes over a bf16 shadow with exact-pass corrections

Once the Weiszfeld coefficients settle, one exact fp32 pass also writes a bf16 shadow of the client panels and records a base iterate and base distances. Later iterations then stream only the bf16 shadow to compute the coefficient delta contribution, g = gbase + Xᵀ(c − cb). Distances are rebuilt algebraically from the base distances and a dot-product term. When any coefficient drifts beyond a per-config threshold, the next pass falls back to an exact fp32 pass, and timing events for whichever pass kind was skipped are dropped. The aim is to roughly halve the HBM bytes per settled iteration, at the cost of extra shadow memory and a shadow-write pass, plus added precision risk bounded by the threshold check.

After: 27.99 aggregations/s (median of 6 runs). 7.2% higher.

```diff
diff --git a/byzantine_aircomp_amd/_lib.py b/byzantine_aircomp_amd/_lib.py
--- a/byzantine_aircomp_amd/_lib.py
+++ b/byzantine_aircomp_amd/_lib.py
@@ -106,6 +106,7 @@
     ("gm_trimmed_mean_panels_f32", C.c_int, [_P, _P, _I64, _I64, _I64, _I64, _P, _P]),
     ("gm_krum_panels_f32", C.c_int, [_P, _P, _I64, _I64, _I64, _I64, _P, C.POINTER(_I64), _P]),
     ("gm_krum_last_info", C.c_int, [_P, C.POINTER(_I64)]),
+    ("gm_delta_last_info", C.c_int, [_P, C.POINTER(_I64)]),
     ("gm_meamed_f32", C.c_int, [_P, _P, _I64, _I64, _I64, C.c_int32, _P, _I64, _I64, _P, _P]),
     ("gm_multi_krum_f32", C.c_int, [_P, _P, _I64, _I64, _I64, C.c_int32, _I64, _I64, _P, _P, _P]),
     ("gm_bulyan_f32", C.c_int, [_P, _P, _I64, _I64, _I64, C.c_int32, _I64, _P, _P, _P]),
diff --git a/byzantine_aircomp_amd/aggregators.py b/byzantine_aircomp_amd/aggregators.py
--- a/byzantine_aircomp_amd/aggregators.py
+++ b/byzantine_aircomp_amd/aggregators.py
@@ -27,6 +27,9 @@
     guard: str = "none"
     gram_kind: str = ""
     exchange: str = "none"
+    corrections: int = 0
+    correction_mask: int = 0
+    shadow: str = "off"
 
 
 last_result: GMResult | None = None
@@ -38,12 +41,18 @@
                 _lib.GM_GUARD_REJECTED: "rejected", _lib.GM_GUARD_ACCEPTED_FLOOR: "accepted_floor"}
 
 
-def _result(res) -> "GMResult":
-    return GMResult(res.iters, res.last_movement, bool(res.converged),
-                    _ALGO_NAMES.get(res.algo_used, "?"), _GUARD_NAMES.get(res.guard, "?"),
-                    {1: "f16_split", 2: "bf16_split", 3: "f32"}.get(res.gram_kind, ""),
-                    {1: "agent", 2: "xcd_local", 3: "xcd_hier",
-                     4: "xcd_split"}.get(res.exchange, "none"))
+def _result(res, ctx=None) -> "GMResult":
+    r = GMResult(res.iters, res.last_movement, bool(res.converged),
+                 _ALGO_NAMES.get(res.algo_used, "?"), _GUARD_NAMES.get(res.guard, "?"),
+                 {1: "f16_split", 2: "bf16_split", 3: "f32"}.get(res.gram_kind, ""),
+                 {1: "agent", 2: "xcd_local", 3: "xcd_hier",
+                  4: "xcd_split"}.get(res.exchange, "none"))
+    if ctx is not None and res.algo_used == _lib.GM_ALGO_STREAM:
+        info = (C.c_int64 * 3)()
+        _lib.check(ctx.lib.gm_delta_last_info(ctx.handle, info), "gm_delta_last_info")
+        r.corrections, r.correction_mask = int(info[0]), int(info[1])
+        r.shadow = {1: "armed", 2: "no_shadow"}.get(int(info[2]), "off")
+    return r
 
 
 class Context:
@@ -276,7 +285,7 @@
     context(X.device).call("gm_weiszfeld_bf16" if bf16 else "gm_weiszfeld_f32", X.data_ptr(), K, d,
                            ldx, g0.data_ptr(), out.data_ptr(), C.byref(o), C.byref(res),
                            _stream_ptr(X.device))
-    last_result = _result(res)
+    last_result = _result(res, None if bf16 else context(X.device))
     if pre_var is not None and not isinstance(wList, ClientPanels) and X is not wList:
         wList.copy_(X)
     return out if wList.device == out.device else out.to(wList.device)
diff --git a/byzantine_aircomp_amd/csrc/api.hip b/byzantine_aircomp_amd/csrc/api.hip
--- a/byzantine_aircomp_amd/csrc/api.hip
+++ b/byzantine_aircomp_amd/csrc/api.hip
@@ -41,6 +41,7 @@
   if (c->comm) ncclCommDestroy(c->comm);
   if (c->ws) (void)hipFree(c->ws);
   if (c->stage) (void)hipFree(c->stage);
+  if (c->shadow) (void)hipFree(c->shadow);
   if (c->host) (void)hipHostFree(c->host);
   for (auto e : c->poll_ev)
     if (e) (void)hipEventDestroy(e);
@@ -301,6 +302,12 @@
   return GM_OK;
 }
 
+int gm_delta_last_info(gm_ctx* c, int64_t* info) {
+  if (!c || !info) return fail(GM_ERR_INVALID, "gm_delta_last_info: bad args");
+  for (int i = 0; i < 3; ++i) info[i] = c->delta_info[i];
+  return GM_OK;
+}
+
 int gm_krum_last_info(gm_ctx* c, int64_t* info) {
   if (!c || !info) return fail(GM_ERR_INVALID, "gm_krum_last_info: bad args");
   for (int i = 0; i < 3; ++i) info[i] = c->krum_info[i];
diff --git a/byzantine_aircomp_amd/csrc/gmagg_internal.h b/byzantine_aircomp_amd/csrc/gmagg_internal.h
--- a/byzantine_aircomp_amd/csrc/gmagg_internal.h
+++ b/byzantine_aircomp_amd/csrc/gmagg_internal.h
@@ -18,8 +18,14 @@
   double guard_r;
   int32_t gram_bad;
   int32_t clipped;
-  double pad1;
-};
+  uint32_t kind_mask;
+  uint32_t flags;
+};
+static_assert(sizeof(KState) == 64, "KState: one 64-byte line, as the kernels index it");
+constexpr uint32_t kFlagNextDelta = 1;
+constexpr uint32_t kFlagWriteShadow = 2;
+constexpr uint32_t kFlagShadowDone = 4;
+constexpr int kDeltaMaxIter = 32;
 
 struct PassCfg {
   int V, NW, LPR, R;
@@ -46,6 +52,10 @@
   float oma_sd;
   uint64_t oma_seed;
   int chunk_pair;
+  uint16_t* shadow;
+  int64_t shadow_stride;
+  float* gbase;
+  int64_t slab_rows;
 };
 
 __host__ __device__ inline int64_t first_chunk(int P, int64_t b, int64_t grid) {
@@ -77,9 +87,24 @@
   int* n_done;
   KState* mirror;
   double tau;
-};
+  int delta;
+  float* cb;
+  double* Db;
+  double theta;
+};
+inline double delta_theta(const PassCfg& cfg) {
+  int lq = 0;
+  if (cfg.LPR <= 0) return 0.0;
+  while ((64 / cfg.LPR) >> (lq + 1)) ++lq;
+  return (double)(cfg.R + lq + cfg.NW + 32) / (double)(1 << 17);
+}
+constexpr double kDeltaArmRatio = 64.0;
+constexpr double kDeltaArmMove = 4096.0;
 
 constexpr int kPassStepSelf = 5;
+constexpr int kPassStepExactD = 6;
+constexpr int kPassStepDelta = 7;
+const void* pass_kernel_delta(const PassCfg& cfg, int mode);
 hipError_t launch_pass(const PassCfg& cfg, int mode, int grid, const PassArgs& a, hipStream_t s,
                        int problems = 1);
 int pass_blocks_per_cu(const PassCfg& cfg, int mode);
diff --git a/byzantine_aircomp_amd/csrc/host_ctx.h b/byzantine_aircomp_amd/csrc/host_ctx.h
--- a/byzantine_aircomp_amd/csrc/host_ctx.h
+++ b/byzantine_aircomp_amd/csrc/host_ctx.h
@@ -34,6 +34,9 @@
   bool ws_pending = false;
   float* stage = nullptr;
   size_t stage_bytes = 0;
+  uint16_t* shadow = nullptr;
+  size_t shadow_bytes = 0;
+  int64_t delta_info[3] = {0, 0, GM_DELTA_OFF};
   int res_skip = 0;
   int64_t krum_info[3] = {GM_KRUM_EXACT, 0, GM_KRUM_REASON_NOT_CHOSEN};
 };
@@ -212,10 +215,13 @@
   double* G;
   double* alpha;
   double* u;
+  float* gbase;
+  float* cb;
+  double* Db;
 };
 
 inline int ensure_ws(gm_ctx* c, int64_t K, int64_t d, int nb, Workspace* w,
-                     size_t gram_slab_n = 0, int KP = 0) {
+                     size_t gram_slab_n = 0, int KP = 0, bool delta = false) {
   const size_t S = 2 * K + 2;
   auto lay = [&](char* base) {
     Carve cv{base};
@@ -233,6 +239,9 @@
     w->G = cv.take<double>((size_t)KP * KP);
     w->alpha = cv.take<double>(K);
     w->u = cv.take<double>(K);
+    w->gbase = cv.take<float>(delta ? d : 0);
+    w->cb = cv.take<float>(delta ? K : 0);
+    w->Db = cv.take<double>(delta ? K : 0);
     return cv.off;
   };
   const int rc = grow_ws(c, lay(nullptr));
@@ -303,6 +312,20 @@
   c->ev_free.push_back(c->ev_used.back().first);
   c->ev_free.push_back(c->ev_used.back().second);
   c->ev_used.pop_back();
+}
+
+inline void drop_timings(gm_ctx* c, size_t first, const std::vector<char>& drop) {
+  if (!c->timing) return;
+  size_t keep = first;
+  for (size_t i = first; i < c->ev_used.size(); ++i) {
+    if (i - first < drop.size() && drop[i - first]) {
+      c->ev_free.push_back(c->ev_used[i].first);
+      c->ev_free.push_back(c->ev_used[i].second);
+    } else {
+      c->ev_used[keep++] = c->ev_used[i];
+    }
+  }
+  c->ev_used.resize(keep);
 }
 
 
@@ -365,6 +388,30 @@
     return false;
   }
   c->stage_bytes = bytes;
+  return true;
+}
+
+
+constexpr int64_t kDeltaMinBytes = (int64_t)1 << 31;
+inline int delta_knob() {
+  static const int v = [] {
+    const char* e = getenv("GMAGG_DELTA");
+    return !e ? -1 : e[0] == '0' && !e[1] ? 0 : e[0] == '1' && !e[1] ? 1 : -1;
+  }();
+  return v;
+}
+
+inline bool ensure_shadow(gm_ctx* c, size_t bytes) {
+  if (bytes <= c->shadow_bytes) return true;
+  if (c->shadow) (void)hipFree(c->shadow);
+  c->shadow = nullptr;
+  c->shadow_bytes = 0;
+  if (hipMalloc(&c->shadow, bytes) != hipSuccess) {
+    (void)hipGetLastError();
+    c->shadow = nullptr;
+    return false;
+  }
+  c->shadow_bytes = bytes;
   return true;
 }
 
diff --git a/byzantine_aircomp_amd/csrc/host_weiszfeld.hip b/byzantine_aircomp_amd/csrc/host_weiszfeld.hip
--- a/byzantine_aircomp_amd/csrc/host_weiszfeld.hip
+++ b/byzantine_aircomp_amd/csrc/host_weiszfeld.hip
@@ -261,9 +261,42 @@
   sp.mode[1] = init_mode;
   stream_grids(c, K, d, j.algo, sp.cfg[0], sp.cfg[1], init_mode, step_mode, &sp.nb[0], &sp.nb[1]);
   const int nb = std::max(sp.nb[0], sp.nb[1]);
+  PassCfg dcfg{};
+  int64_t Wb = 0;
+  bool delta = j.rule == Rule::Gm2 && j.panels && !j.cfg.B16 && !sp.twopass && !host_noise &&
+               noise_kind == 0 && delta_knob() != 0 &&
+               (delta_knob() == 1 || 4 * K * d_total >= kDeltaMinBytes) &&
+               pass_kernel_delta(j.cfg, kPassStepExactD) != nullptr;
+  int nb_d = 0;
+  if (delta) {
+    Wb = (int64_t)j.cfg.LPR * j.cfg.V;
+    dcfg = PassCfg{8, 8, (int)(Wb / 8), 8, 2, true};
+    delta = K <= 1024 && pass_kernel_delta(dcfg, kPassStepDelta) != nullptr;
+    nb_d = (int)std::max<int64_t>(
+        1, std::min<int64_t>((d + Wb - 1) / Wb,
+                             (int64_t)c->num_cu * pass_blocks_per_cu(dcfg, kPassStepDelta)));
+  }
+  const int64_t slab_rows = std::max(sp.nb[0], nb_d);
+  c->delta_info[0] = c->delta_info[1] = 0;
+  c->delta_info[2] = GM_DELTA_OFF;
   Workspace w;
-  int rc = ensure_ws(c, K, d, nb, &w);
-  if (rc) return rc;
+  int rc = ensure_ws(c, K, d, std::max(nb, nb_d), &w, 0, 0, delta);
+  if (rc) return rc;
+  if (delta) {
+    bool have = ensure_shadow(c, sizeof(uint16_t) * (size_t)((d + Wb - 1) / Wb) * (size_t)(K * Wb));
+    if (j.tr.collective) {
+      const double mine = have ? 0.0 : 1.0;
+      double all = 0.0;
+      HIPCHK(hipMemcpyAsync(w.sums, &mine, sizeof(double), hipMemcpyHostToDevice, s));
+      rc = allreduce(c, w.sums, 1, s);
+      if (rc) return rc;
+      HIPCHK(hipMemcpyAsync(&all, w.sums, sizeof(double), hipMemcpyDeviceToHost, s));
+      HIPCHK(hipStreamSynchronize(s));
+      have = all == 0.0;
+    }
+    c->delta_info[2] = have ? GM_DELTA_ARMED : GM_DELTA_NO_SHADOW;
+    delta = have;
+  }
   rc = ensure_host(c, kHostNoiseOff + sizeof(float) * (2 * K + d_total + 1) + 256);
   if (rc) return rc;
   KState* hst = host_state(c);
@@ -291,6 +324,38 @@
   ka.n_last = w.hnoise + d;
   ka.coef = w.coef;
   ka.st = w.st;
+  ka.delta = !delta ? 0 : delta_knob() == 1 ? 2 : 1;
+  ka.cb = w.cb;
+  ka.Db = w.Db;
+  ka.theta = delta ? delta_theta(j.cfg) : 0.0;
+  const size_t timing_first = c->ev_used.size();
+
+  auto delta_pair = [&](int64_t t) -> int {
+    PassArgs a = sp.a;
+    a.g_old = w.g[(t - 1) & 1];
+    a.g_new = w.g[t & 1];
+    a.slab_stride = K + 3;
+    a.iter = t;
+    a.shadow = c->shadow;
+    a.shadow_stride = K * Wb;
+    a.gbase = w.gbase;
+    a.slab_rows = slab_rows;
+    PassArgs b = a;
+    b.X = reinterpret_cast<const float*>(c->shadow);
+    b.ldx = b.panel_stride = K * Wb;
+    const PassArgs* args[2] = {&a, &b};
+    for (int kind = 0; kind < 2; ++kind) {
+      hipEvent_t e0, e1;
+      int rc2 = record_pass_begin(c, s, &e0, &e1);
+      if (rc2) return rc2;
+      HIPCHK(launch_pass(kind ? dcfg : j.cfg, kind ? kPassStepDelta : kPassStepExactD,
+                         kind ? nb_d : sp.nb[0], *args[kind], s));
+      rc2 = record_pass_end(c, s, e0, e1);
+      if (rc2) return rc2;
+    }
+    HIPCHK(launch_slab_reduce(w.slab, (int)slab_rows, K + 3, w.sums, w.st, s));
+    return allreduce(c, w.sums, K + 3, s);
+  };
 
   auto poll = [&](KState* dst) -> int {
     HIPCHK(hipMemcpyAsync(dst, w.st, sizeof(KState), hipMemcpyDeviceToHost, s));
@@ -299,6 +364,7 @@
   };
 
   auto do_pass = [&](int64_t t) -> int {
+    if (delta && t >= 1) return delta_pair(t);
     const int rc2 = t <= 0 ? stream_pass(sp, t, j.guess0, 0, t < 0 ? nullptr : w.g[0])
                            : stream_pass(sp, t, w.g[(t - 1) & 1], 0, w.g[t & 1]);
     return rc2 ? rc2 : allreduce(c, w.sums, t < 0 ? 2 * K + 2 : K + 2, s);
@@ -375,7 +441,21 @@
   gm_result r = result_from(*final_st, j.algo);
   r.guard = j.guard_rejected ? GM_GUARD_REJECTED : GM_GUARD_NONE;
   if (r.iters < 1) return fail(GM_ERR_HIP, "Weiszfeld loop recorded no iteration");
-  for (int64_t k = r.iters; k < enqueued; ++k) drop_last_timing(c);
+  if (!delta) {
+    for (int64_t k = r.iters; k < enqueued; ++k) drop_last_timing(c);
+  } else {
+    const uint32_t mask = final_st->kind_mask;
+    std::vector<char> drop(1 + 2 * (size_t)std::max<int64_t>(0, enqueued - 1), 0);
+    for (int64_t k = 1; k < enqueued; ++k) {
+      const bool ran = k < r.iters;
+      const bool corr = k < kDeltaMaxIter && ((mask >> k) & 1u) != 0;
+      drop[1 + 2 * (k - 1)] = !ran || corr;
+      drop[2 + 2 * (k - 1)] = !ran || !corr;
+    }
+    drop_timings(c, timing_first, drop);
+    c->delta_info[0] = __builtin_popcount(mask);
+    c->delta_info[1] = mask;
+  }
   HIPCHK(hipMemcpyAsync(j.out, w.g[(r.iters - 1) & 1], sizeof(float) * d, hipMemcpyDeviceToDevice,
                         s));
   if (res) *res = r;
diff --git a/byzantine_aircomp_amd/csrc/stream_pass.hip b/byzantine_aircomp_amd/csrc/stream_pass.hip
--- a/byzantine_aircomp_amd/csrc/stream_pass.hip
+++ b/byzantine_aircomp_amd/csrc/stream_pass.hip
@@ -50,6 +50,8 @@
 }
 
 static const void* pass_kernel(const PassCfg& cfg, int mode, bool panel = false) {
+  if (mode == kPassStepExactD || mode == kPassStepDelta)
+    return panel ? pass_kernel_delta(cfg, mode) : nullptr;
   if (cfg.B16) return pass_kernel_bf16(cfg, mode, panel);
   if (mode == kPassStepSelf) return pass_kernel_self(cfg, panel);
 #define GMK_CASE(V_, W_, L_, R_, O_)                                                 \
@@ -76,7 +78,7 @@
 }
 
 int pass_blocks_per_cu(const PassCfg& cfg, int mode) {
-  const void* fn = pass_kernel(cfg, mode);
+  const void* fn = pass_kernel(cfg, mode, mode == kPassStepExactD || mode == kPassStepDelta);
   int n = 0;
   if (!fn || hipOccupancyMaxActiveBlocksPerMultiprocessor(&n, fn, cfg.NW * 64, 0) != hipSuccess ||
       n < 1)
diff --git a/byzantine_aircomp_amd/csrc/stream_pass_bf16.hip b/byzantine_aircomp_amd/csrc/stream_pass_bf16.hip
--- a/byzantine_aircomp_amd/csrc/stream_pass_bf16.hip
+++ b/byzantine_aircomp_amd/csrc/stream_pass_bf16.hip
@@ -36,4 +36,10 @@
   return nullptr;
 }
 
+const void* pass_kernel_bf16_delta(const PassCfg& cfg) {
+  if (!(cfg.B16 && cfg.V == 8 && cfg.NW == 8 && cfg.LPR == 4 && cfg.R == 8 && cfg.OCC == 2))
+    return nullptr;
+  return reinterpret_cast<const void*>(&weiszfeld_pass<8, 8, 4, 8, 0, 0, 2, true, true, false, 2>);
 }
+
+}
diff --git a/byzantine_aircomp_amd/csrc/stream_pass_delta.hip b/byzantine_aircomp_amd/csrc/stream_pass_delta.hip
--- /dev/null
+++ b/byzantine_aircomp_amd/csrc/stream_pass_delta.hip
@@ -0,0 +1,18 @@
+#include "stream_pass_kernel.h"
+
+namespace gmk {
+
+const void* pass_kernel_bf16_delta(const PassCfg& cfg);
+
+const void* pass_kernel_delta(const PassCfg& cfg, int mode) {
+  if (mode == kPassStepDelta) return cfg.B16 && cfg.V == 8 ? pass_kernel_bf16_delta(cfg) : nullptr;
+  if (mode != kPassStepExactD || cfg.B16 || cfg.V != 4 || cfg.NW != 8 || cfg.LPR != 8 ||
+      cfg.R != 16 || cfg.OCC != 2)
+    return nullptr;
+  if (pass_variant() == 0)
+    return reinterpret_cast<const void*>(
+        &weiszfeld_pass<4, 8, 8, 16, 0, 0, 2, true, false, false, 1>);
+  return reinterpret_cast<const void*>(&weiszfeld_pass<4, 8, 8, 16, 0, 2, 2, true, false, false, 1>);
+}
+
+}
diff --git a/byzantine_aircomp_amd/csrc/stream_pass_kernel.h b/byzantine_aircomp_amd/csrc/stream_pass_kernel.h
--- a/byzantine_aircomp_amd/csrc/stream_pass_kernel.h
+++ b/byzantine_aircomp_amd/csrc/stream_pass_kernel.h
@@ -14,8 +14,10 @@
 
 namespace gmk {
 
-template <int V, int R, bool B16 = false>
-struct Tile {
+template <bool GB> struct TileBase {};
+template <> struct TileBase<true> { float gb; };
+template <int V, int R, bool B16 = false, bool GB = false>
+struct Tile : TileBase<GB> {
   static_assert(!B16 || V == 8, "bf16 tiles: 8 columns = one 16-byte load per lane");
   typedef typename std::conditional<B16, uint32_t, float>::type word;
   word x[R][B16 ? V / 2 : V];
@@ -24,9 +26,12 @@
 };
 
 template <int V, int NW, int LPR, int R, int MODE, int SCHED, int OCC = 1, bool PANEL = false,
-          bool B16 = false, bool SELF = false>
+          bool B16 = false, bool SELF = false, int DELTA = 0>
 __global__ void __launch_bounds__(NW * 64, OCC * NW / 4) weiszfeld_pass(PassArgs a) {
   static_assert(!SELF || MODE == 0, "the old iterate as column term: STEP passes only");
+  static_assert(DELTA == 0 || (MODE == 0 && PANEL && !SELF), "DELTA: gm2 STEP on panels");
+  static_assert(DELTA != 1 || (!B16 && V == 4), "the shadow is written from the fp32 tile");
+  static_assert(DELTA != 2 || (B16 && SCHED == 0), "the correction pass reads the bf16 shadow");
   constexpr bool PIPE = SCHED == 1, ROLL = SCHED == 2 || SCHED == 3, ROLL2 = SCHED == 3;
   constexpr bool SUM_ONLY = MODE == 3;
   constexpr bool OMA_INIT = MODE == 4;
@@ -40,12 +45,13 @@
   constexpr int J = LPR * V;
   constexpr int RPL = R > LPR ? R / LPR : 1;
   static_assert(J <= NW * 64, "one finisher thread per column");
-  using T = Tile<V, R, B16>;
+  using T = Tile<V, R, B16, DELTA == 2>;
+  constexpr int NFIN = DELTA == 2 ? 3 : 2;
 
   typedef typename std::conditional<SELF, double, float>::type red_t;
   __shared__ red_t s_red[NW][J];
   __shared__ float s_g[INIT ? 2 : 1][J];
-  __shared__ double s_fin[2][NW];
+  __shared__ double s_fin[NFIN][NW];
   __shared__ float s_w[OCC > 1 ? NW * QW * R : 1];
 
   if (gridDim.y > 1) {
@@ -60,6 +66,13 @@
     a.oma_seed += (uint64_t)pb * kSeedStride;
   }
   if (!SUM_ONLY && a.st->done) return;
+  bool wr_shadow = false;
+  (void)wr_shadow;
+  if constexpr (DELTA != 0) {
+    const uint32_t fl = a.st->flags;
+    if (((fl & kFlagNextDelta) != 0) != (DELTA == 2)) return;
+    wr_shadow = DELTA == 1 && (fl & kFlagWriteShadow) != 0;
+  }
 
   const int tid = threadIdx.x, lane = tid & 63;
   const int w = __builtin_amdgcn_readfirstlane(tid >> 6);
@@ -150,6 +163,7 @@
     const bool fin = tid < J && ch < nch && gj < d;
     t.gold = fin ? a.g_old[gj] : 0.f;
     if constexpr (!INIT) t.hn = (fin && a.noise == 2) ? a.hnoise[gj] : 0.f;
+    if constexpr (DELTA == 2) t.gb = fin ? a.gbase[gj] : 0.f;
   };
   auto fetch = [&](int64_t ch, T& t) {
 #pragma unroll
@@ -160,7 +174,7 @@
   double row_acc[RPL], row_acc2[RPL];
 #pragma unroll
   for (int m = 0; m < RPL; ++m) row_acc[m] = row_acc2[m] = 0.0;
-  double mv_acc = 0.0, gn_acc = 0.0;
+  double mv_acc = 0.0, gn_acc = 0.0, cg_acc = 0.0;
 
   int par = 0;
   auto oma_tile = [&](int64_t ch, auto& t) {
@@ -190,9 +204,31 @@
       }
     }
   };
+  auto store_shadow = [&](int64_t ch, const auto& t) {
+    auto rne = [](float f) -> uint32_t {
+      const uint32_t u = __float_as_uint(f);
+      return f != f ? 0x7fc0u : (u + 0x7fffu + ((u >> 16) & 1u)) >> 16;
+    };
+    constexpr int RB = J * 2;
+    char* const pan = reinterpret_cast<char*>(a.shadow + ch * a.shadow_stride);
+    const uint32_t vo = (uint32_t)(q * RB + c * V * 2);
+#pragma unroll
+    for (int i = 0; i < R; ++i) {
+      const int64_t wb = (int64_t)(w * QW + NRG * i) * RB;
+      const int64_t nrec = (int64_t)K * RB - wb;
+      const __amdgpu_buffer_rsrc_t rs = __builtin_amdgcn_make_buffer_rsrc(
+          pan + wb, 0, nrec <= 0 ? 0 : (int)nrec, 0x00020000);
+      typedef uint32_t u2 __attribute__((ext_vector_type(2)));
+      const u2 o = u2{rne(t.x[i][0]) | rne(t.x[i][1]) << 16, rne(t.x[i][2]) | rne(t.x[i][3]) << 16};
+      __builtin_amdgcn_raw_buffer_store_b64(o, rs, vo, 0, 0);
+    }
+  };
   auto process = [&](int64_t ch, T& t, int64_t nxt) {
     float gv[V];
     zero_padding(ch, t);
+    if constexpr (DELTA == 1) {
+      if (wr_shadow) store_shadow(ch, t);
+    }
     if constexpr (OMA_INIT) oma_tile(ch, t);
     if constexpr (INIT) {
       if (tid < J) {
@@ -272,10 +308,17 @@
             gnew = fmaf(a_noise, t.hn, gnew);
           }
           if constexpr (SELF) gnew = (float)fma((double)a_noise, (double)t.gold, (double)sum);
+          if constexpr (DELTA == 2) gnew = t.gb + sum;
           a.g_new[gj] = gnew;
+          if constexpr (DELTA == 1) a.gbase[gj] = gnew;
           const float diff = t.gold - gnew;
           mv_acc += (double)(diff * diff);
           gn_acc += (double)(gnew * gnew);
+        }
+        if constexpr (DELTA == 2) {
+          const float dj = gj < d ? gnew - t.gb : 0.f;
+          cg_acc += (double)dj * ((double)dj + 2.0 * (double)t.gb);
+          gnew = dj;
         }
         s_g[0][tid] = gnew;
       }
@@ -302,6 +345,10 @@
 #pragma unroll
         for (int j = 0; j < V / 2; ++j) {
           const f2 xv = xpair(t, i, j);
+          if constexpr (DELTA == 2) {
+            sp = __builtin_elementwise_fma(xv, f2{gv[2 * j], gv[2 * j + 1]}, sp);
+            continue;
+          }
           const f2 tt = xv - f2{gv[2 * j], gv[2 * j + 1]};
           sp = __builtin_elementwise_fma(tt, tt, sp);
           if constexpr (WANT_R) sp2 = __builtin_elementwise_fma(xv, xv, sp2);
@@ -381,11 +428,19 @@
       }
     }
   }
+  if constexpr (DELTA != 0) {
+    for (int64_t r = blockIdx.x + grid; r < a.slab_rows; r += grid)
+      for (int64_t k2 = tid; k2 < a.slab_stride; k2 += NW * 64) a.slab[r * a.slab_stride + k2] = 0.0;
+  }
   const double mv = wave_sum(mv_acc), gn = wave_sum(gn_acc);
   if (lane == 0) {
     s_fin[0][w] = mv;
     s_fin[1][w] = gn;
   }
+  if constexpr (DELTA == 2) {
+    const double cg = wave_sum(cg_acc);
+    if (lane == 0) s_fin[2][w] = cg;
+  }
   __syncthreads();
   if (tid == 0) {
     double m = 0.0, g = 0.0;
@@ -397,6 +452,12 @@
     const int64_t b = SUM_ONLY ? 0 : INIT ? 2 * K : K;
     out[b] = m;
     out[b + 1] = g;
+    if constexpr (DELTA == 2) {
+      double cg = 0.0;
+#pragma unroll
+      for (int ww = 0; ww < NW; ++ww) cg += s_fin[2][ww];
+      out[b + 2] = cg;
+    }
   }
 }
 
diff --git a/byzantine_aircomp_amd/csrc/weiszfeld.hip b/byzantine_aircomp_amd/csrc/weiszfeld.hip
--- a/byzantine_aircomp_amd/csrc/weiszfeld.hip
+++ b/byzantine_aircomp_amd/csrc/weiszfeld.hip
@@ -42,6 +42,53 @@
 
 __device__ void kspace_body(KspaceArgs& a);
 
+__device__ void kspace_gm2_delta(KspaceArgs& a, bool ran_delta, uint32_t fl_in, double* scratch) {
+  KState* st = a.st;
+  const int tid = threadIdx.x;
+  const int64_t K = a.K;
+  const bool init = a.t < 0;
+  const bool new_base = !ran_delta && a.t >= 1;
+  const bool shadow_done = (fl_in & kFlagShadowDone) != 0 ||
+                           (new_base && (fl_in & kFlagWriteShadow) != 0);
+  const double C = ran_delta ? a.sums[K + 2] : 0.0;
+  auto dist2 = [&](int64_t k) {
+    return ran_delta ? fmax(a.Db[k] + C - 2.0 * a.sums[k], 0.0) : a.sums[k];
+  };
+  double wsum = 0.0;
+  for (int64_t k = tid; k < K; k += blockDim.x) wsum += 1.0 / (double)clamp_dist(dist2(k), a.eps);
+  const double W = block_sum(wsum, scratch);
+  double viol = 0.0, unsettled = 0.0;
+  for (int64_t k = tid; k < K; k += blockDim.x) {
+    const double ck = (double)(float)((1.0 / (double)clamp_dist(dist2(k), a.eps)) / W);
+    if (shadow_done) {
+      const double cbk = new_base ? (double)a.coef[k] : (double)a.cb[k];
+      if (!(fabs(ck - cbk) <= a.theta * cbk)) viol += 1.0;
+    } else if (!init) {
+      const double cp = (double)a.coef[k];
+      if (!(fabs(ck - cp) <= kDeltaArmRatio * a.theta * cp)) unsettled += 1.0;
+    }
+  }
+  const double nviol = block_sum(viol, scratch);
+  const double nuns = block_sum(unsettled, scratch);
+  const bool next_delta = shadow_done && nviol == 0.0 && a.t + 1 < kDeltaMaxIter;
+  for (int64_t k = tid; k < K; k += blockDim.x) {
+    const float ck = (float)((1.0 / (double)clamp_dist(dist2(k), a.eps)) / W);
+    if (new_base) {
+      a.cb[k] = a.coef[k];
+      a.Db[k] = a.sums[k];
+    }
+    a.coef[k] = next_delta ? (float)((double)ck - (double)a.cb[k]) : ck;
+  }
+  if (tid == 0) {
+    const float mv = init ? 0.f : (float)sqrt(a.sums[K]);
+    const bool arm = !init && !shadow_done && a.t + 2 < kDeltaMaxIter &&
+                     (a.delta == 2 ||
+                      (nuns == 0.0 && (double)mv > kDeltaArmMove * (double)a.tol));
+    st->flags = (shadow_done ? kFlagShadowDone : 0u) | (next_delta ? kFlagNextDelta : 0u) |
+                (arm ? kFlagWriteShadow : 0u);
+  }
+}
+
 __global__ void __launch_bounds__(1024) kspace_step(KspaceArgs a) {
   kspace_body(a);
   if (a.mirror && threadIdx.x == 0 && gridDim.x == 1) *a.mirror = *a.st;
@@ -65,9 +112,12 @@
   const bool init = a.t < 0;
   const double* D2 = a.sums;
   const double gn2 = init ? a.sums[2 * K + 1] : a.sums[K + 1];
+  const uint32_t fl_in = a.delta ? st->flags : 0u;
+  const bool ran_delta = a.delta && a.t >= 1 && (fl_in & kFlagNextDelta) != 0;
 
   if (tid == 0) {
     s_stop = 0;
+    if (ran_delta) st->kind_mask |= 1u << a.t;
     if (a.do_check && !init) {
       const float mv = (float)sqrt(a.sums[K]);
       st->last_movement = (double)mv;
@@ -85,6 +135,10 @@
   __syncthreads();
   if (s_stop || !a.do_coef) return;
 
+  if (a.mode == 0 && a.delta) {
+    kspace_gm2_delta(a, ran_delta, fl_in, scratch);
+    return;
+  }
   if (a.mode == 0) {
     double wsum = 0.0;
     for (int64_t k = tid; k < K; k += blockDim.x) wsum += 1.0 / (double)clamp_dist(D2[k], a.eps);
diff --git a/byzantine_aircomp_amd/sharded.py b/byzantine_aircomp_amd/sharded.py
--- a/byzantine_aircomp_amd/sharded.py
+++ b/byzantine_aircomp_amd/sharded.py
@@ -131,7 +131,7 @@
         res = _lib.GmResult()
         self.ctx.call("gm_weiszfeld_f32", ptr, X.shape[0], self.d_local, ldx, g0.data_ptr(),
                       out.data_ptr(), C.byref(o), C.byref(res), _stream_ptr(self.device))
-        self.last_result = _result(res)
+        self.last_result = _result(res, self.ctx)
         if o.pre_oma and X is not X_in:
             X_in.copy_(X)
         return out
diff --git a/include/gmagg.h b/include/gmagg.h
--- a/include/gmagg.h
+++ b/include/gmagg.h
@@ -105,6 +105,13 @@
                      const float* guess0, float* out, const gm_opts* opts,
                      gm_result* result, void* stream);
 
+enum gm_delta_status {
+  GM_DELTA_OFF = 0,
+  GM_DELTA_ARMED = 1,
+  GM_DELTA_NO_SHADOW = 2
+};
+int gm_delta_last_info(gm_ctx* ctx, int64_t* info);
+
 int64_t gm_panel_width(int64_t K);
 
 int gm_weiszfeld_bf16(gm_ctx* ctx, const uint16_t* X, int64_t K, int64_t d, int64_t ldx,
```
